# UDC-GAC/pRIblast

Measured on AMD Instinct MI355X. Metric: query RNAs/sec in `ris` step, higher is better.
Workload: dtype f64

## Files before the change

include/priblast_hip.h:

```cpp
#ifndef PRIBLAST_HIP_H
#define PRIBLAST_HIP_H

#include <stddef.h>
#include <stdint.h>

#ifdef __cplusplus
extern "C" {
#endif

#define PRB_OK 0
#define PRB_ERR_ARG (-1)
#define PRB_ERR_IO (-2)
#define PRB_ERR_HIP (-3)
#define PRB_ERR_NOMEM (-4)
#define PRB_ERR_STATE (-5)

typedef struct prb_ctx prb_ctx;
typedef struct prb_db prb_db;
typedef struct prb_qbatch prb_qbatch;
typedef struct prb_hitset prb_hitset;
typedef struct prb_pairmask prb_pairmask;

typedef struct prb_ris_opts {
  int32_t max_seed_length;
  double hybrid_threshold;
  double interaction_threshold;
  double final_threshold;
  int32_t drop_out_wo_gap;
  int32_t drop_out_w_gap;
  int32_t min_helix_length;
  int32_t output_style;
  int32_t distinct_sites;
  int32_t chain_sites;
  const prb_pairmask *allowed_pairs;
} prb_ris_opts;
#ifdef __cplusplus
static_assert(sizeof(prb_ris_opts) == 64, "prb_ris_opts: eleven fields, allowed_pairs the last one, no tail padding");
#endif


int prb_pairmask_create(prb_ctx *ctx, const prb_qbatch *qb, const prb_db *db, prb_pairmask **out);
int prb_pairmask_allow(prb_pairmask *pm, int64_t n, const int32_t *query, const int32_t *page, const int32_t *db_id);
int64_t prb_pairmask_count(const prb_pairmask *pm);
void prb_pairmask_free(prb_pairmask *pm);

typedef struct prb_hit {
  int32_t q_sp, db_sp;
  int32_t q_len, db_len;
  int32_t db_id, db_id_start;
  double e_acc, e_hyb, e_tot;
  int32_t query;
  int32_t bp_count;
  int64_t bp_offset;
} prb_hit;

const char *prb_last_error(void);
const char *prb_version(void);
int prb_cpu_budget(void);
int prb_host_threads_default(void);
void prb_ris_opts_default(prb_ris_opts *o);

int prb_ctx_create(int device, const char *param_file, prb_ctx **out);
void prb_ctx_destroy(prb_ctx *ctx);
int prb_ctx_synchronize(prb_ctx *ctx);
int prb_ctx_stage_ms(prb_ctx *ctx, const char *stage, double *ms, int64_t *launches);
void prb_ctx_reset_timers(prb_ctx *ctx);

int prb_accessibility(prb_ctx *ctx, int32_t nseq, const char *seqs, const int64_t *offsets,
                      int32_t maximal_span, int32_t min_accessible_length, float *acc, float *cond);

int prb_accessibility_tables(prb_ctx *ctx, const char *seq, int32_t len, int32_t maximal_span,
                             int32_t min_accessible_length, float *acc, float *cond,
                             double *alpha_outer, double *beta_outer, double *const tables[12]);

int prb_encode_query(const char *seq, int32_t len, int32_t repeat_flag, uint8_t *enc );
int prb_suffix_array(const uint8_t *text, int32_t n, int32_t *sa);
int prb_shuffle_sequence(const char *seq, int32_t len, uint64_t seed, int64_t file_pos, int32_t decoy, char *out);

int prb_db_open(prb_ctx *ctx, const char *prefix, prb_db **out);
int prb_db_open_streaming(prb_ctx *ctx, const char *prefix, int32_t max_resident_pages, prb_db **out);
int64_t prb_db_page_uploads(const prb_db *db);
void prb_db_close(prb_db *db);
int prb_db_info(const prb_db *db, int32_t *hash_size, int32_t *repeat_flag, int32_t *maximal_span,
                int32_t *min_accessible_length, int32_t *npages);
int prb_db_page_info(const prb_db *db, int32_t page, int32_t *nseq, int64_t *nchars);
const char *prb_db_seq_name(const prb_db *db, int32_t page, int32_t id);
int prb_db_seq_lengths(const prb_db *db, int32_t page, int32_t id, int32_t *length,
                       int32_t *length_unmasked, int32_t *start_pos);
int prb_db_build(prb_ctx *ctx, const char *prefix, int32_t nseq, const char *const *names,
                 const char *seqs, const int64_t *offsets, int32_t repeat_flag, int32_t hash_size,
                 int32_t maximal_span, int32_t min_accessible_length, int32_t page_size);

int prb_qbatch_create(prb_ctx *ctx, int32_t nq, const char *seqs, const int64_t *offsets,
                      int32_t repeat_flag, prb_qbatch **out);
void prb_qbatch_destroy(prb_qbatch *qb);
int prb_qbatch_accessibility(prb_ctx *ctx, prb_qbatch *qb, int32_t maximal_span,
                             int32_t min_accessible_length);
int prb_qbatch_get(prb_qbatch *qb, int32_t q, uint8_t *enc, int32_t *sa, float *acc, float *cond);
int32_t prb_qbatch_length_unmasked(const prb_qbatch *qb, int32_t q);
int prb_qbatch_seed_search_begin(prb_ctx *ctx, prb_qbatch *qb, const prb_db *db, int32_t page, const prb_ris_opts *opts);

int prb_search_page(prb_ctx *ctx, prb_qbatch *qb, prb_db *db, int32_t page, const prb_ris_opts *opts,
                    int32_t last_stage, prb_hitset **out);
int64_t prb_hitset_size(const prb_hitset *hs);
const prb_hit *prb_hitset_hits(const prb_hitset *hs);
const int32_t *prb_hitset_basepairs(const prb_hitset *hs, int64_t *count);
void prb_hitset_counts(const prb_hitset *hs, int64_t counts[3]);
void prb_hitset_free(prb_hitset *hs);

int prb_distinct_sites(prb_ctx *ctx, const prb_hit *hits, int64_t n, uint8_t *keep);
int prb_chain_sites(prb_ctx *ctx, const prb_hit *hits, int64_t n, uint8_t *keep);

enum {
  PRB_SORT_PACKED_TWO_LENGTHS = 0,
  PRB_SORT_PACKED_ONE_LENGTH = 1,
  PRB_SORT_GENERAL_WIDTH = 2,
  PRB_SORT_GENERAL_TIE_RUN = 3,
  PRB_SORT_GENERAL_FORCED = 4
};
int prb_sort_filter(prb_ctx *ctx, const prb_hit *hits, int64_t n, double threshold, prb_hit *sorted, uint8_t *keep,
                    int32_t *form);

typedef struct prb_pair_summary {
  int32_t query, db_id;
  int64_t hits;
  double e_min, e_sum, e_acc, e_hyb;
  int32_t bp_first[2], bp_last[2];
} prb_pair_summary;
typedef struct prb_pairset prb_pairset;
int prb_search_page_summary(prb_ctx *ctx, prb_qbatch *qb, prb_db *db, int32_t page, const prb_ris_opts *opts,
                            prb_pairset **out);
int64_t prb_pairset_size(const prb_pairset *ps);
const prb_pair_summary *prb_pairset_pairs(const prb_pairset *ps);
void prb_pairset_counts(const prb_pairset *ps, int64_t counts[3]);
void prb_pairset_free(prb_pairset *ps);

typedef struct prb_top_pair {
  prb_pair_summary s;
  int32_t page, rank;
} prb_top_pair;
typedef struct prb_topset prb_topset;
int prb_topset_create(prb_ctx *ctx, const prb_qbatch *qb, int32_t n, prb_topset **out);
int prb_search_page_top(prb_ctx *ctx, prb_qbatch *qb, prb_db *db, int32_t page, const prb_ris_opts *opts,
                        prb_topset *ts);
int prb_topset_merge(prb_ctx *ctx, prb_topset *dst, prb_topset *src);
int prb_topset_finish(prb_ctx *ctx, prb_topset *ts);
int64_t prb_topset_size(const prb_topset *ts);
const prb_top_pair *prb_topset_pairs(const prb_topset *ts);
void prb_topset_counts(const prb_topset *ts, int64_t counts[3]);
void prb_topset_free(prb_topset *ts);

typedef struct prb_top_hit {
  prb_hit h;
  int32_t page, rank;
} prb_top_hit;
typedef struct prb_tophits prb_tophits;
int prb_tophits_create(prb_ctx *ctx, const prb_qbatch *qb, int32_t n, prb_tophits **out);
int prb_search_page_tophits(prb_ctx *ctx, prb_qbatch *qb, prb_db *db, int32_t page, const prb_ris_opts *opts,
                            prb_tophits *th);
int prb_tophits_merge(prb_ctx *ctx, prb_tophits *dst, prb_tophits *src);
int prb_tophits_finish(prb_ctx *ctx, prb_tophits *th);
int64_t prb_tophits_size(const prb_tophits *th);
const prb_top_hit *prb_tophits_hits(const prb_tophits *th);
const int32_t *prb_tophits_basepairs(const prb_tophits *th, int64_t *npairs);
void prb_tophits_counts(const prb_tophits *th, int64_t counts[3]);
void prb_tophits_free(prb_tophits *th);

typedef struct prb_profile_pos {
  int32_t query, pos;
  int64_t hits;
  int32_t targets, page, db_id;
  int32_t reserved;
  double e_min;
  int32_t bp_first[2], bp_last[2];
} prb_profile_pos;
typedef struct prb_profset prb_profset;
int prb_profset_create(prb_ctx *ctx, const prb_qbatch *qb, prb_profset **out);
int prb_search_page_profile(prb_ctx *ctx, prb_qbatch *qb, prb_db *db, int32_t page, const prb_ris_opts *opts,
                            prb_profset *ps);
int prb_profset_merge(prb_ctx *ctx, prb_profset *dst, prb_profset *src);
int prb_profset_finish(prb_ctx *ctx, prb_profset *ps);
int64_t prb_profset_size(const prb_profset *ps);
const prb_profile_pos *prb_profset_rows(const prb_profset *ps);
void prb_profset_counts(const prb_profset *ps, int64_t counts[3]);
void prb_profset_free(prb_profset *ps);

typedef struct prb_target_pair {
  prb_pair_summary s;
  int32_t page, rank;
} prb_target_pair;
typedef struct prb_targetset prb_targetset;
int prb_targetset_create(prb_ctx *ctx, prb_db *db, int32_t n, prb_targetset **out);
int prb_search_page_targets(prb_ctx *ctx, prb_qbatch *qb, prb_db *db, int32_t page, const prb_ris_opts *opts,
                            const int32_t *query_ids, prb_targetset *ts);
int prb_targetset_merge(prb_ctx *ctx, prb_targetset *dst, prb_targetset *src);
int prb_targetset_finish(prb_ctx *ctx, prb_targetset *ts);
int64_t prb_targetset_size(const prb_targetset *ts);
const prb_target_pair *prb_targetset_pairs(const prb_targetset *ts);
void prb_targetset_counts(const prb_targetset *ts, int64_t counts[3]);
void prb_targetset_free(prb_targetset *ts);

typedef struct prb_target_region {
  int32_t page, db_id;
  int32_t start, end;
  int64_t hits, max_hits;
  int32_t max_queries, peak;
  double e_min;
  int32_t query, reserved;
  int32_t bp_first[2], bp_last[2];
} prb_target_region;
#ifdef __cplusplus
static_assert(sizeof(prb_target_region) == 72, "prb_target_region: no padding");
#endif
// ... 81 lines not shown
```

priblast_amd/capi.py:

```python
import ctypes
import os
import subprocess

import numpy as np

ROOT = os.path.dirname(os.path.abspath(__file__))
LIB_PATH = os.environ.get("PRB_LIB_PATH") or os.path.join(ROOT, "lib", "libpriblast_hip.so")
BIN_PATH = os.path.join(ROOT, "bin", "pRIblast-hip")
PARAMS = os.path.join(ROOT, "params", "rna_andronescu2007.par")

c_i32, c_i64, c_dbl = ctypes.c_int32, ctypes.c_int64, ctypes.c_double
P = ctypes.POINTER


class RisOpts(ctypes.Structure):
    _fields_ = [("max_seed_length", c_i32), ("hybrid_threshold", c_dbl), ("interaction_threshold", c_dbl),
                ("final_threshold", c_dbl), ("drop_out_wo_gap", c_i32), ("drop_out_w_gap", c_i32),
                ("min_helix_length", c_i32), ("output_style", c_i32), ("distinct_sites", c_i32), ("chain_sites", c_i32),
                ("allowed_pairs", ctypes.c_void_p)]


class Hit(ctypes.Structure):
    _fields_ = [("q_sp", c_i32), ("db_sp", c_i32), ("q_len", c_i32), ("db_len", c_i32), ("db_id", c_i32),
                ("db_id_start", c_i32), ("e_acc", c_dbl), ("e_hyb", c_dbl), ("e_tot", c_dbl), ("query", c_i32),
                ("bp_count", c_i32), ("bp_offset", c_i64)]


class PageHits(ctypes.Structure):
    _fields_ = [("hits", ctypes.c_void_p), ("nhits", c_i64), ("basepairs", ctypes.c_void_p), ("npairs", c_i64)]


HIT_DTYPE = np.dtype([("q_sp", "<i4"), ("db_sp", "<i4"), ("q_len", "<i4"), ("db_len", "<i4"), ("db_id", "<i4"),
                      ("db_id_start", "<i4"), ("e_acc", "<f8"), ("e_hyb", "<f8"), ("e_tot", "<f8"),
                      ("query", "<i4"), ("bp_count", "<i4"), ("bp_offset", "<i8")])
assert HIT_DTYPE.itemsize == ctypes.sizeof(Hit)

PAIR_DTYPE = np.dtype([("query", "<i4"), ("db_id", "<i4"), ("hits", "<i8"), ("e_min", "<f8"), ("e_sum", "<f8"),
                       ("e_acc", "<f8"), ("e_hyb", "<f8"), ("bp_first", "<i4", (2,)), ("bp_last", "<i4", (2,))])
assert PAIR_DTYPE.itemsize == 64

TOP_DTYPE = np.dtype(PAIR_DTYPE.descr + [("page", "<i4"), ("rank", "<i4")])
assert TOP_DTYPE.itemsize == 72

TOPHIT_DTYPE = np.dtype(HIT_DTYPE.descr + [("page", "<i4"), ("rank", "<i4")])
assert TOPHIT_DTYPE.itemsize == 72

TARGET_DTYPE = np.dtype(PAIR_DTYPE.descr + [("page", "<i4"), ("rank", "<i4")])
assert TARGET_DTYPE.itemsize == 72

PROFILE_DTYPE = np.dtype([("query", "<i4"), ("pos", "<i4"), ("hits", "<i8"), ("targets", "<i4"), ("page", "<i4"),
                          ("db_id", "<i4"), ("reserved", "<i4"), ("e_min", "<f8"), ("bp_first", "<i4", (2,)),
                          ("bp_last", "<i4", (2,))])
assert PROFILE_DTYPE.itemsize == 56

REGION_DTYPE = np.dtype([("page", "<i4"), ("db_id", "<i4"), ("start", "<i4"), ("end", "<i4"), ("hits", "<i8"),
                         ("max_hits", "<i8"), ("max_queries", "<i4"), ("peak", "<i4"), ("e_min", "<f8"), ("query", "<i4"),
                         ("reserved", "<i4"), ("bp_first", "<i4", (2,)), ("bp_last", "<i4", (2,))])
assert REGION_DTYPE.itemsize == 72

NULL_DTYPE = np.dtype(PAIR_DTYPE.descr + [("page", "<i4"), ("decoys", "<i4"), ("null_hits", "<i8"), ("null_le", "<i8"),
                                          ("null_min", "<f8")])
assert NULL_DTYPE.itemsize == 96


class PagePairs(ctypes.Structure):
    _fields_ = [("pairs", ctypes.c_void_p), ("npairs", c_i64)]

SYMBOLS = {
    "prb_last_error": (ctypes.c_char_p, []),
    "prb_version": (ctypes.c_char_p, []),
    "prb_cpu_budget": (ctypes.c_int, []),
    "prb_host_threads_default": (ctypes.c_int, []),
    "prb_ris_opts_default": (None, [P(RisOpts)]),
    "prb_ctx_create": (ctypes.c_int, [ctypes.c_int, ctypes.c_char_p, P(ctypes.c_void_p)]),
    "prb_ctx_destroy": (None, [ctypes.c_void_p]),
    "prb_ctx_synchronize": (ctypes.c_int, [ctypes.c_void_p]),
    "prb_ctx_stage_ms": (ctypes.c_int, [ctypes.c_void_p, ctypes.c_char_p, P(c_dbl), P(c_i64)]),
    "prb_ctx_reset_timers": (None, [ctypes.c_void_p]),
    "prb_accessibility": (ctypes.c_int, [ctypes.c_void_p, c_i32, ctypes.c_char_p, ctypes.c_void_p, c_i32, c_i32,
                                         ctypes.c_void_p, ctypes.c_void_p]),
    "prb_accessibility_tables": (ctypes.c_int, [ctypes.c_void_p, ctypes.c_char_p, c_i32, c_i32, c_i32,
                                                ctypes.c_void_p, ctypes.c_void_p, ctypes.c_void_p, ctypes.c_void_p,
                                                ctypes.c_void_p]),
    "prb_encode_query": (ctypes.c_int, [ctypes.c_char_p, c_i32, c_i32, ctypes.c_void_p]),
    "prb_suffix_array": (ctypes.c_int, [ctypes.c_void_p, c_i32, ctypes.c_void_p]),
    "prb_db_open": (ctypes.c_int, [ctypes.c_void_p, ctypes.c_char_p, P(ctypes.c_void_p)]),
    "prb_db_open_streaming": (ctypes.c_int, [ctypes.c_void_p, ctypes.c_char_p, c_i32, P(ctypes.c_void_p)]),
    "prb_db_page_uploads": (c_i64, [ctypes.c_void_p]),
    "prb_db_close": (None, [ctypes.c_void_p]),
    "prb_db_info": (ctypes.c_int, [ctypes.c_void_p, P(c_i32), P(c_i32), P(c_i32), P(c_i32), P(c_i32)]),
    "prb_db_page_info": (ctypes.c_int, [ctypes.c_void_p, c_i32, P(c_i32), P(c_i64)]),
    "prb_db_seq_name": (ctypes.c_char_p, [ctypes.c_void_p, c_i32, c_i32]),
    "prb_db_seq_lengths": (ctypes.c_int, [ctypes.c_void_p, c_i32, c_i32, P(c_i32), P(c_i32), P(c_i32)]),
    "prb_db_build": (ctypes.c_int, [ctypes.c_void_p, ctypes.c_char_p, c_i32, P(ctypes.c_char_p), ctypes.c_char_p,
                                    ctypes.c_void_p, c_i32, c_i32, c_i32, c_i32, c_i32]),
    "prb_qbatch_create": (ctypes.c_int, [ctypes.c_void_p, c_i32, ctypes.c_char_p, ctypes.c_void_p, c_i32,
                                         P(ctypes.c_void_p)]),
    "prb_qbatch_destroy": (None, [ctypes.c_void_p]),
    "prb_qbatch_accessibility": (ctypes.c_int, [ctypes.c_void_p, ctypes.c_void_p, c_i32, c_i32]),
    "prb_qbatch_get": (ctypes.c_int, [ctypes.c_void_p, c_i32, ctypes.c_void_p, ctypes.c_void_p, ctypes.c_void_p,
                                      ctypes.c_void_p]),
    "prb_qbatch_length_unmasked": (c_i32, [ctypes.c_void_p, c_i32]),
    "prb_qbatch_seed_search_begin": (ctypes.c_int, [ctypes.c_void_p, ctypes.c_void_p, ctypes.c_void_p, c_i32, P(RisOpts)]),
    "prb_search_page": (ctypes.c_int, [ctypes.c_void_p, ctypes.c_void_p, ctypes.c_void_p, c_i32, P(RisOpts), c_i32,
                                       P(ctypes.c_void_p)]),
    "prb_pairmask_create": (ctypes.c_int, [ctypes.c_void_p, ctypes.c_void_p, ctypes.c_void_p, P(ctypes.c_void_p)]),
    "prb_pairmask_allow": (ctypes.c_int, [ctypes.c_void_p, c_i64, ctypes.c_void_p, ctypes.c_void_p, ctypes.c_void_p]),
    "prb_pairmask_count": (c_i64, [ctypes.c_void_p]),
    "prb_pairmask_free": (None, [ctypes.c_void_p]),
    "prb_hitset_size": (c_i64, [ctypes.c_void_p]),
    "prb_hitset_hits": (ctypes.c_void_p, [ctypes.c_void_p]),
    "prb_hitset_basepairs": (ctypes.c_void_p, [ctypes.c_void_p, P(c_i64)]),
    "prb_hitset_counts": (None, [ctypes.c_void_p, P(c_i64)]),
    "prb_hitset_free": (None, [ctypes.c_void_p]),
    "prb_distinct_sites": (ctypes.c_int, [ctypes.c_void_p, ctypes.c_void_p, c_i64, ctypes.c_void_p]),
    "prb_chain_sites": (ctypes.c_int, [ctypes.c_void_p, ctypes.c_void_p, c_i64, ctypes.c_void_p]),
    "prb_sort_filter": (ctypes.c_int, [ctypes.c_void_p, ctypes.c_void_p, c_i64, c_dbl, ctypes.c_void_p, ctypes.c_void_p,
                                       ctypes.c_void_p]),
    "prb_search_page_summary": (ctypes.c_int, [ctypes.c_void_p, ctypes.c_void_p, ctypes.c_void_p, c_i32, P(RisOpts),
                                               P(ctypes.c_void_p)]),
    "prb_pairset_size": (c_i64, [ctypes.c_void_p]),
    "prb_pairset_pairs": (ctypes.c_void_p, [ctypes.c_void_p]),
    "prb_pairset_counts": (None, [ctypes.c_void_p, P(c_i64)]),
    "prb_pairset_free": (None, [ctypes.c_void_p]),
    "prb_topset_create": (ctypes.c_int, [ctypes.c_void_p, ctypes.c_void_p, c_i32, P(ctypes.c_void_p)]),
    "prb_search_page_top": (ctypes.c_int, [ctypes.c_void_p, ctypes.c_void_p, ctypes.c_void_p, c_i32, P(RisOpts), ctypes.c_void_p]),
    "prb_topset_merge": (ctypes.c_int, [ctypes.c_void_p, ctypes.c_void_p, ctypes.c_void_p]),
    "prb_topset_finish": (ctypes.c_int, [ctypes.c_void_p, ctypes.c_void_p]),
    "prb_topset_size": (c_i64, [ctypes.c_void_p]),
    "prb_topset_pairs": (ctypes.c_void_p, [ctypes.c_void_p]),
    "prb_topset_counts": (None, [ctypes.c_void_p, P(c_i64)]),
    "prb_topset_free": (None, [ctypes.c_void_p]),
    "prb_tophits_create": (ctypes.c_int, [ctypes.c_void_p, ctypes.c_void_p, c_i32, P(ctypes.c_void_p)]),
    "prb_search_page_tophits": (ctypes.c_int, [ctypes.c_void_p, ctypes.c_void_p, ctypes.c_void_p, c_i32, P(RisOpts), ctypes.c_void_p]),
    "prb_tophits_merge": (ctypes.c_int, [ctypes.c_void_p, ctypes.c_void_p, ctypes.c_void_p]),
    "prb_tophits_finish": (ctypes.c_int, [ctypes.c_void_p, ctypes.c_void_p]),
    "prb_tophits_size": (c_i64, [ctypes.c_void_p]),
    "prb_tophits_hits": (ctypes.c_void_p, [ctypes.c_void_p]),
    "prb_tophits_basepairs": (ctypes.c_void_p, [ctypes.c_void_p, P(c_i64)]),
    "prb_tophits_counts": (None, [ctypes.c_void_p, P(c_i64)]),
    "prb_tophits_free": (None, [ctypes.c_void_p]),
    "prb_profset_create": (ctypes.c_int, [ctypes.c_void_p, ctypes.c_void_p, P(ctypes.c_void_p)]),
    "prb_search_page_profile": (ctypes.c_int, [ctypes.c_void_p, ctypes.c_void_p, ctypes.c_void_p, c_i32, P(RisOpts), ctypes.c_void_p]),
    "prb_profset_merge": (ctypes.c_int, [ctypes.c_void_p, ctypes.c_void_p, ctypes.c_void_p]),
    "prb_profset_finish": (ctypes.c_int, [ctypes.c_void_p, ctypes.c_void_p]),
    "prb_profset_size": (c_i64, [ctypes.c_void_p]),
    "prb_profset_rows": (ctypes.c_void_p, [ctypes.c_void_p]),
    "prb_profset_counts": (None, [ctypes.c_void_p, P(c_i64)]),
    "prb_profset_free": (None, [ctypes.c_void_p]),
    "prb_targetset_create": (ctypes.c_int, [ctypes.c_void_p, ctypes.c_void_p, c_i32, P(ctypes.c_void_p)]),
    "prb_search_page_targets": (ctypes.c_int, [ctypes.c_void_p, ctypes.c_void_p, ctypes.c_void_p, c_i32, P(RisOpts), ctypes.c_void_p,
                                               ctypes.c_void_p]),
    "prb_targetset_merge": (ctypes.c_int, [ctypes.c_void_p, ctypes.c_void_p, ctypes.c_void_p]),
    "prb_targetset_finish": (ctypes.c_int, [ctypes.c_void_p, ctypes.c_void_p]),
    "prb_targetset_size": (c_i64, [ctypes.c_void_p]),
    "prb_targetset_pairs": (ctypes.c_void_p, [ctypes.c_void_p]),
    "prb_targetset_counts": (None, [ctypes.c_void_p, P(c_i64)]),
    "prb_targetset_free": (None, [ctypes.c_void_p]),
    "prb_covset_create": (ctypes.c_int, [ctypes.c_void_p, ctypes.c_void_p, P(ctypes.c_void_p)]),
    "prb_search_page_coverage": (ctypes.c_int, [ctypes.c_void_p, ctypes.c_void_p, ctypes.c_void_p, c_i32, P(RisOpts), ctypes.c_void_p,
                                                ctypes.c_void_p]),
    "prb_covset_add_hits": (ctypes.c_int, [ctypes.c_void_p, ctypes.c_void_p, c_i32, ctypes.c_void_p, c_i32, ctypes.c_void_p, c_i64,
                                           ctypes.c_void_p, c_i64]),
    "prb_covset_merge": (ctypes.c_int, [ctypes.c_void_p, ctypes.c_void_p, ctypes.c_void_p]),
    "prb_covset_finish": (ctypes.c_int, [ctypes.c_void_p, ctypes.c_void_p, c_i32]),
    "prb_covset_size": (c_i64, [ctypes.c_void_p]),
    "prb_covset_regions": (ctypes.c_void_p, [ctypes.c_void_p]),
    "prb_covset_counts": (None, [ctypes.c_void_p, P(c_i64)]),
    "prb_covset_free": (None, [ctypes.c_void_p]),
    "prb_nullset_create": (ctypes.c_int, [ctypes.c_void_p, ctypes.c_void_p, ctypes.c_void_p, c_i32, P(ctypes.c_void_p)]),
    "prb_search_page_observed": (ctypes.c_int, [ctypes.c_void_p, ctypes.c_void_p, ctypes.c_void_p, c_i32, P(RisOpts), ctypes.c_void_p]),
    "prb_search_page_decoys": (ctypes.c_int, [ctypes.c_void_p, ctypes.c_void_p, ctypes.c_void_p, c_i32, P(RisOpts), ctypes.c_void_p,
                                              ctypes.c_void_p, ctypes.c_void_p]),
    "prb_nullset_observe": (ctypes.c_int, [ctypes.c_void_p, ctypes.c_void_p, c_i32, ctypes.c_void_p, c_i64]),
    "prb_nullset_add_pairs": (ctypes.c_int, [ctypes.c_void_p, ctypes.c_void_p, c_i32, ctypes.c_void_p, ctypes.c_void_p, c_i32,
                                             ctypes.c_void_p, c_i64]),
    "prb_nullset_finish": (ctypes.c_int, [ctypes.c_void_p, ctypes.c_void_p]),
    "prb_nullset_size": (c_i64, [ctypes.c_void_p]),
    "prb_nullset_pairs": (ctypes.c_void_p, [ctypes.c_void_p]),
    "prb_nullset_counts": (None, [ctypes.c_void_p, P(c_i64)]),
    "prb_nullset_decoy_counts": (None, [ctypes.c_void_p, P(c_i64)]),
    "prb_nullset_free": (None, [ctypes.c_void_p]),
    "prb_write_null_lines": (ctypes.c_int, [ctypes.c_void_p, c_i32, P(ctypes.c_char_p), ctypes.c_void_p, ctypes.c_void_p, c_i64,
                                            c_i64, ctypes.c_int, P(c_i64), P(c_i64)]),
    "prb_comm_unique_id": (ctypes.c_int, [ctypes.c_char_p]),
    "prb_comm_create": (ctypes.c_int, [ctypes.c_void_p, c_i32, c_i32, ctypes.c_char_p, P(ctypes.c_void_p)]),
    "prb_comm_destroy": (None, [ctypes.c_void_p]),
    "prb_gather_hits": (ctypes.c_int, [ctypes.c_void_p, ctypes.c_void_p, c_i32, ctypes.c_void_p, c_i32, P(ctypes.c_void_p)]),
    "prb_hitset_gathered_queries": (ctypes.c_int, [ctypes.c_void_p, P(c_i32), P(P(c_i32)), P(P(c_i32))]),
    "prb_gather_plan": (ctypes.c_int, [c_i32, ctypes.c_void_p, ctypes.c_void_p]),
    "prb_ctx_keep_device_records": (None, [ctypes.c_void_p, c_i32]),
    "prb_write_lines": (ctypes.c_int, [ctypes.c_void_p, c_i32, P(ctypes.c_char_p), ctypes.c_void_p, ctypes.c_void_p, c_i32,
                                       c_i32, c_i64, ctypes.c_int, P(c_i64), P(c_i64)]),
    "prb_write_summary_lines": (ctypes.c_int, [ctypes.c_void_p, c_i32, P(ctypes.c_char_p), ctypes.c_void_p, ctypes.c_void_p,
                                               c_i32, c_i64, ctypes.c_int, P(c_i64), P(c_i64)]),
    "prb_write_top_lines": (ctypes.c_int, [ctypes.c_void_p, c_i32, P(ctypes.c_char_p), ctypes.c_void_p, ctypes.c_void_p, c_i64,
                                           c_i64, ctypes.c_int, P(c_i64), P(c_i64)]),
    "prb_shuffle_sequence": (ctypes.c_int, [ctypes.c_char_p, c_i32, ctypes.c_uint64, c_i64, c_i32, ctypes.c_char_p]),
    "prb_write_target_lines": (ctypes.c_int, [ctypes.c_void_p, c_i32, P(ctypes.c_char_p), ctypes.c_void_p, ctypes.c_void_p, c_i64,
                                              c_i64, ctypes.c_int, P(c_i64), P(c_i64)]),
    "prb_write_profile_lines": (ctypes.c_int, [ctypes.c_void_p, c_i32, P(ctypes.c_char_p), ctypes.c_void_p, ctypes.c_void_p, c_i64,
                                               c_i64, ctypes.c_int, P(c_i64), P(c_i64)]),
    "prb_write_region_lines": (ctypes.c_int, [ctypes.c_void_p, c_i32, P(ctypes.c_char_p), ctypes.c_void_p, ctypes.c_void_p, c_i64,
                                              c_i64, ctypes.c_int, P(c_i64), P(c_i64)]),
}

_lib = None


def build():
    subprocess.run(["make", "-s", "-j8", "-C", os.path.join(ROOT, "csrc")], check=True)


def lib():
    global _lib
    if _lib is None:
        if not os.path.exists(LIB_PATH):
            raise RuntimeError(f"{LIB_PATH} is missing: run `python -c 'import __graft_entry__ as g; g.build()'` "
                               "(there is no CPU fallback)")
        L = ctypes.CDLL(LIB_PATH)
        for name, (res, args) in SYMBOLS.items():
            if not hasattr(L, name):
                continue
            fn = getattr(L, name)
            fn.restype = res
            fn.argtypes = args
        _lib = L
    return _lib


class PrbError(RuntimeError):
    pass


def _check(rc):
    if rc != 0:
        raise PrbError(f"libpriblast_hip error {rc}: {lib().prb_last_error().decode()}")


def _concat(seqs):
    offs = np.zeros(len(seqs) + 1, np.int64)
    for i, s in enumerate(seqs):
        offs[i + 1] = offs[i] + len(s)
    return "".join(seqs).encode(), offs


def encode_query(seq, repeat_flag=0):
    enc = np.zeros(len(seq) + 1, np.uint8)
    _check(lib().prb_encode_query(seq.encode(), len(seq), repeat_flag, enc.ctypes.data))
    return enc


def suffix_array(text):
    text = np.ascontiguousarray(text, np.uint8)
    sa = np.zeros(len(text), np.int32)
    _check(lib().prb_suffix_array(text.ctypes.data, len(text), sa.ctypes.data))
    return sa


def shuffle_sequence(seq, seed=1, file_pos=0, decoy=0):
    raw = seq.encode("latin-1") if isinstance(seq, str) else bytes(seq)
    out = ctypes.create_string_buffer(max(len(raw), 1))
    _check(lib().prb_shuffle_sequence(raw, len(raw), seed, file_pos, decoy, out))
    res = out.raw[:len(raw)]
    return res.decode("latin-1") if isinstance(seq, str) else res


def default_opts(**kw):
    o = RisOpts()
    lib().prb_ris_opts_default(ctypes.byref(o))
    for k, v in kw.items():
        setattr(o, k, v)
    return o


class Context:
    def __init__(self, device=0, param_file=None):
        h = ctypes.c_void_p()
        _check(lib().prb_ctx_create(device, param_file.encode() if param_file else PARAMS.encode(), ctypes.byref(h)))
        self.h = h

    def close(self):
        if self.h:
            lib().prb_ctx_destroy(self.h)
            self.h = None

    def __enter__(self):
        return self

    def __exit__(self, *a):
        self.close()

    def accessibility(self, seqs, W=70, delta=5):
        buf, offs = _concat(seqs)
        total = int(offs[-1])
        acc = np.zeros(max(total, 1), np.float32)
        cond = np.zeros(max(total, 1), np.float32)
        _check(lib().prb_accessibility(self.h, len(seqs), buf, offs.ctypes.data, W, delta, acc.ctypes.data,
                                       cond.ctypes.data))
        return [(acc[offs[i]:offs[i + 1]], cond[offs[i]:offs[i + 1]]) for i in range(len(seqs))]

    def accessibility_tables(self, seq, W=70, delta=5):
        L = len(seq)
        acc = np.zeros(max(L, 1), np.float32)
        cond = np.zeros(max(L, 1), np.float32)
        out = {"alpha_outer": np.zeros(L + 1), "beta_outer": np.zeros(L + 1)}
        names = ["stem", "stemend", "multi", "multibif", "multi1", "multi2"]
        ptrs = (ctypes.c_void_p * 12)()
        k = 0
        for side in ("alpha", "beta"):
            for nm in names:
                t = np.zeros((L + 1, W + 2))
                out[f"{side}_{nm}"] = t
                ptrs[k] = t.ctypes.data
                k += 1
        _check(lib().prb_accessibility_tables(self.h, seq.encode(), L, W, delta, acc.ctypes.data, cond.ctypes.data,
                                              out["alpha_outer"].ctypes.data, out["beta_outer"].ctypes.data, ptrs))
        return acc[:L], cond[:L], out

    def stage_ms(self, stage):
        ms, n = c_dbl(), c_i64()
        _check(lib().prb_ctx_stage_ms(self.h, stage.encode(), ctypes.byref(ms), ctypes.byref(n)))
        return ms.value, n.value

    def reset_timers(self):
        lib().prb_ctx_reset_timers(self.h)

    def synchronize(self):
        _check(lib().prb_ctx_synchronize(self.h))


class Db:

    def __init__(self, ctx, prefix, max_resident_pages=None):
        h = ctypes.c_void_p()
        if max_resident_pages is None:
            _check(lib().prb_db_open(ctx.h, prefix.encode(), ctypes.byref(h)))
        else:
            _check(lib().prb_db_open_streaming(ctx.h, prefix.encode(), max_resident_pages, ctypes.byref(h)))
        self.h, self.ctx = h, ctx
        v = [c_i32() for _ in range(5)]
        _check(lib().prb_db_info(self.h, *[ctypes.byref(x) for x in v]))
        self.hash_size, self.repeat_flag, self.W, self.delta, self.npages = (x.value for x in v)

    def close(self):
        if self.h:
            lib().prb_db_close(self.h)
            self.h = None

    @property
    def page_uploads(self):
        return lib().prb_db_page_uploads(self.h)

    def page_info(self, page):
        n, c = c_i32(), c_i64()
        _check(lib().prb_db_page_info(self.h, page, ctypes.byref(n), ctypes.byref(c)))
        return n.value, c.value

    def seq_name(self, page, i):
        return lib().prb_db_seq_name(self.h, page, i).decode()

    def seq_lengths(self, page, i):
        a, b, c = c_i32(), c_i32(), c_i32()
        _check(lib().prb_db_seq_lengths(self.h, page, i, ctypes.byref(a), ctypes.byref(b), ctypes.byref(c)))
        return a.value, b.value, c.value


def db_build(ctx, prefix, names, seqs, repeat_flag=0, hash_size=8, W=70, delta=5, page_size=2 ** 31 - 1):
    buf, offs = _concat(seqs)
    arr = (ctypes.c_char_p * len(names))(*[n.encode() for n in names])
    _check(lib().prb_db_build(ctx.h, prefix.encode(), len(seqs), arr, buf, offs.ctypes.data, repeat_flag, hash_size, W,
                              delta, page_size))


class QBatch:

    def __init__(self, ctx, seqs, repeat_flag=0):
        buf, offs = _concat(seqs)
        h = ctypes.c_void_p()
        _check(lib().prb_qbatch_create(ctx.h, len(seqs), buf, offs.ctypes.data, repeat_flag, ctypes.byref(h)))
        self.h, self.ctx, self.lens = h, ctx, [len(s) for s in seqs]

    def close(self):
        if self.h:
            lib().prb_qbatch_destroy(self.h)
            self.h = None

    def accessibility(self, W, delta):
        _check(lib().prb_qbatch_accessibility(self.ctx.h, self.h, W, delta))

    def get(self, q):
        L = self.lens[q]
        enc = np.zeros(L + 1, np.uint8)
        sa = np.zeros(L + 1, np.int32)
        acc = np.zeros(max(L, 1), np.float32)
        cond = np.zeros(max(L, 1), np.float32)
        _check(lib().prb_qbatch_get(self.h, q, enc.ctypes.data, sa.ctypes.data, acc.ctypes.data, cond.ctypes.data))
        return enc, sa, acc[:L], cond[:L]

    def length_unmasked(self, q):
        return lib().prb_qbatch_length_unmasked(self.h, q)

    def seed_search_begin(self, db, page, opts=None):
        o = opts or default_opts()
        _check(lib().prb_qbatch_seed_search_begin(self.ctx.h, self.h, db.h, page, ctypes.byref(o)))


class PairMask:

    def __init__(self, ctx, qb, db):
        h = ctypes.c_void_p()
        _check(lib().prb_pairmask_create(ctx.h, qb.h, db.h, ctypes.byref(h)))
        self.h = h

    def allow(self, query, page, db_id):
        q, p, d = (np.ascontiguousarray(np.atleast_1d(x), np.int32) for x in (query, page, db_id))
        assert len(q) == len(p) == len(d)
        _check(lib().prb_pairmask_allow(self.h, len(q), q.ctypes.data, p.ctypes.data, d.ctypes.data))
        return self

# ... 455 lines not shown
```

priblast_amd/csrc/capi_search.hip:

```cpp
#include <omp.h>

#include <algorithm>
#include <cmath>
#include <cstdlib>
#include <cstring>

#include "search_stages.hpp"

using namespace prb;

namespace prb {

static bool env_off(const char *e) { return e && atoi(e) == 0; }
static SearchKnobs read_search_knobs() {
  SearchKnobs k;
  const char *e;
  e = getenv("PRB_SEARCH_PAIRS");
  k.budget = e ? atof(e) : 4.0e8;
  k.chunk_pairs = k.budget;
  if ((e = getenv("PRB_SEARCH_CHUNK_PAIRS"))) k.chunk_pairs = atof(e);
  e = getenv("PRB_SEED_ROW_SHIFT");
  k.row_shift = e ? std::min(atoi(e), 30) : 7;
  k.fused = !env_off(getenv("PRB_SEED_FUSED"));
  k.front_ahead = !getenv("PRB_NO_FRONT_AHEAD");
  k.sort_four_keys = getenv("PRB_SORT_FOUR_KEYS") != nullptr;
  k.sort_two_lengths = getenv("PRB_SORT_TWO_LENGTHS") != nullptr;
  e = getenv("PRB_BIG_LIST_BYTES");
  k.big_list_bytes = e ? (size_t)atof(e) : (size_t)20 << 30;
  e = getenv("PRB_GAPPED_CHUNK_HITS");
  k.gapped_chunk_hits = e ? std::max<int64_t>(1, (int64_t)atof(e)) : 120000000;
  e = getenv("PRB_GAPPED_FIRST_TIER");
  k.first_tier = e ? std::min(std::max(atoi(e), 0), kWaveTier) : 0;
  k.wave_hbm = getenv("PRB_GAPPED_WAVE_HBM") != nullptr;
  k.no_resume = getenv("PRB_GAPPED_NO_RESUME") != nullptr;
  e = getenv("PRB_GAPPED_RESUME_CAP");
  k.resume_cap = e ? std::max(1, atoi(e)) : 0;
  k.front_paired = getenv("PRB_GAPPED_FRONT_PAIRED") != nullptr;
  e = getenv("PRB_GAPPED_SKIP_TIERS");
  k.skip_tiers = e ? atoi(e) : 0;
  k.front = !env_off(getenv("PRB_GAPPED_FRONT"));
  k.handover = !env_off(getenv("PRB_GAPPED_HANDOVER"));
  k.tiers.pair = !env_off(getenv("PRB_GAPPED_PAIR"));
  k.tiers.pool = !env_off(getenv("PRB_GAPPED_POOL"));
  GapTierKnobs &t = k.tiers;
  if ((e = getenv("PRB_GAPPED_LDS_PAD"))) sscanf(e, "%d,%d,%d", &t.pad[1], &t.pad[2], &t.pad[3]);
  t.pad_set = e != nullptr;
  if ((e = getenv("PRB_GAPPED_PERIOD"))) sscanf(e, "%d,%d,%d,%d", &t.period[0], &t.period[1], &t.period[2], &t.period[3]);
  t.period_set = e != nullptr;
  if ((e = getenv("PRB_GAPPED_EARLY"))) sscanf(e, "%d,%d,%d,%d", &t.early[0], &t.early[1], &t.early[2], &t.early[3]);
  t.early_set = e != nullptr;
  k.filter_tiles = !env_off(getenv("PRB_FILTER_TILES"));
  k.trace_no_long = getenv("PRB_TRACE_NO_LONG") != nullptr;
  e = getenv("PRB_TRACE_LONG_CAP");
  k.trace_long_cap = e ? std::max(1, atoi(e)) : 1024;
  k.trace_no_slots = getenv("PRB_TRACE_NO_SLOTS") != nullptr;
  e = getenv("PRB_TRACE_SLOT_CAP");
  k.trace_slot_cap = e ? std::min(kTraceCap, atoi(e)) : kTraceCap;
  e = getenv("PRB_DISTINCT_LDS_HITS");
  k.distinct_lds_hits = e ? atoi(e) : kSiteLdsHits;
  e = getenv("PRB_CHAIN_LDS_HITS");
  k.chain_lds_hits = e ? atoi(e) : kChainLdsHits;
  k.debug_rows = getenv("PRB_DEBUG_ROWS") != nullptr;
  k.debug_mem = getenv("PRB_DEBUG_MEM") != nullptr;
  return k;
}

HitSoA carve_hits(uint8_t *p, int64_t n) {
  HitSoA h;
  const size_t n8 = ((size_t)n + 1) & ~(size_t)1;
  h.e_acc = reinterpret_cast<double *>(p);
  h.e_hyb = h.e_acc + n8;
  h.e_tot = h.e_hyb + n8;
  int32_t *ip = reinterpret_cast<int32_t *>(h.e_tot + n8);
  h.q_sp = ip;
  h.db_sp = ip + n8;
  h.q_len = ip + 2 * n8;
  h.db_len = ip + 3 * n8;
  h.db_id = ip + 4 * n8;
  h.db_id_start = ip + 5 * n8;
  h.query = ip + 6 * n8;
  return h;
}

int sort_target_keys(hipStream_t s, DevBuf &tmp, const uint32_t *kin, uint32_t *kout, const uint32_t *vin, uint32_t *vout, size_t n, unsigned bits) {
  return sort_pairs(s, tmp, kin, kout, vin, vout, n, bits);
}
hipError_t sort_span_keys(void *tmp, size_t &bytes, uint64_t *kin, uint64_t *kout, uint32_t *vin, uint32_t *vout, size_t n, int bits, hipStream_t s) {
  return rocprim::radix_sort_pairs(tmp, bytes, kin, kout, vin, vout, n, 0, bits, s);
}

static int sort_hits(prb_ctx *ctx, SearchWs &w, const SearchKnobs &k, const HitRec *recs, HitSoA out, int64_t n, const SortBounds &sb,
                     uint32_t **perm_out, int32_t *form = nullptr) {
  int rc;
  int32_t why = PRB_SORT_GENERAL_FORCED;
  const size_t N = (size_t)n;
  {
    PackedKeyInfo f;
    f.qmin = sb.qmin;
    f.one_len = sb.eq_len_max > 0;
    f.lmax = f.one_len ? sb.eq_len_max : std::max(sb.max_qlen, sb.max_dblen);
    f.bl = bits_for(f.lmax);
    f.bq = bits_for(sb.max_qlen);
    f.bd = bits_for(sb.nchars);
    const int total = (f.one_len ? 1 : 2) * f.bl + f.bq + f.bd + bits_for(sb.qspan - 1);
    if (!k.sort_four_keys) why = PRB_SORT_GENERAL_WIDTH;
    if (total <= 64 && f.lmax <= 65535 && !k.sort_four_keys) {
      if ((rc = w.kP.ensure(N * 8)) || (rc = w.kTmp2.ensure(N * 8)) || (rc = w.kE.ensure(N * 8)) || (rc = w.kTmp.ensure(N * 8)) ||
          (rc = w.idxA.ensure(N * 4)) || (rc = w.idxB.ensure(N * 4)) || (rc = w.pending.ensure(16)))
        return rc;
      PRB_HIP(launch_make_packed_keys_recs(recs, n, f, w.kP.as<uint64_t>(), w.kE.as<uint64_t>(), w.idxA.as<uint32_t>(), ctx->stream));
      if ((rc = sort_pairs(ctx->stream, w.sortTmp, w.kP.as<uint64_t>(), w.kTmp2.as<uint64_t>(), w.idxA.as<uint32_t>(),
                           w.idxB.as<uint32_t>(), N, (unsigned)total)))
        return rc;
      PRB_HIP(launch_gather_u64(w.kE.as<uint64_t>(), w.idxB.as<uint32_t>(), w.kTmp.as<uint64_t>(), n, ctx->stream));
      PRB_HIP(hipMemsetAsync(w.pending.p, 0, 4, ctx->stream));
      PRB_HIP(launch_fix_ties(w.kTmp2.as<uint64_t>(), w.kTmp.as<uint64_t>(), w.idxB.as<uint32_t>(), n, recs, w.idxA.as<uint32_t>(),
                              w.pending.as<int32_t>(), ctx->stream));
      int32_t too_long = 0;
      PRB_HIP(hipMemcpyAsync(&too_long, w.pending.p, 4, hipMemcpyDeviceToHost, ctx->stream));
      PRB_HIP(hipStreamSynchronize(ctx->stream));
      if (!too_long) {
        PRB_HIP(launch_gather_recs_to_hits(recs, w.idxA.as<uint32_t>(), out, n, ctx->stream));
        *perm_out = w.idxA.as<uint32_t>();
        if (form) *form = f.one_len ? PRB_SORT_PACKED_ONE_LENGTH : PRB_SORT_PACKED_TWO_LENGTHS;
        return PRB_OK;
      }
      why = PRB_SORT_GENERAL_TIE_RUN;
    }
  }
  if (form) *form = why;
  if (k.debug_mem) fprintf(stderr, "[mem] sort: the general form (%lld hits)\n", (long long)n);
  if ((rc = w.hitsTmp.ensure(hits_bytes(n)))) return rc;
  const HitSoA in = carve_hits(w.hitsTmp, n);
  PRB_HIP(launch_gather_recs_to_hits(recs, nullptr, in, n, ctx->stream));
  if ((rc = w.kE.ensure(N * 8)) || (rc = w.kL.ensure(N * 4)) || (rc = w.kQ.ensure(N * 4)) || (rc = w.kP.ensure(N * 8)) ||
      (rc = w.kTmp.ensure(N * 8)) || (rc = w.kTmp2.ensure(N * 8)) || (rc = w.idxA.ensure(N * 4)) ||
      (rc = w.idxB.ensure(N * 4)))
    return rc;
  PRB_HIP(launch_make_keys(in, n, w.kE.as<uint64_t>(), w.kL.as<uint32_t>(), w.kQ.as<uint32_t>(), w.kP.as<uint64_t>(),
                           w.idxA.as<uint32_t>(), ctx->stream));
  uint32_t *ia = w.idxA.as<uint32_t>(), *ib = w.idxB.as<uint32_t>();
  auto sort_step = [&](auto *keys, unsigned bits) -> int {
    using K = std::remove_pointer_t<decltype(keys)>;
    if (int r = sort_pairs(ctx->stream, w.sortTmp, keys, w.kTmp2.as<K>(), ia, ib, N, bits)) return r;
    std::swap(ia, ib);
    return PRB_OK;
  };
  PRB_HIP(launch_order_keys(in.e_acc, n, w.kTmp.as<uint64_t>(), ctx->stream));
  if ((rc = sort_step(w.kTmp.as<uint64_t>(), 64))) return rc;
  PRB_HIP(launch_order_keys(in.e_hyb, n, w.kTmp2.as<uint64_t>(), ctx->stream));
  PRB_HIP(launch_gather_u64(w.kTmp2.as<uint64_t>(), ia, w.kTmp.as<uint64_t>(), n, ctx->stream));
  if ((rc = sort_step(w.kTmp.as<uint64_t>(), 64))) return rc;
  PRB_HIP(launch_gather_u64(w.kE.as<uint64_t>(), ia, w.kTmp.as<uint64_t>(), n, ctx->stream));
  if ((rc = sort_step(w.kTmp.as<uint64_t>(), 64))) return rc;
  PRB_HIP(launch_gather_u32(w.kL.as<uint32_t>(), ia, w.kTmp.as<uint32_t>(), n, ctx->stream));
  if ((rc = sort_step(w.kTmp.as<uint32_t>(), 32))) return rc;
  PRB_HIP(launch_gather_u32(w.kQ.as<uint32_t>(), ia, w.kTmp.as<uint32_t>(), n, ctx->stream));
  if ((rc = sort_step(w.kTmp.as<uint32_t>(), 32))) return rc;
  PRB_HIP(launch_gather_u64(w.kP.as<uint64_t>(), ia, w.kTmp.as<uint64_t>(), n, ctx->stream));
  unsigned qbits = 1;
  while ((int64_t(1) << qbits) < (int64_t)sb.qmin + sb.qspan && qbits < 31) qbits++;
  if ((rc = sort_step(w.kTmp.as<uint64_t>(), 32 + qbits))) return rc;
  PRB_HIP(launch_gather_hits(in, ia, out, n, ctx->stream));
  *perm_out = ia;
  return PRB_OK;
}

struct MaxOp {
  __host__ __device__ int64_t operator()(const int64_t &a, const int64_t &b) const { return a > b ? a : b; }
};

static int filter_hits(prb_ctx *ctx, SearchWs &w, const HitSoA &h, int64_t n, double thr, bool tiles, int64_t *nsurv) {
  int rc;
  const size_t N = (size_t)n;
  *nsurv = 0;
  if (n == 0) return PRB_OK;
  if ((rc = w.endKey.ensure(N * 8)) || (rc = w.pmax.ensure(N * 8)) || (rc = w.state.ensure(N)) || (rc = w.keep.ensure(N)) ||
      (rc = w.pending.ensure(16)) || (rc = w.surv.ensure(N * 4)) || (rc = w.count.ensure(16)))
    return rc;
  PRB_HIP(launch_filter_init(h, n, thr, w.endKey.as<int64_t>(), w.state.as<uint8_t>(), ctx->stream));
  if ((rc = with_temp(w.scanTmp, "rocprim::inclusive_scan", [&](void *t, size_t &b) {
         return rocprim::inclusive_scan(t, b, w.endKey.as<int64_t>(), w.pmax.as<int64_t>(), N, MaxOp(), ctx->stream);
       })))
    return rc;
  for (int round = 0;; round++) {
    PRB_HIP(hipMemsetAsync(w.pending.p, 0, 4, ctx->stream));
    PRB_HIP(launch_filter_round(h, n, w.pmax.as<int64_t>(), w.state.as<uint8_t>(), w.pending.as<int32_t>(), tiles, ctx->stream));
    int32_t pend = 0;
    PRB_HIP(hipMemcpyAsync(&pend, w.pending.p, 4, hipMemcpyDeviceToHost, ctx->stream));
    PRB_HIP(hipStreamSynchronize(ctx->stream));
    if (!pend) break;
    if (round > 100000) {
      set_error("redundancy filter did not converge");
      return PRB_ERR_STATE;
    }
  }
  PRB_HIP(launch_filter_final(h, n, w.pmax.as<int64_t>(), w.state.as<uint8_t>(), w.keep.as<uint8_t>(), tiles, ctx->stream));
  return select_flagged(ctx, w, nullptr, w.keep.as<uint8_t>(), w.surv.as<uint32_t>(), N, nsurv);
}

static void mem_note(const char *where, const SearchWs &w) {
  static const bool on = getenv("PRB_DEBUG_MEM") != nullptr;
  if (!on) return;
  size_t free_b = 0, total_b = 0;
  (void)hipMemGetInfo(&free_b, &total_b);
  fprintf(stderr, "[mem] %-18s free %7zu MiB | hitsA %6zu hitsB %6zu hitsC %6zu hitsTmp %6zu MiB\n", where, free_b >> 20, w.hitsA.cap >> 20,
          w.hitsB.cap >> 20, w.hitsC.cap >> 20, w.hitsTmp.cap >> 20);
}

int grow_keep(prb_ctx *ctx, DevBuf &buf, size_t have, size_t need, size_t spare_limit) {
  int rc;
  if (have > 0 && need > buf.cap) {
    DevBuf bigger;
    if ((rc = need > spare_limit ? PRB_ERR_NOMEM : bigger.ensure(need + need / 2)) && (rc = bigger.ensure(need + need / 6)) &&
        (rc = bigger.ensure(need)))
      return rc;
    PRB_HIP(hipMemcpyAsync(bigger.p, buf.p, have, hipMemcpyDeviceToDevice, ctx->stream));
    PRB_HIP(hipStreamSynchronize(ctx->stream));
    buf.release();
    buf = bigger;
    return PRB_OK;
  }
  return buf.ensure(need);
}
static int reserve_recs(prb_ctx *ctx, DevBuf &recbuf, int64_t have, int64_t more) {
  return grow_keep(ctx, recbuf, (size_t)have * sizeof(HitRec), ((size_t)have + (size_t)more) * sizeof(HitRec), (size_t)16 << 30);
}

int compact_below(prb_ctx *ctx, SearchWs &w, const HitSoA &in, int64_t n, double thr, DevBuf &idxbuf, DevBuf &recbuf, int64_t *m,
                  int64_t have) {
  int rc;
  *m = 0;
  if (n == 0) return PRB_OK;
  const size_t N = (size_t)n;
  if ((rc = w.keep.ensure(N)) || (rc = idxbuf.ensure(N * 4)) || (rc = w.count.ensure(16))) return rc;
  PRB_HIP(launch_flag_not_above(in.e_tot, n, thr, w.keep.as<uint8_t>(), ctx->stream));
  if ((rc = select_flagged(ctx, w, nullptr, w.keep.as<uint8_t>(), idxbuf.as<uint32_t>(), N, m))) return rc;
  if ((rc = reserve_recs(ctx, recbuf, have, std::max<int64_t>(*m, 1)))) return rc;
  PRB_HIP(launch_gather_hits_to_recs(in, idxbuf.as<uint32_t>(), recbuf.as<HitRec>() + have, *m, ctx->stream));
  return PRB_OK;
}

static int download_hits(prb_ctx *ctx, SearchWs &w, const HitSoA &h, int64_t n, std::vector<prb_hit> &out) {
  HostTimer ht(ctx, "host_download");
  const size_t base = out.size();
  if (n == 0) return PRB_OK;
  int rc;
  const size_t bytes = (size_t)n * sizeof(prb_hit);
  if ((rc = w.packed.ensure(bytes)) || (rc = w.pinned.ensure(bytes))) return rc;
  PRB_HIP(launch_pack_hits(h, n, nullptr, nullptr, -1, w.packed.p, ctx->stream));
  PRB_HIP(hipMemcpyAsync(w.pinned.p, w.packed.p, bytes, hipMemcpyDeviceToHost, ctx->stream));
  if (out.capacity() < base + (size_t)n) out.reserve(std::max(2 * out.capacity(), base + (size_t)n));
  PRB_HIP(hipStreamSynchronize(ctx->stream));
  const prb_hit *src = static_cast<const prb_hit *>(w.pinned.p);
  out.insert(out.end(), src, src + n);
  return PRB_OK;
}

static int32_t chunk_end(const CandDev *cd, int32_t ncand, int32_t c0, double chunk_pairs, double *pairs_out) {
  int32_t c1 = c0;
  double acc = 0;
  while (c1 < ncand) {
    const double pairs = (double)(cd[c1].ep_q - cd[c1].sp_q + 1) * (double)(cd[c1].ep_db - cd[c1].sp_db + 1);
    if (c1 > c0 && (acc + pairs > chunk_pairs || c1 - c0 >= kMaxFusedCands)) break;
    acc += pairs;
    c1++;
  }
  *pairs_out = acc;
  return c1;
}

struct RowKeyBits {
  int dbits, kbits;
  bool wide() const { return kbits > 32; }
};
static RowKeyBits row_key_bits(const PageDev &pd, int row_shift, const CandDev *cd, int32_t nc) {
  const int dbits = bits_for(std::max<int64_t>(1, ((int64_t)pd.nchars - 1) >> row_shift));
  return RowKeyBits{dbits, dbits + bits_for(std::max<int64_t>(1, (int64_t)cd[nc - 1].query - cd[0].query))};
}
template <class V>
static int sort_by_row_key(hipStream_t s, DevBuf &tmp, const RowKeyBits &kb, DevBuf &kin, DevBuf &kout, const V *vin, V *vout, size_t n) {
  return kb.wide() ? sort_pairs(s, tmp, kin.as<uint64_t>(), kout.as<uint64_t>(), vin, vout, n, (unsigned)kb.kbits)
                   : sort_pairs(s, tmp, kin.as<uint32_t>(), kout.as<uint32_t>(), vin, vout, n, (unsigned)kb.kbits);
}

static int scan_row_counts(prb_ctx *ctx, SearchWs &w, int64_t n) {
  auto in = rocprim::make_transform_iterator(w.row_count.as<int32_t>(), ToI64());
  return with_temp(w.scanTmp, "rocprim::exclusive_scan", [&](void *t, size_t &b) {
    return rocprim::exclusive_scan(t, b, in, w.row_off.as<int64_t>(), (int64_t)0, (size_t)n + 1, rocprim::plus<int64_t>(), ctx->stream);
  });
}

static int issue_front(SearchWs &w, const prb_qbatch *qb, const PageDev &pd, int delta, int row_shift, const CandDev *cd, int32_t nc,
                       int64_t cents, hipStream_t s, int64_t *np_out, const AllowDev *allow, prb_ctx *timed) {
  SearchWs::FrontStage &F = w.front;
  int rc;
  *np_out = -1;
  if ((rc = F.pair0_pin.ensure(((size_t)nc + 1) * 8))) return rc;
  int64_t *pair0 = static_cast<int64_t *>(F.pair0_pin.p);
  int64_t np = 0;
  for (int32_t c = 0; c < nc; c++) {
    const int64_t qw = cd[c].ep_q - cd[c].sp_q + 1;
    if (qw > kMaxFusedEntries) return PRB_OK;
    pair0[c] = np;
    np += qw * (int64_t)(cd[c].ep_db - cd[c].sp_db + 1);
  }
  pair0[nc] = np;
  const size_t NP = (size_t)np;
  const RowKeyBits kb = row_key_bits(pd, row_shift, cd, nc);
  if ((rc = F.cands.ensure((size_t)nc * sizeof(CandDev))) || (rc = F.seed_qacc.ensure((size_t)std::max<int64_t>(cents, 1) * 8)) ||
      (rc = F.pair0.ensure(((size_t)nc + 1) * 8)) || (rc = F.keyA.ensure(NP * (kb.wide() ? 8 : 4))) ||
      (rc = F.keyB.ensure(NP * (kb.wide() ? 8 : 4))) || (rc = F.valA.ensure(NP * 8)) || (rc = F.valB.ensure(NP * 8)))
    return rc;
  PRB_HIP(hipMemcpyAsync(F.cands.p, cd, (size_t)nc * sizeof(CandDev), hipMemcpyHostToDevice, s));
  PRB_HIP(hipMemcpyAsync(F.pair0.p, pair0, ((size_t)nc + 1) * 8, hipMemcpyHostToDevice, s));
  PRB_HIP(launch_seed_qacc(F.cands.as<CandDev>(), nc, cents, qb->view, delta, F.seed_qacc.as<double>(), s));
  PRB_HIP(launch_pair_keys(F.cands.as<CandDev>(), F.pair0.as<int64_t>(), nc, np, pd, cd[0].query, row_shift, kb.dbits, kb.wide(), F.keyA.p,
                           F.valA.as<uint64_t>(), s));
  F.unsorted = false;
  F.np_all = np;
  F.vals = F.valB.as<uint64_t>();
  if (allow) {
    const int64_t nw = allow_words(np);
    if ((rc = F.ballot.ensure((size_t)nw * 8)) || (rc = F.wcount.ensure((size_t)(nw + 1) * 4)) || (rc = F.woff.ensure((size_t)(nw + 1) * 8)) ||
        (rc = F.kept_pin.ensure(8)))
      return rc;
    if (timed && ((rc = timed->time_end("seed", 1)) || (rc = timed->time_begin()))) return rc;
    PRB_HIP(hipMemsetAsync(F.wcount.as<int32_t>() + nw, 0, 4, s));
    PRB_HIP(launch_allow_test(F.cands.as<CandDev>(), F.pair0.as<int64_t>(), F.valA.as<uint64_t>(), np, pd, *allow, F.ballot.as<uint64_t>(),
                              F.wcount.as<int32_t>(), s));
    auto counts = rocprim::make_transform_iterator(F.wcount.as<int32_t>(), ToI64());
    if ((rc = with_temp(F.scanTmp, "rocprim::exclusive_scan", [&](void *t, size_t &b) {
           return rocprim::exclusive_scan(t, b, counts, F.woff.as<int64_t>(), (int64_t)0, (size_t)nw + 1, rocprim::plus<int64_t>(), s);
         })))
      return rc;
    PRB_HIP(launch_allow_scatter(F.keyA.p, F.valA.as<uint64_t>(), np, kb.wide(), F.ballot.as<uint64_t>(), F.woff.as<int64_t>(), F.keyB.p,
                                 F.valB.as<uint64_t>(), s));
    PRB_HIP(hipMemcpyAsync(F.kept_pin.p, F.woff.as<int64_t>() + nw, 8, hipMemcpyDeviceToHost, s));
    if (timed && ((rc = timed->time_end(timed->allow_timer, 3)) || (rc = timed->time_begin()))) return rc;
    F.unsorted = true;
    F.key_bits = kb.kbits;
    *np_out = np;
    return PRB_OK;
  }
  if ((rc = sort_by_row_key(s, F.sortTmp, kb, F.keyA, F.keyB, F.valA.as<uint64_t>(), F.valB.as<uint64_t>(), NP))) return rc;
  *np_out = np;
  return PRB_OK;
}

static int finish_front(prb_ctx *ctx, SearchWs &w, const SearchKnobs &k, int32_t nc, int64_t *np) {
  SearchWs::FrontStage &F = w.front;
  int rc;
  PRB_HIP(hipStreamSynchronize(ctx->stream));
  F.unsorted = false;
  const int64_t kept = *static_cast<const int64_t *>(F.kept_pin.p);
  if (kept < 0 || kept > F.np_all) {
    set_error("pair mask: " + std::to_string(kept) + " of " + std::to_string(F.np_all) + " pairs kept");
    return PRB_ERR_STATE;
  }
  if (k.debug_rows) fprintf(stderr, "[allow] cands %d pairs %lld allowed %lld\n", nc, (long long)F.np_all, (long long)kept);
  *np = kept;
  if (kept == 0) return PRB_OK;
  if ((rc = sort_by_row_key(ctx->stream, F.sortTmp, RowKeyBits{0, F.key_bits}, F.keyB, F.keyA, F.valB.as<uint64_t>(), F.valA.as<uint64_t>(),
                            (size_t)kept)))
    return rc;
  F.vals = F.valA.as<uint64_t>();
  return PRB_OK;
}

struct SeedChunk {
  int32_t c0, c1, nc;
  int64_t crows, cents;
  double pairs;
};

static int count_hits_under_f(SubSearch &s, int64_t more) {
  s.nf += more;
  if (s.nf > (int64_t)UINT32_MAX - 16) {
    set_error("more than 4e9 hits under the -f threshold in one sub-batch: build the database in smaller pages (db -c)");
    return PRB_ERR_NOMEM;
  }
  return PRB_OK;
}

static int seed_chunk_one_pass(SubSearch &s, const SeedChunk &c, int64_t np) {
  prb_ctx *ctx = s.ctx;
  SearchWs &w = s.w;
  SearchWs::FrontStage &F = w.front;
  int rc;
  if ((rc = w.count.ensure(16))) return rc;
  if ((rc = ctx->time_end("seed", s.allow ? 1 : 2))) return rc;
  if ((rc = ctx->time_begin())) return rc;
  const int64_t nsl = fused_slices(np);
  if ((rc = w.hitsA.ensure((size_t)nsl * kFusePairs * kSliceRecBytes)) || (rc = w.row_count.ensure((size_t)(nsl + 1) * 4)) ||
      (rc = w.row_off.ensure((size_t)(nsl + 1) * 8)))
    return rc;
  PRB_HIP(hipMemsetAsync(w.count.p, 0, 16, ctx->stream));
  PRB_HIP(hipMemsetAsync(w.row_count.as<int32_t>() + nsl, 0, 4, ctx->stream));
  PRB_HIP(launch_seed_extend(F.cands.as<CandDev>(), F.vals, np, s.qb->view, s.pd, s.sc, s.eo, F.seed_qacc.as<double>(),
                             s.opts.interaction_threshold, s.max_qlen, w.hitsA.p, w.row_count.as<int32_t>(), w.count.as<uint64_t>(),
                             ctx->stream));
  if ((rc = scan_row_counts(ctx, w, nsl))) return rc;
  uint64_t kept = 0, seeds_maxlen[2] = {0, 0};
  PRB_HIP(hipMemcpyAsync(seeds_maxlen, w.count.p, 16, hipMemcpyDeviceToHost, ctx->stream));
  PRB_HIP(hipMemcpyAsync(&kept, w.row_off.as<int64_t>() + nsl, 8, hipMemcpyDeviceToHost, ctx->stream));
  PRB_HIP(hipStreamSynchronize(ctx->stream));
  s.one_pass_maxlen = std::max<int64_t>(s.one_pass_maxlen, (int64_t)seeds_maxlen[1]);
  if (kept > 0) {
    if ((rc = reserve_recs(ctx, w.hitsB, s.nf, (int64_t)kept))) return rc;
    PRB_HIP(launch_collect_slices(w.hitsA.p, w.row_count.as<int32_t>(), w.row_off.as<int64_t>(), nsl, w.hitsB.as<HitRec>() + s.nf,
                                  ctx->stream));
  }
  if ((rc = ctx->time_end("ungapped", 1))) return rc;
  s.hs->counts[0] += (int64_t)seeds_maxlen[0];
  if (s.k.debug_rows)
    fprintf(stderr, "[pairs] cands %d pairs %lld seeds %lld kept %lld\n", c.nc, (long long)np, (long long)seeds_maxlen[0], (long long)kept);
  return count_hits_under_f(s, (int64_t)kept);
}

static int seed_chunk_lists(SubSearch &s, const SeedChunk &c) {
  prb_ctx *ctx = s.ctx;
  SearchWs &w = s.w;
  const CandDev *cd = s.b.cd + c.c0;
  const int32_t nc = c.nc;
  const int64_t crows = c.crows, cents = c.cents;
  const int delta = s.eo.delta;
  int rc;
  s.all_one_pass = false;
  if ((rc = w.cands.ensure((size_t)nc * sizeof(CandDev))) || (rc = w.row_count.ensure((size_t)(crows + 1) * 4)) ||
      (rc = w.row_off.ensure((size_t)(crows + 1) * 8)) || (rc = w.row_cand.ensure((size_t)(crows + 1) * 4)) ||
      (rc = w.seed_qacc.ensure((size_t)std::max<int64_t>(cents, 1) * 8)))
    return rc;
  PRB_HIP(hipMemcpyAsync(w.cands.p, cd, (size_t)nc * sizeof(CandDev), hipMemcpyHostToDevice, ctx->stream));
  if ((rc = ctx->time_begin())) return rc;
  PRB_HIP(hipMemsetAsync(w.row_count.as<int32_t>() + crows, 0, 4, ctx->stream));
  PRB_HIP(launch_seed_qacc(w.cands.as<CandDev>(), nc, cents, s.qb->view, delta, w.seed_qacc.as<double>(), ctx->stream));
  const uint32_t *row_perm = nullptr;
  if (s.last_stage != 1 && crows > 1 && crows < (int64_t)UINT32_MAX && s.k.row_shift >= 0) {
    const size_t NR = (size_t)crows;
    const RowKeyBits kb = row_key_bits(s.pd, s.k.row_shift, cd, nc);
    if ((rc = w.kP.ensure(NR * 8)) || (rc = w.kTmp2.ensure(NR * 8)) || (rc = w.idxA.ensure(NR * 4)) || (rc = w.idxB.ensure(NR * 4)))
      return rc;
    PRB_HIP(launch_row_keys(w.cands.as<CandDev>(), nc, crows, s.pd, cd[0].query, s.k.row_shift, kb.dbits, kb.wide(), w.row_cand.as<int32_t>(),
                            w.kP.p, w.idxA.as<uint32_t>(), ctx->stream));
    if ((rc = sort_by_row_key(ctx->stream, w.sortTmp, kb, w.kP, w.kTmp2, w.idxA.as<uint32_t>(), w.idxB.as<uint32_t>(), NR))) return rc;
    row_perm = w.idxB.as<uint32_t>();
  }
  if (s.allow)
    PRB_HIP(launch_seed_count_allowed(w.cands.as<CandDev>(), nc, crows, s.qb->view, s.pd, delta, w.seed_qacc.as<double>(),
                                      w.row_count.as<int32_t>(), w.row_cand.as<int32_t>(), row_perm, *s.allow, ctx->stream));
  else
    PRB_HIP(launch_seed_count(w.cands.as<CandDev>(), nc, crows, s.qb->view, s.pd, delta, w.seed_qacc.as<double>(),
                              w.row_count.as<int32_t>(), w.row_cand.as<int32_t>(), row_perm, ctx->stream));
  if ((rc = scan_row_counts(ctx, w, crows))) return rc;
  int64_t nseed = 0;
  PRB_HIP(hipMemcpyAsync(&nseed, w.row_off.as<int64_t>() + crows, 8, hipMemcpyDeviceToHost, ctx->stream));
  PRB_HIP(hipStreamSynchronize(ctx->stream));
  s.hs->counts[0] += nseed;
  if (s.k.debug_rows)
    fprintf(stderr, "[rows] cands %d rows %lld qents %lld pairs %.0f seeds %lld\n", nc, (long long)crows, (long long)cents, c.pairs, (long long)nseed);
  if (nseed == 0) return ctx->time_end("seed", 2);
  if (nseed > (int64_t)UINT32_MAX - 16) {
    set_error("too many seed hits in one chunk of candidates (a single candidate with more than 4e9 seed hits?): lower "
              "PRB_SEARCH_CHUNK_PAIRS");
    return PRB_ERR_NOMEM;
  }
  if ((rc = w.hitsA.ensure(hits_bytes(nseed)))) return rc;
  HitSoA A = carve_hits(w.hitsA, nseed);
  if (s.allow)
    PRB_HIP(launch_seed_emit_allowed(w.cands.as<CandDev>(), nc, crows, s.qb->view, s.pd, delta, w.seed_qacc.as<double>(),
                                     w.row_cand.as<int32_t>(), w.row_off.as<int64_t>(), A, row_perm, *s.allow, ctx->stream));
  else
    PRB_HIP(launch_seed_emit(w.cands.as<CandDev>(), nc, crows, s.qb->view, s.pd, delta, w.seed_qacc.as<double>(),
                             w.row_cand.as<int32_t>(), w.row_off.as<int64_t>(), A, row_perm, ctx->stream));
  if ((rc = ctx->time_end("seed", 2))) return rc;
  if (s.last_stage == 1) return download_hits(ctx, w, A, nseed, s.hs->hits);
  if ((rc = ctx->time_begin())) return rc;
  PRB_HIP(launch_ungapped(A, nseed, s.qb->view, s.pd, s.sc, s.eo, s.max_qlen, ctx->stream));
  if ((rc = ctx->time_end("ungapped", 1))) return rc;
  int64_t mc = 0;
  if ((rc = ctx->time_begin())) return rc;
  if ((rc = compact_below(ctx, w, A, nseed, s.opts.interaction_threshold, w.cidx, w.hitsB, &mc, s.nf))) return rc;
  if ((rc = ctx->time_end("filter", 2))) return rc;
  return count_hits_under_f(s, mc);
}

static int seeds_to_hits(SubSearch &s) {
  SearchWs &w = s.w;
  CandDev *cd = s.b.cd;
  int rc;
  if ((rc = w.front.init())) return rc;
  for (int32_t c0 = 0; c0 < s.ncand;) {
    SeedChunk c;
    c.c0 = c0;
    c.c1 = chunk_end(cd, s.ncand, c0, s.k.chunk_pairs, &c.pairs);
    c.nc = c.c1 - c0;
    const int64_t row_base = cd[c0].row0, ent_base = cd[c0].qoff;
    c.crows = (c.c1 < s.ncand ? cd[c.c1].row0 : s.b.nrows) - row_base;
    c.cents = (c.c1 < s.ncand ? cd[c.c1].qoff : s.b.nqent) - ent_base;
    for (int32_t i = c0; i < c.c1; i++) {
      cd[i].row0 -= row_base;
      cd[i].qoff -= ent_base;
    }
    int64_t np = -1;
    if (s.k.fused && s.last_stage != 1 && s.k.row_shift >= 0 && c.pairs < 4.0e9) {
      if ((rc = s.ctx->time_begin())) return rc;
      SearchWs::FrontStage &F = w.front;
      if (c0 == 0 && F.ahead && F.cd == cd && F.nc == c.nc) {
        np = F.np;
        PRB_HIP(hipStreamWaitEvent(s.ctx->stream, F.done, 0));
      } else {
        if (F.ahead) PRB_HIP(hipStreamSynchronize(F.stream));
        if ((rc = issue_front(w, s.qb, s.pd, s.eo.delta, s.k.row_shift, cd + c0, c.nc, c.cents, s.ctx->stream, &np, s.allow, s.ctx))) return rc;
      }
      F.ahead = false;
      if (np >= 0 && F.unsorted) {
        if ((rc = finish_front(s.ctx, w, s.k, c.nc, &np))) return rc;
        if (np == 0) {
          if ((rc = s.ctx->time_end("seed", 0))) return rc;
          c0 = c.c1;
          continue;
        }
      }
    }
    if ((rc = np >= 0 ? seed_chunk_one_pass(s, c, np) : seed_chunk_lists(s, c))) return rc;
    c0 = c.c1;
  }
  return PRB_OK;
}

static int sort_filter_ungapped(SubSearch &s) {
  prb_ctx *ctx = s.ctx;
  SearchWs &w = s.w;
  int rc;
  const bool big_list = hits_bytes(s.nf) > s.k.big_list_bytes;
  mem_note("seed chunks done", w);
  if (big_list) {
    w.trim_next = true;
    PRB_HIP(hipStreamSynchronize(ctx->stream));
    w.front.release();
    for (DevBuf *b : {&w.hitsA, &w.hitsTmp, &w.row_count, &w.row_off, &w.row_cand, &w.seed_qacc, &w.cands, &w.trace, &w.keptU, &w.keptTrace})
      b->release();
    for (DevBuf &b : w.resumePool) b.release();
    for (DevBuf *b : {&ctx->ra_band, &ctx->ra_vec, &ctx->ra_codes, &ctx->ra_desc}) b->release();
    if ((rc = w.front.init())) return rc;
  }
  mem_note("before the sort", w);
  if ((rc = w.hitsC.ensure(hits_bytes(s.nf)))) return rc;
  HitSoA B = carve_hits(w.hitsC, s.nf);
  uint32_t *perm = nullptr;
  if ((rc = ctx->time_begin())) return rc;
  SortBounds sb1 = s.sb;
  if (s.all_one_pass && s.one_pass_maxlen > 0 && !s.k.sort_two_lengths) sb1.eq_len_max = (int32_t)s.one_pass_maxlen;
  if ((rc = sort_hits(ctx, w, s.k, w.hitsB.as<HitRec>(), B, s.nf, sb1, &perm))) return rc;
  if ((rc = ctx->time_end("sort", 9))) return rc;
  if (big_list)
    for (DevBuf *b : {&w.hitsB, &w.kE, &w.kL, &w.kQ, &w.kP, &w.kTmp, &w.kTmp2, &w.idxA, &w.idxB, &w.sortTmp}) b->release();
  mem_note("sorted", w);
  if ((rc = ctx->time_begin())) return rc;
  if ((rc = filter_hits(ctx, w, B, s.nf, s.opts.interaction_threshold, s.k.filter_tiles, &s.nung))) return rc;
  if ((rc = ctx->time_end("filter", 3))) return rc;
  s.hs->counts[1] += s.nung;
  if (s.nung == 0) return PRB_OK;
  if ((rc = w.hitsA.ensure(hits_bytes(s.nung)))) return rc;
  s.U = carve_hits(w.hitsA, s.nung);
  PRB_HIP(launch_gather_hits(B, w.surv.as<uint32_t>(), s.U, s.nung, ctx->stream));
  if ((rc = w.first.ensure((size_t)s.nung))) return rc;
  PRB_HIP(launch_mark_first(s.U.query, s.nung, w.first.as<uint8_t>(), ctx->stream));
  s.first = w.first.as<uint8_t>();
  return PRB_OK;
}

static int emit_ungapped(SubSearch &s) {
  prb_hitset *hs = s.hs;
  const size_t base = hs->hits.size();
  if (int rc = download_hits(s.ctx, s.w, s.U, s.nung, hs->hits)) return rc;
  auto code_base = [](unsigned c) { return c <= 5 ? (int)c - 1 : (int)c - 5; };
  for (size_t i = base; i < hs->hits.size(); i++) {
    prb_hit &h = hs->hits[i];
    const uint8_t *qs = s.qb->enc.data() + s.qb->off[h.query];
    h.bp_offset = (int64_t)hs->bp.size() / 2;
    const int len = (int)(uint16_t)h.q_len;
    for (int j = 0; j < len; j++)
      if (s.ctx->params.bp_pair[code_base(qs[h.q_sp + j])][code_base(s.pg.seqs[h.db_sp + j])] != 0) {
        hs->bp.push_back(h.q_sp + j);
        hs->bp.push_back(h.db_sp + j);
        h.bp_count++;
      }
  }
  return PRB_OK;
}

static int final_sort_filter(SubSearch &s) {
  prb_ctx *ctx = s.ctx;
  SearchWs &w = s.w;
  int rc;
  if (!s.chunked) {
    if ((rc = ctx->time_begin())) return rc;
    if ((rc = compact_below(ctx, w, s.G, s.nung, s.opts.final_threshold, w.cidx, w.hitsB, &s.ngap))) return rc;
    if ((rc = ctx->time_end("filter", 2))) return rc;
  }
  if (s.ngap == 0) return PRB_OK;
  if ((rc = w.hitsC.ensure(hits_bytes(s.ngap)))) return rc;
  HitSoA S = carve_hits(w.hitsC, s.ngap);
  uint32_t *perm = nullptr;
  if ((rc = ctx->time_begin())) return rc;
  if ((rc = sort_hits(ctx, w, s.k, w.hitsB.as<HitRec>(), S, s.ngap, s.sb, &perm))) return rc;
  if ((rc = ctx->time_end("sort", 9))) return rc;
  if ((rc = ctx->time_begin())) return rc;
  if ((rc = filter_hits(ctx, w, S, s.ngap, s.opts.final_threshold, s.k.filter_tiles, &s.nfin))) return rc;
  if ((rc = ctx->time_end("filter", 3))) return rc;
  s.hs->counts[2] += s.nfin;
  if (s.nfin == 0) return PRB_OK;
  if ((rc = w.hitsB.ensure(hits_bytes(s.nfin)))) return rc;
  s.F = carve_hits(w.hitsB, s.nfin);
  PRB_HIP(launch_gather_hits(S, w.surv.as<uint32_t>(), s.F, s.nfin, ctx->stream));
  if ((rc = w.subset2.ensure((size_t)s.nfin * 4)) || (rc = w.subset.ensure((size_t)s.nfin * 4))) return rc;
  PRB_HIP(launch_gather_u32(perm, w.surv.as<uint32_t>(), w.subset2.as<uint32_t>(), s.nfin, ctx->stream));
  PRB_HIP(launch_gather_u32(w.cidx.as<uint32_t>(), w.subset2.as<uint32_t>(), w.subset.as<uint32_t>(), s.nfin, ctx->stream));
  return PRB_OK;
}

enum class SiteRule { kDistinct, kChain };
static const char *rule_name(SiteRule rule) { return rule == SiteRule::kChain ? "chain sites" : "distinct sites"; }
static StageTimer &rule_timer(prb_ctx *ctx, SiteRule rule) { return rule == SiteRule::kChain ? ctx->chain_timer : ctx->distinct_timer; }

static int select_sites(prb_ctx *ctx, SearchWs &w, const HitSoA &h, int64_t n, SiteRule rule, const SearchKnobs &k) {
  const size_t N = (size_t)n;
  const bool chain = rule == SiteRule::kChain;
  int rc;
  if (n > INT32_MAX) {
    set_error(std::string(rule_name(rule)) + ": more than 2^31 - 1 final hits in one list");
    return PRB_ERR_ARG;
  }
  if ((rc = w.pairHead.ensure(N)) || (rc = w.keep.ensure(N)) || (rc = w.state.ensure(N)) || (rc = w.endKey.ensure(N * (chain ? 8 : 4))) ||
      (rc = w.pmax.ensure(N * 4)) || (rc = w.listA.ensure((size_t)site_long_runs_max(n) * 4)) || (rc = w.pending.ensure(16)))
    return rc;
  PRB_HIP(launch_pair_heads(h.query, h.db_id, n, w.pairHead.as<uint8_t>(), ctx->stream));
  if (chain) {
    const ChainScratch scratch{w.listA.as<uint32_t>(), w.pending.as<uint32_t>(), w.endKey.as<double>(), w.pmax.as<int32_t>()};
    PRB_HIP(launch_chain_select(h, n, w.pairHead.as<uint8_t>(), k.chain_lds_hits, scratch, w.keep.as<uint8_t>(), ctx->stream));
  } else {
    const SiteScratch scratch{w.listA.as<uint32_t>(), w.pending.as<uint32_t>(), w.endKey.as<int32_t>(), w.pmax.as<int32_t>(), w.state.as<uint8_t>()};
    PRB_HIP(launch_site_select(h, n, w.pairHead.as<uint8_t>(), k.distinct_lds_hits, scratch, w.keep.as<uint8_t>(), ctx->stream));
  }
  return PRB_OK;
}

static int thin_sites(SubSearch &s, SiteRule rule) {
  prb_ctx *ctx = s.ctx;
  SearchWs &w = s.w;
  StageTimer &timer = rule_timer(ctx, rule);
  int rc;
  if ((rc = ctx->time_begin())) return rc;
  if ((rc = select_sites(ctx, w, s.F, s.nfin, rule, s.k))) return rc;
  int64_t nkeep = 0;
  if ((rc = w.surv.ensure((size_t)s.nfin * 4)) || (rc = w.count.ensure(16))) return rc;
  if ((rc = select_flagged(ctx, w, nullptr, w.keep.as<uint8_t>(), w.surv.as<uint32_t>(), (size_t)s.nfin, &nkeep))) return rc;
  if (nkeep <= 0 || nkeep > s.nfin) {
    set_error(std::string(rule_name(rule)) + ": " + std::to_string(nkeep) + " of " + std::to_string(s.nfin) + " final hits kept");
    return PRB_ERR_STATE;
  }
  if (nkeep == s.nfin) return ctx->time_end(timer, 4);
  if ((rc = w.hitsTmp.ensure(hits_bytes(nkeep))) || (rc = w.subset2.ensure((size_t)nkeep * 4))) return rc;
  const HitSoA kept = carve_hits(w.hitsTmp, nkeep);
  PRB_HIP(launch_gather_hits(s.F, w.surv.as<uint32_t>(), kept, nkeep, ctx->stream));
// ... 345 lines not shown
  }
  if (opts->chain_sites && opts->distinct_sites) {
    set_error(std::string(fn) + ": chain_sites and distinct_sites can't both be 1 (each of them selects among every final hit of a pair)");
    return PRB_ERR_ARG;
  }
  return PRB_OK;
}

static int convert_cands(prb_ctx *ctx, SeedPlan &plan, int32_t a, int32_t b, PinnedBuf &pin, CandBatch &out) {
  const int32_t nb = b - a;
  std::vector<int64_t> cbase((size_t)nb + 1, 0), rbase((size_t)nb + 1, 0), ebase((size_t)nb + 1, 0);
  for (int32_t k = 0; k < nb; k++) {
    cbase[k + 1] = cbase[k] + (int64_t)plan.per_q[a + k].size();
    rbase[k + 1] = rbase[k] + plan.qrows[a + k];
    ebase[k + 1] = ebase[k] + plan.qents[a + k];
  }
  out.q0 = a;
  out.q1 = b;
  out.ncand = cbase[nb];
  out.nrows = rbase[nb];
  out.nqent = ebase[nb];
  if (int r = pin.ensure((size_t)std::max<int64_t>(out.ncand, 1) * sizeof(CandDev))) return r;
  CandDev *cd = static_cast<CandDev *>(pin.p);
  out.cd = cd;
  HostTimer ht(ctx, "host_cands");
#pragma omp parallel for schedule(dynamic, 1) num_threads(std::min(8, host_threads(nb)))
  for (int32_t k = 0; k < nb; k++) {
    std::vector<SeedCandidate> &v = plan.per_q[a + k];
    CandDev *o = cd + cbase[k];
    int64_t row = rbase[k], ent = ebase[k];
    for (size_t i = 0; i < v.size(); i++) {
      const SeedCandidate &c = v[i];
      o[i] = CandDev{c.sp_q, c.ep_q, c.sp_db, c.ep_db, c.length, c.query, c.score, row, ent};
      row += (int64_t)c.ep_db - c.sp_db + 1;
      ent += (int64_t)c.ep_q - c.sp_q + 1;
    }
    std::vector<SeedCandidate>().swap(v);
  }
  return PRB_OK;
}

static bool take_queries(SeedPlan &plan, int32_t q0, double budget, bool wait, int32_t *q1_out) {
  int32_t q1 = q0;
  double acc = 0;
  for (; q1 < plan.nq; q1++) {
    if (wait) plan.wait_for(q1);
    else if (!plan.done[q1].load(std::memory_order_acquire)) return false;
    if (q1 > q0 && acc + plan.qpairs[q1] > budget) break;
    acc += plan.qpairs[q1];
  }
  *q1_out = q1;
  return true;
}

int search_page(prb_ctx *ctx, prb_qbatch *qb, prb_db *db, int32_t page, const prb_ris_opts *opts, int32_t last_stage,
                SearchMode mode, prb_hitset **out, TableState *table) {
  const bool summary = reduces_to_pairs(mode);
  const char *fn = summary ? "prb_search_page_summary" : "prb_search_page";
  if (!out) {
    set_error(std::string(fn) + ": bad argument");
    return PRB_ERR_ARG;
  }
  if (int rc = check_search_args(fn, ctx, qb, db, page, opts, last_stage)) return rc;
  *out = nullptr;
  PRB_HIP(hipSetDevice(ctx->device));
  AllowDev allow{};
  if (opts->allowed_pairs)
    if (int rc = use_pairmask(fn, ctx, qb, db, page, opts->allowed_pairs, &allow)) return rc;
  {
    int slot = -1, rcp;
    if ((rcp = page_slot(ctx, db, page, -1, ctx->stream, &slot))) return rcp;
    PRB_HIP(hipStreamWaitEvent(ctx->stream, db->slot_ready[(size_t)slot], 0));
    const int next = page + 1 < (int32_t)db->pages.size() ? page + 1 : 0;
    if (db->copy_stream && db->mem.size() >= 2 && next != page && db->slot_of_page[(size_t)next] < 0) {
      int ns = -1;
      if ((rcp = page_slot(ctx, db, next, page, db->copy_stream, &ns))) return rcp;
      db->slot_used[(size_t)slot] = ++db->clock;
    }
  }
  const int32_t nq = qb->nq;
  std::unique_ptr<SeedPlan> plan_owner;
  if (qb->plan && qb->plan->db == db && qb->plan->page == page && qb->plan->max_seed_length == opts->max_seed_length &&
      qb->plan->hybrid_threshold == opts->hybrid_threshold) {
    plan_owner = std::move(qb->plan);
  } else {
    plan_owner = start_seed_plan(ctx, qb, db, page, opts->max_seed_length, opts->hybrid_threshold);
  }
  SeedPlan &plan = *plan_owner;
  auto *hs = new prb_hitset();
  hs->device = ctx->device;
  hs->on_device = ctx->keep_device_records && last_stage == 3 && !summary;
  hs->d_hits.hint = ctx->keep_hint_hits;
  hs->d_bp.hint = ctx->keep_hint_bp;
  SearchWs &wsp = ws_of(ctx);
  Drainer drain(&hs->hits, &hs->bp, wsp.pin_hits, wsp.pin_bp);
  if (summary) drain.pairs = &hs->pairs;
  hs->drain = &drain;
  if (last_stage == 3 && !summary) {
    drain.hint_hits = ctx->host_hint_hits + ctx->host_hint_hits / 20;
    drain.hint_bp = ctx->host_hint_bp + ctx->host_hint_bp / 20;
  }
  int rc = drain.start();
  double wait_ms = 0;
  const SearchKnobs knobs = read_search_knobs();
  const int delta = db->hdr.min_accessible_length;
  PageSearch ps{ctx,
                wsp,
                qb,
                db->pages[(size_t)page],
                db->mem[(size_t)db->slot_of_page[(size_t)page]].view,
                static_cast<SearchConstMem *>(ctx->search_const)->view,
                ExtOpts{delta, opts->drop_out_wo_gap, opts->drop_out_w_gap, opts->min_helix_length},
                *opts,
                knobs,
                page,
                last_stage,
                mode,
                table,
                hs,
                0,
                0};
  if (opts->allowed_pairs) ps.allow = &allow;
  for (int32_t q = 0; q < nq; q++) ps.max_qlen = std::max(ps.max_qlen, qb->len[q]);
  for (int32_t L : ps.pg.seq_length) ps.max_dblen = std::max(ps.max_dblen, L);
  CandBatch next;
  int parity = 0;
  for (int32_t q0 = 0; q0 < nq && rc == PRB_OK;) {
    CandBatch cur;
    if (next.q1 > next.q0 && next.q0 == q0) {
      cur = next;
    } else {
      const auto tw0 = std::chrono::steady_clock::now();
      int32_t q1 = q0;
      take_queries(plan, q0, knobs.budget, true, &q1);
      wait_ms += std::chrono::duration<double, std::milli>(std::chrono::steady_clock::now() - tw0).count();
      if ((rc = convert_cands(ctx, plan, q0, q1, wsp.cand_pinned[parity], cur))) break;
    }
    next = CandBatch{};
    const int32_t q1 = cur.q1;
    std::function<void()> front_free = [&]() {
      if (!knobs.front_ahead || q1 >= nq || last_stage == 1 || !knobs.fused || knobs.row_shift < 0) return;
      int32_t q2 = q1;
      if (!take_queries(plan, q1, knobs.budget, false, &q2)) return;
      CandBatch nb;
      if (convert_cands(ctx, plan, q1, q2, wsp.cand_pinned[parity ^ 1], nb) != PRB_OK) return;
      next = nb;
      if (nb.ncand == 0 || nb.ncand > INT32_MAX) return;
      double pairs = 0;
      const int32_t c1 = chunk_end(nb.cd, (int32_t)nb.ncand, 0, knobs.chunk_pairs, &pairs);
      if (pairs >= 4.0e9) return;
      const int64_t cents = (c1 < nb.ncand ? nb.cd[c1].qoff : nb.nqent) - nb.cd[0].qoff;
      SearchWs::FrontStage &F = wsp.front;
      int64_t np = -1;
      if (issue_front(wsp, qb, ps.pd, delta, knobs.row_shift, nb.cd, c1, cents, F.stream, &np, ps.allow, nullptr) != PRB_OK || np < 0 ||
          hipEventRecord(F.done, F.stream) != hipSuccess) {
        (void)hipStreamSynchronize(F.stream);
        return;
      }
      F.ahead = true;
      F.cd = nb.cd;
      F.nc = c1;
      F.np = np;
    };
    {
      HostTimer ht(ctx, "host_search_range");
      rc = search_range(ps, cur, front_free);
      if (rc == PRB_ERR_NOMEM)
        set_error(std::string(prb_last_error()) + " - the hits of queries " + std::to_string(q0) + ".." + std::to_string(q1 - 1) +
                  " that pass -f against this page do not fit the device (lower PRB_GAPPED_CHUNK_HITS / PRB_SEARCH_CHUNK_PAIRS if it is "
                  "their working state; else build the database in smaller pages, db -c, which bounds the list per page)");
    }
    if (rc == PRB_OK && hipStreamSynchronize(ctx->stream) != hipSuccess) rc = PRB_ERR_HIP;
    q0 = q1;
    parity ^= 1;
    if (q0 < nq) {
      const double scale = 1.1 * (double)nq / (double)q0;
      drain.hint_hits = std::max(drain.hint_hits.load(), (size_t)((double)hs->counts[2] * scale));
      drain.hint_bp = std::max(drain.hint_bp.load(), (size_t)((double)hs->bp_ints_total * scale));
    }
  }
  if (wsp.front.stream && wsp.front.ahead) {
    (void)hipStreamSynchronize(wsp.front.stream);
    wsp.front.ahead = false;
  }
  plan.producer.join();
  {
    HostTimer ht(ctx, "host_drain_tail");
    const int drc = drain.finish();
    if (rc == PRB_OK) rc = drc;
    hs->drain = nullptr;
  }
  ctx->timers["host_dfs"].ms += plan.dfs_ms;
  ctx->timers["host_dfs"].launches++;
  ctx->timers["host_dfs_wait"].ms += wait_ms;
  ctx->timers["host_dfs_wait"].launches++;
  if (rc != PRB_OK) {
    delete hs;
    return rc;
  }
  if (hs->on_device) {
    ctx->keep_hint_hits = hs->d_hits.used;
    ctx->keep_hint_bp = hs->d_bp.used;
  }
  if (last_stage == 3 && !summary) {
    ctx->host_hint_hits = hs->hits.size();
    ctx->host_hint_bp = hs->bp.size();
  }
  *out = hs;
  return PRB_OK;
}

}

extern "C" {

int prb_search_page(prb_ctx *ctx, prb_qbatch *qb, prb_db *db, int32_t page, const prb_ris_opts *opts, int32_t last_stage,
                    prb_hitset **out) {
  return search_page(ctx, qb, db, page, opts, last_stage, SearchMode::kRecords, out);
}

static int select_callers_sites(const char *fn_name, prb_ctx *ctx, const prb_hit *hits, int64_t n, uint8_t *keep, prb::SiteRule rule) {
  const std::string fn = fn_name;
  if (!ctx || n < 0 || (n > 0 && (!hits || !keep))) {
    set_error(fn + ": bad argument");
    return PRB_ERR_ARG;
  }
  if (n == 0) return PRB_OK;
  if (n > INT32_MAX) {
    set_error(fn + ": more than 2^31 - 1 hits");
    return PRB_ERR_ARG;
  }
  if (rule == prb::SiteRule::kChain)
    for (int64_t i = 1; i < n; i++)
      if (hits[i].query == hits[i - 1].query && hits[i].db_id == hits[i - 1].db_id && hits[i].db_sp < hits[i - 1].db_sp) {
        set_error(fn + ": hit " + std::to_string(i) + " has a lower db_sp than the hit before it in its run of equal (query, db_id)");
        return PRB_ERR_ARG;
      }
  PRB_HIP(hipSetDevice(ctx->device));
  SearchWs &w = ws_of(ctx);
  const SearchKnobs knobs = read_search_knobs();
  int rc;
  if ((rc = w.hitsTmp.ensure(hits_bytes(n)))) return rc;
  try {
    std::vector<uint8_t> host(hits_bytes(n), 0);
    const HitSoA hh = carve_hits(host.data(), n);
    for (int64_t i = 0; i < n; i++) {
      hh.q_sp[i] = hits[i].q_sp;
      hh.db_sp[i] = hits[i].db_sp;
      hh.q_len[i] = hits[i].q_len;
      hh.db_len[i] = hits[i].db_len;
      hh.db_id[i] = hits[i].db_id;
      hh.query[i] = hits[i].query;
      hh.e_tot[i] = hits[i].e_tot;
    }
    PRB_HIP(hipMemcpyAsync(w.hitsTmp.p, host.data(), host.size(), hipMemcpyHostToDevice, ctx->stream));
    PRB_HIP(hipStreamSynchronize(ctx->stream));
  } catch (const std::exception &e) {
    set_error(fn + ": " + e.what());
    return PRB_ERR_NOMEM;
  }
  if ((rc = ctx->time_begin())) return rc;
  if ((rc = select_sites(ctx, w, carve_hits(w.hitsTmp, n), n, rule, knobs))) return rc;
  if ((rc = ctx->time_end(rule_timer(ctx, rule), 3))) return rc;
  PRB_HIP(hipMemcpyAsync(keep, w.keep.p, (size_t)n, hipMemcpyDeviceToHost, ctx->stream));
  PRB_HIP(hipStreamSynchronize(ctx->stream));
  return PRB_OK;
}
int prb_distinct_sites(prb_ctx *ctx, const prb_hit *hits, int64_t n, uint8_t *keep) {
  return select_callers_sites("prb_distinct_sites", ctx, hits, n, keep, prb::SiteRule::kDistinct);
}
int prb_chain_sites(prb_ctx *ctx, const prb_hit *hits, int64_t n, uint8_t *keep) {
  return select_callers_sites("prb_chain_sites", ctx, hits, n, keep, prb::SiteRule::kChain);
}

int prb_sort_filter(prb_ctx *ctx, const prb_hit *hits, int64_t n, double threshold, prb_hit *sorted, uint8_t *keep, int32_t *form) {
  if (!ctx || n < 0 || (n > 0 && (!hits || !sorted || !keep || !form))) {
    set_error("prb_sort_filter: bad argument");
    return PRB_ERR_ARG;
  }
  if (n == 0) return PRB_OK;
  if (n > INT32_MAX) {
    set_error("prb_sort_filter: more than 2^31 - 1 hits");
    return PRB_ERR_ARG;
  }
  const SearchKnobs knobs = read_search_knobs();
  SortBounds sb;
  int32_t qlo = INT32_MAX, qhi = 0, eq_len = 0;
  bool one_len = !knobs.sort_two_lengths;
  auto len16 = [](int32_t v) { return (int32_t)(uint16_t)v; };
  for (int64_t i = 0; i < n; i++) {
    const prb_hit &h = hits[i];
    const int64_t qend = (int64_t)h.q_sp + len16(h.q_len), dend = (int64_t)h.db_sp + len16(h.db_len);
    if (h.query < 0 || h.q_sp < 0 || h.db_sp < 0 || qend > INT32_MAX || dend > INT32_MAX) {
      set_error("prb_sort_filter: hit " + std::to_string(i) + " has a negative query or a coordinate outside 0 .. 2^31 - 1");
      return PRB_ERR_ARG;
    }
    qlo = std::min(qlo, h.query);
    qhi = std::max(qhi, h.query);
    sb.max_qlen = std::max(sb.max_qlen, (int32_t)qend);
    sb.max_dblen = std::max(sb.max_dblen, len16(h.db_len));
    sb.nchars = std::max(sb.nchars, (int32_t)dend);
    one_len = one_len && len16(h.q_len) == len16(h.db_len);
    eq_len = std::max(eq_len, len16(h.db_len));
  }
  sb.qmin = qlo;
  sb.qspan = qhi - qlo + 1;
  sb.eq_len_max = one_len ? eq_len : 0;
  PRB_HIP(hipSetDevice(ctx->device));
  SearchWs &w = ws_of(ctx);
  int rc;
  const size_t N = (size_t)n;
  if ((rc = w.hitsB.ensure(N * sizeof(HitRec))) || (rc = w.hitsC.ensure(hits_bytes(n))) || (rc = w.packed.ensure(N * sizeof(prb_hit))))
    return rc;
  try {
    std::vector<HitRec> host(N);
    for (int64_t i = 0; i < n; i++) {
      const prb_hit &h = hits[i];
      host[(size_t)i] = HitRec{h.q_sp, h.db_sp, h.q_len, h.db_len, h.db_id, h.db_id_start, h.query, 0, h.e_acc, h.e_hyb, h.e_tot, 0};
    }
    PRB_HIP(hipMemcpyAsync(w.hitsB.p, host.data(), N * sizeof(HitRec), hipMemcpyHostToDevice, ctx->stream));
    PRB_HIP(hipStreamSynchronize(ctx->stream));
  } catch (const std::exception &e) {
    set_error(std::string("prb_sort_filter: ") + e.what());
    return PRB_ERR_NOMEM;
  }
  const HitSoA S = carve_hits(w.hitsC, n);
  uint32_t *perm = nullptr;
  int64_t nsurv = 0;
  if ((rc = sort_hits(ctx, w, knobs, w.hitsB.as<HitRec>(), S, n, sb, &perm, form))) return rc;
  if ((rc = filter_hits(ctx, w, S, n, threshold, knobs.filter_tiles, &nsurv))) return rc;
  PRB_HIP(launch_pack_hits(S, n, nullptr, nullptr, -1, w.packed.p, ctx->stream));
  PRB_HIP(hipMemcpyAsync(sorted, w.packed.p, N * sizeof(prb_hit), hipMemcpyDeviceToHost, ctx->stream));
  PRB_HIP(hipMemcpyAsync(keep, w.keep.p, N, hipMemcpyDeviceToHost, ctx->stream));
  PRB_HIP(hipStreamSynchronize(ctx->stream));
  return PRB_OK;
}

int prb_search_page_summary(prb_ctx *ctx, prb_qbatch *qb, prb_db *db, int32_t page, const prb_ris_opts *opts, prb_pairset **out) {
  if (!out) {
    set_error("prb_search_page_summary: bad argument");
    return PRB_ERR_ARG;
  }
  *out = nullptr;
  prb_hitset *hs = nullptr;
  const int rc = search_page(ctx, qb, db, page, opts, 3, SearchMode::kSummary, &hs);
  if (rc != PRB_OK) return rc;
  auto *ps = new (std::nothrow) prb_pairset();
  if (!ps) {
    delete hs;
    set_error("prb_search_page_summary: out of host memory");
    return PRB_ERR_NOMEM;
  }
  ps->pairs.swap(hs->pairs);
  for (int i = 0; i < 3; i++) ps->counts[i] = hs->counts[i];
  delete hs;
  *out = ps;
  return PRB_OK;
}

int64_t prb_pairset_size(const prb_pairset *ps) { return ps ? (int64_t)ps->pairs.size() : -1; }
const prb_pair_summary *prb_pairset_pairs(const prb_pairset *ps) { return ps ? ps->pairs.data() : nullptr; }
void prb_pairset_counts(const prb_pairset *ps, int64_t counts[3]) {
  for (int i = 0; i < 3; i++) counts[i] = ps ? ps->counts[i] : 0;
}
void prb_pairset_free(prb_pairset *ps) { delete ps; }

int64_t prb_hitset_size(const prb_hitset *hs) { return !hs ? -1 : hs->ext_hits ? hs->ext_nhits : (int64_t)hs->hits.size(); }
const prb_hit *prb_hitset_hits(const prb_hitset *hs) { return !hs ? nullptr : hs->ext_hits ? hs->ext_hits : hs->hits.data(); }
const int32_t *prb_hitset_basepairs(const prb_hitset *hs, int64_t *count) {
  if (!hs) return nullptr;
  if (count) *count = (hs->ext_hits ? hs->ext_bp_ints : (int64_t)hs->bp.size()) / 2;
  return hs->ext_hits ? hs->ext_bp : hs->bp.data();
}
// ... 7 lines not shown
```

priblast_amd/csrc/search_host.hpp:

```cpp
#pragma once
#include <atomic>
#include <chrono>
#include <condition_variable>
#include <cstring>
#include <deque>
#include <memory>
#include <mutex>
#include <thread>

#include <rocprim/rocprim.hpp>

#include "../../include/priblast_hip.h"
#include "context.hpp"
#include "db_format.hpp"
#include "hitset.hpp"
#include "output.hpp"
#include "search_kernels.hpp"
#include "seed_dfs.hpp"

namespace prb {

struct SearchConstMem {
  DevBuf ints, bulge;
  SearchConst view{};
};

struct PageMem {
  DevBuf seqs, sa, sa_seq, blk_seq, start_pos, seq_length, acc, cond;
  PageDev view{};
};

#define PRB_SEARCH_BUFFERS(X)                                                                                                   \
  X(cands, 1) X(row_count, 1) X(row_off, 1) X(row_cand, 1) X(seed_qacc, 1)                                           \
  X(hitsA, 1) X(hitsB, 1) X(hitsC, 1) X(hitsTmp, 1)                                                              \
  X(kE, 1) X(kL, 1) X(kQ, 1) X(kP, 1) X(kTmp, 1) X(kTmp2, 1) X(idxA, 1) X(idxB, 1) X(sortTmp, 1)                      \
  X(endKey, 1) X(pmax, 1) X(state, 1) X(keep, 1) X(pending, 0) X(surv, 1) X(count, 0) X(scanTmp, 1)         \
  X(first, 1) X(cidx, 1)                                                                                                        \
  X(gapScratch, 1) X(overflow, 1) X(tierOf, 1) X(listA, 1) X(listB, 1) X(listC, 1) X(ntrace, 1) X(trace, 1)         \
  X(frontScratch, 1) X(accScratch, 0)                                                                                           \
  X(resumeSlot, 0) X(resumeCount, 0)                                                                                            \
  X(slowList, 1) X(slowSlot, 1) X(slowCnt, 1) X(slowTrace, 1)                                                                   \
  X(keptU, 1) X(keptFirst, 1) X(keptTier, 1) X(keptNtrace, 1) X(keptTrace, 1)                               \
  X(subset, 1) X(subset2, 1) X(tierFin, 1) X(ntraceFin, 1)                                                       \
  X(bpCount, 1) X(bpOff, 1) X(bpOff2, 1) X(bpOut, 1) X(bpEnds, 1)                                                               \
  X(packed, 0) X(pairHead, 1) X(pairStart, 1)

struct SearchWs {
#define X(name, trimmable) DevBuf name;
  PRB_SEARCH_BUFFERS(X)
#undef X
  DevBuf resumePool[kLdsTiers - 1];
  struct FrontStage {
    DevBuf cands, seed_qacc, pair0, keyA, keyB, valA, valB, sortTmp;
    PinnedBuf pair0_pin;
    hipStream_t stream = nullptr;
    hipEvent_t done = nullptr;
    bool ahead = false;
    const CandDev *cd = nullptr;
    int32_t nc = 0;
    int64_t np = 0;
    const uint64_t *vals = nullptr;
    DevBuf ballot, wcount, woff, scanTmp;
    PinnedBuf kept_pin;
    bool unsorted = false;
    int key_bits = 0;
    int64_t np_all = 0;
    int init() {
      if (stream) return PRB_OK;
      int lo = 0, hi = 0;
      (void)hipDeviceGetStreamPriorityRange(&lo, &hi);
      if (hipStreamCreateWithPriority(&stream, hipStreamNonBlocking, lo) != hipSuccess ||
          hipEventCreateWithFlags(&done, hipEventDisableTiming) != hipSuccess) {
        set_error("hipStreamCreateWithPriority / hipEventCreate failed (seed front stage)");
        return PRB_ERR_HIP;
      }
      return PRB_OK;
    }
    void release() {
      if (stream) {
        (void)hipStreamSynchronize(stream);
        (void)hipStreamDestroy(stream);
        (void)hipEventDestroy(done);
        stream = nullptr;
      }
      for (DevBuf *b : {&cands, &seed_qacc, &pair0, &keyA, &keyB, &valA, &valB, &sortTmp, &ballot, &wcount, &woff, &scanTmp}) b->release();
      pair0_pin.release();
      kept_pin.release();
      ahead = false;
    }
  } front;
  hipStream_t copy_stream = nullptr;
  hipEvent_t packed_ready = nullptr, copy_done = nullptr;
  bool copy_pending = false;
  int copy_init() {
    if (copy_stream) return PRB_OK;
    if (hipStreamCreateWithFlags(&copy_stream, hipStreamNonBlocking) != hipSuccess ||
        hipEventCreateWithFlags(&packed_ready, hipEventDisableTiming) != hipSuccess ||
        hipEventCreateWithFlags(&copy_done, hipEventDisableTiming) != hipSuccess) {
      set_error("hipStreamCreate / hipEventCreate failed (result copies)");
      return PRB_ERR_HIP;
    }
    return PRB_OK;
  }
  PinnedBuf pinned, cand_pinned[2], tb_pinned, pin_hits[2], pin_bp[2];
  bool trim_next = false;
  void trim() {
#define X(name, trimmable) \
  if (trimmable && name.cap > ((size_t)256 << 20)) name.release();
    PRB_SEARCH_BUFFERS(X)
#undef X
    for (DevBuf &b : resumePool)
      if (b.cap > ((size_t)256 << 20)) b.release();
    trim_next = false;
  }
  void release() {
#define X(name, trimmable) name.release();
    PRB_SEARCH_BUFFERS(X)
#undef X
    for (DevBuf &b : resumePool) b.release();
    front.release();
    if (copy_stream) {
      (void)hipStreamSynchronize(copy_stream);
      (void)hipStreamDestroy(copy_stream);
      (void)hipEventDestroy(packed_ready);
      (void)hipEventDestroy(copy_done);
      copy_stream = nullptr;
    }
    for (PinnedBuf *b : {&pinned, &cand_pinned[0], &cand_pinned[1], &tb_pinned, &pin_hits[0], &pin_hits[1], &pin_bp[0], &pin_bp[1]})
      b->release();
  }
};

inline SearchWs &ws_of(prb_ctx *ctx) {
  if (!ctx->search_ws) ctx->search_ws = new SearchWs();
  return *static_cast<SearchWs *>(ctx->search_ws);
}

struct Drainer {
  struct Job {
    int slot;
    int64_t nhits, nbp_ints;
  };
  std::vector<prb_hit> *hits;
  std::vector<int32_t> *bp;
  std::vector<prb_pair_summary> *pairs = nullptr;
  PinnedBuf *pin_hits, *pin_bp;
  hipEvent_t ev[2] = {nullptr, nullptr};
  std::thread th;
  std::mutex m;
  std::condition_variable cv;
  std::deque<Job> jobs;
  bool busy[2] = {false, false}, stop = false, failed = false;
  std::atomic<size_t> hint_hits{0}, hint_bp{0};

  Drainer(std::vector<prb_hit> *h, std::vector<int32_t> *b, PinnedBuf *ph, PinnedBuf *pb)
      : hits(h), bp(b), pin_hits(ph), pin_bp(pb) {}
  int start() {
    for (int i = 0; i < 2; i++)
      if (hipEventCreateWithFlags(&ev[i], hipEventDisableTiming) != hipSuccess) return PRB_ERR_HIP;
    th = std::thread([this] { run(); });
    return PRB_OK;
  }
  void run() {
    for (;;) {
      Job j;
      {
        std::unique_lock<std::mutex> lk(m);
        cv.wait(lk, [this] { return stop || !jobs.empty(); });
        if (jobs.empty()) return;
        j = jobs.front();
        jobs.pop_front();
      }
      if (hipEventSynchronize(ev[j.slot]) != hipSuccess) failed = true;
      if (pairs) {
        const prb_pair_summary *ps = static_cast<const prb_pair_summary *>(pin_hits[j.slot].p);
        pairs->insert(pairs->end(), ps, ps + j.nhits);
      } else {
        const prb_hit *src = static_cast<const prb_hit *>(pin_hits[j.slot].p);
        if (hits->capacity() < hits->size() + (size_t)j.nhits)
          hits->reserve(std::max({2 * hits->capacity(), hits->size() + (size_t)j.nhits, hint_hits.load()}));
        hits->insert(hits->end(), src, src + j.nhits);
        const int32_t *bsrc = static_cast<const int32_t *>(pin_bp[j.slot].p);
        if (bp->capacity() < bp->size() + (size_t)j.nbp_ints)
          bp->reserve(std::max({2 * bp->capacity(), bp->size() + (size_t)j.nbp_ints, hint_bp.load()}));
        bp->insert(bp->end(), bsrc, bsrc + j.nbp_ints);
      }
      {
        std::lock_guard<std::mutex> lk(m);
        busy[j.slot] = false;
      }
      cv.notify_all();
    }
  }
  void acquire(int slot) {
    std::unique_lock<std::mutex> lk(m);
    cv.wait(lk, [&] { return !busy[slot]; });
    busy[slot] = true;
  }
  void submit(const Job &j) {
    {
      std::lock_guard<std::mutex> lk(m);
      jobs.push_back(j);
    }
    cv.notify_all();
  }
  int finish() {
    {
      std::lock_guard<std::mutex> lk(m);
      stop = true;
    }
    cv.notify_all();
    if (th.joinable()) th.join();
    for (int i = 0; i < 2; i++)
      if (ev[i]) (void)hipEventDestroy(ev[i]);
    return failed ? PRB_ERR_HIP : PRB_OK;
  }
};

struct HostTimer {
  prb_ctx *ctx;
  const char *name;
  std::chrono::steady_clock::time_point t0 = std::chrono::steady_clock::now();
  HostTimer(prb_ctx *c, const char *n) : ctx(c), name(n) {}
  ~HostTimer() {
    auto &t = ctx->timers[name];
    t.ms += std::chrono::duration<double, std::milli>(std::chrono::steady_clock::now() - t0).count();
    t.launches++;
  }
};

struct ToI64 {
  __host__ __device__ int64_t operator()(const int32_t &v) const { return (int64_t)v; }
};
inline int bits_for(int64_t max_value) {
  int b = 1;
  while (b < 40 && (int64_t(1) << b) <= max_value) b++;
  return b;
}

template <class Call> int with_temp(DevBuf &tmp, const char *what, Call &&call) {
  size_t bytes = 0;
  if (hipError_t e = call(nullptr, bytes); e != hipSuccess) return hip_fail(e, what);
  if (int rc = tmp.ensure(bytes)) return rc;
  if (hipError_t e = call(tmp.p, bytes); e != hipSuccess) return hip_fail(e, what);
  return PRB_OK;
}

template <class K, class V>
int sort_pairs(hipStream_t s, DevBuf &tmp, const K *kin, K *kout, const V *vin, V *vout, size_t n, unsigned bits) {
  return with_temp(tmp, "rocprim::radix_sort_pairs",
                   [&](void *t, size_t &b) { return rocprim::radix_sort_pairs(t, b, kin, kout, vin, vout, n, 0, bits, s); });
}

inline int select_flagged(prb_ctx *ctx, SearchWs &w, const uint32_t *in, const uint8_t *flags, uint32_t *out, size_t n, int64_t *nsel) {
  int rc;
  if (in)
    rc = with_temp(w.scanTmp, "rocprim::select",
                   [&](void *t, size_t &b) { return rocprim::select(t, b, in, flags, out, w.count.as<size_t>(), n, ctx->stream); });
  else
    rc = with_temp(w.scanTmp, "rocprim::select", [&](void *t, size_t &b) {
      return rocprim::select(t, b, rocprim::counting_iterator<uint32_t>(0), flags, out, w.count.as<size_t>(), n, ctx->stream);
    });
  if (rc) return rc;
  size_t cnt = 0;
  PRB_HIP(hipMemcpyAsync(&cnt, w.count.p, sizeof(size_t), hipMemcpyDeviceToHost, ctx->stream));
  PRB_HIP(hipStreamSynchronize(ctx->stream));
  *nsel = (int64_t)cnt;
  return PRB_OK;
}

}

struct prb_db {
  prb_ctx *ctx = nullptr;
  prb::DbHeader hdr;
  std::vector<prb::DbPage> pages;
  std::vector<prb::PageMem> mem;
  std::vector<int> slot_of_page, page_in_slot;
  std::vector<uint64_t> slot_used;
  std::vector<hipEvent_t> slot_ready;
  uint64_t clock = 0;
  hipStream_t copy_stream = nullptr;
  bool pinned = false;
  int64_t uploads = 0;
  std::vector<prb::SeqTable> tabs;
};

namespace prb {
struct SeedPlan {
  const prb_db *db = nullptr;
  int32_t page = 0, nq = 0, max_seed_length = 0;
  double hybrid_threshold = 0;
  std::vector<std::vector<SeedCandidate>> per_q;
  std::vector<double> qpairs;
  std::vector<int64_t> qrows, qents;
  std::unique_ptr<std::atomic<int>[]> done;
  std::atomic<int32_t> next_query{0};
  std::thread producer;
  double dfs_ms = 0;
  ~SeedPlan() {
    if (producer.joinable()) producer.join();
  }
  void wait_for(int32_t q) const {
    while (!done[q].load(std::memory_order_acquire)) std::this_thread::sleep_for(std::chrono::microseconds(50));
  }
};
}

struct prb_qbatch {
  prb_ctx *ctx = nullptr;
  int32_t nq = 0, repeat_flag = 0;
  std::vector<int64_t> off;
  std::vector<int32_t> len, len_unmasked;
  std::vector<char> seqs;
  std::vector<uint8_t> enc;
  std::vector<int32_t> sa;
  prb::DevBuf d_enc, d_sa, d_acc, d_cond, d_off, d_len;
  bool have_acc = false;
  int32_t W = 0, delta = 0;
  prb::QBatchDev view{};
  std::unique_ptr<prb::SeedPlan> plan;
};

struct prb_pairmask {
  prb_ctx *ctx = nullptr;
  const prb_qbatch *qb = nullptr;
  const prb_db *db = nullptr;
  int32_t nq = 0;
  std::vector<int64_t> tbase;
  int64_t row_words = 0;
  std::vector<uint32_t> bits;
  int64_t count = 0;
  bool used = false;
  std::mutex first_use;
  prb::DevBuf dev;
  ~prb_pairmask() {
    if (dev.p) (void)hipSetDevice(ctx->device);
    dev.release();
  }
};

namespace prb {
int use_pairmask(const char *fn, prb_ctx *ctx, const prb_qbatch *qb, const prb_db *db, int32_t page, const prb_pairmask *pm, AllowDev *view);

struct TableState {
  prb_ctx *ctx = nullptr;
  const prb_db *db = nullptr;
  bool broken = false;
  bool finished = false;
  int32_t distinct = -1;
  int32_t chain = -1;
  int64_t counts[3] = {0, 0, 0};
  DevBuf table;
};

struct MergeTable : TableState {
  const prb_qbatch *qb = nullptr;
  int32_t nq = 0;
  std::vector<int32_t> qlen;
  std::vector<uint8_t> merged;
};

struct RunTable : TableState {
  std::vector<int64_t> tbase;
  std::vector<std::vector<uint64_t>> merged;
  DevBuf ids;
  int64_t targets() const { return tbase.empty() ? 0 : tbase.back(); }
  bool has(size_t page, int32_t id) const {
    const std::vector<uint64_t> &m = merged[page];
    return ((size_t)id >> 6) < m.size() && (m[(size_t)id >> 6] >> (id & 63) & 1);
  }
  void set(size_t page, int32_t id) {
    std::vector<uint64_t> &m = merged[page];
    if (((size_t)id >> 6) >= m.size()) m.resize(((size_t)id >> 6) + 1, 0);
    m[(size_t)id >> 6] |= 1ull << (id & 63);
  }
};

struct SpanBufs {
  DevBuf keyA, keyB, valA, valB, span, scan, sortTmp;
  void release() {
    for (DevBuf *b : {&keyA, &keyB, &valA, &valB, &span, &scan, &sortTmp}) b->release();
  }
};

template <class Slot> struct TopTable : MergeTable {
  int32_t n = 0;
  size_t slots_bytes() const { return (size_t)nq * (size_t)n * sizeof(Slot); }
  size_t bytes() const { return slots_bytes() + (size_t)nq * sizeof(int32_t); }
  int32_t *fill() const { return reinterpret_cast<int32_t *>(table.template as<char>() + slots_bytes()); }
};
}

struct prb_topset : prb::TopTable<prb_top_pair> {
  std::vector<prb_top_pair> pairs;
  ~prb_topset() {
    if (table.p) (void)hipSetDevice(ctx->device);
    table.release();
  }
};

struct prb_tophits : prb::TopTable<prb_top_hit> {
  int32_t style = -1;
  prb::DevBuf pool, pool2;
// ... 175 lines not shown
```

priblast_amd/csrc/search_kernels.hpp:

```cpp
#pragma once
#include <hip/hip_runtime.h>

#include <cstdint>

namespace prb {

struct SearchTab {
  static constexpr int kStack = 0;
  static constexpr int kInternal = kStack + 49;
  static constexpr int kMismatchI = kInternal + 31;
  static constexpr int kInt11 = kMismatchI + 175;
  static constexpr int kInt21 = kInt11 + 1600;
  static constexpr int kInt22 = kInt21 + 8000;
  static constexpr int kDangle5 = kInt22 + 40000;
  static constexpr int kDangle3 = kDangle5 + 40;
  static constexpr int kBulge = kDangle3 + 40;
  static constexpr int kTau = kBulge + 31;
  static constexpr int kZero = kTau + 8;
  static constexpr int kCount = kZero + 1;
};

struct SearchConst {
  const int32_t *tab;
  const int32_t *stack37;
  const int32_t *internal37;
  const int32_t *mismatchI37;
  const int32_t *int11;
  const int32_t *int21;
  const int32_t *int22;
  const int32_t *dangle5;
  const int32_t *dangle3;
  const double *bulge;
  int32_t terminal_au;
  uint64_t bp_rows;
  uint32_t pair_mask, wobble_mask;
  unsigned char bp_pair[25];
};

struct PageDev {
  const uint8_t *seqs;
  const int32_t *sa;
  const int32_t *sa_seq;
  const int32_t *blk_seq;
  const int32_t *start_pos;
  const int32_t *seq_length;
  const float *acc;
  const float *cond;
  int32_t nchars, nseq;
};

struct QBatchDev {
  const uint8_t *enc;
  const int32_t *sa;
  const float *acc;
  const float *cond;
  const int64_t *off;
  const int32_t *len;
  int32_t nq;
};

struct CandDev {
  int32_t sp_q, ep_q, sp_db, ep_db, length, query;
  double score;
  int64_t row0;
  int64_t qoff;
};

struct AllowDev {
  const uint32_t *bits;
  int64_t row_words, tbase;
};
__host__ __device__ inline bool pair_allowed(const AllowDev &a, int query, int db_id) {
  const int64_t t = a.tbase + db_id;
  return (a.bits[(int64_t)query * a.row_words + (t >> 5)] >> (t & 31)) & 1u;
}

struct HitSoA {
  int32_t *q_sp, *db_sp, *q_len, *db_len, *db_id, *db_id_start, *query;
  double *e_acc, *e_hyb, *e_tot;
};
constexpr int kHitInts = 7, kHitDoubles = 3;
constexpr size_t kHitBytes = kHitInts * 4 + kHitDoubles * 8;

struct ExtOpts {
  int32_t delta;
  int32_t drop_wo_gap;
  int32_t drop_w_gap;
  int32_t min_helix;
};

struct alignas(16) HitRec {
  int32_t q_sp, db_sp, q_len, db_len, db_id, db_id_start, query, pad0;
  double e_acc, e_hyb, e_tot;
  int64_t pad1;
};
static_assert(sizeof(HitRec) == 64, "one cache line half, two per 128-byte line");

hipError_t launch_sa_seq(const PageDev &pg, int32_t *sa_seq, hipStream_t s);
hipError_t launch_seed_qacc(const CandDev *cands, int32_t ncand, int64_t nq_entries, const QBatchDev &qb, int delta, double *qacc,
                            hipStream_t s);
hipError_t launch_row_keys(const CandDev *cands, int32_t ncand, int64_t nrows, const PageDev &pg, int qmin, int shift, int dbits,
                           bool wide, int32_t *row_cand, void *key, uint32_t *val, hipStream_t s);
hipError_t launch_seed_count(const CandDev *cands, int32_t ncand, int64_t nrows, const QBatchDev &qb, const PageDev &pg,
                             int delta, const double *qacc, int32_t *row_count, int32_t *row_cand, const uint32_t *row_perm,
                             hipStream_t s);
hipError_t launch_seed_emit(const CandDev *cands, int32_t ncand, int64_t nrows, const QBatchDev &qb, const PageDev &pg,
                            int delta, const double *qacc, const int32_t *row_cand, const int64_t *row_off, HitSoA hits,
                            const uint32_t *row_perm, hipStream_t s);
hipError_t launch_seed_count_allowed(const CandDev *cands, int32_t ncand, int64_t nrows, const QBatchDev &qb, const PageDev &pg,
                                     int delta, const double *qacc, int32_t *row_count, int32_t *row_cand, const uint32_t *row_perm,
                                     const AllowDev &allow, hipStream_t s);
hipError_t launch_seed_emit_allowed(const CandDev *cands, int32_t ncand, int64_t nrows, const QBatchDev &qb, const PageDev &pg,
                                    int delta, const double *qacc, const int32_t *row_cand, const int64_t *row_off, HitSoA hits,
                                    const uint32_t *row_perm, const AllowDev &allow, hipStream_t s);

hipError_t launch_ungapped(HitSoA hits, int64_t n, const QBatchDev &qb, const PageDev &pg, const SearchConst &sc,
                           ExtOpts o, int max_query_len, hipStream_t s);
inline int64_t blk_seq_entries(int64_t nchars) { return (nchars >> 5) + 1; }
hipError_t launch_blk_seq(const PageDev &pg, int32_t *blk_seq, hipStream_t s);
constexpr int64_t kMaxFusedCands = 1 << 20, kMaxFusedEntries = 1 << 12;
hipError_t launch_pair_keys(const CandDev *cands, const int64_t *pair0, int32_t ncand, int64_t npairs, const PageDev &pg, int qmin,
                            int shift, int dbits, bool wide, void *key, uint64_t *val, hipStream_t s);
inline int64_t allow_words(int64_t npairs) { return (npairs + 63) / 64; }
hipError_t launch_allow_test(const CandDev *cands, const int64_t *pair0, const uint64_t *val, int64_t npairs, const PageDev &pg,
                             const AllowDev &allow, uint64_t *ballot, int32_t *count, hipStream_t s);
hipError_t launch_allow_scatter(const void *key_in, const uint64_t *val_in, int64_t npairs, bool wide, const uint64_t *ballot,
                                const int64_t *off, void *key_out, uint64_t *val_out, hipStream_t s);
constexpr int kFusePairs = 2048, kSliceRecBytes = 48;
inline int64_t fused_slices(int64_t npairs) { return (npairs + kFusePairs - 1) / kFusePairs; }
hipError_t launch_seed_extend(const CandDev *cands, const uint64_t *vals, int64_t npairs, const QBatchDev &qb, const PageDev &pg,
                              const SearchConst &sc, ExtOpts o, const double *qacc, double thr, int max_query_len, void *slices,
                              int32_t *slice_count, uint64_t *nseed, hipStream_t s);
hipError_t launch_collect_slices(const void *slices, const int32_t *slice_count, const int64_t *slice_off, int64_t nslices, HitRec *out,
                                 hipStream_t s);

struct PackedKeyInfo {
  int32_t qmin, lmax;
  int32_t bl, bq, bd;
  int32_t one_len = 0;
};
hipError_t launch_make_packed_keys(const HitSoA &hits, int64_t n, const PackedKeyInfo &f, uint64_t *key, uint64_t *k_energy,
                                   uint32_t *idx, hipStream_t s);
hipError_t launch_make_packed_keys_recs(const HitRec *hits, int64_t n, const PackedKeyInfo &f, uint64_t *key, uint64_t *k_energy,
                                        uint32_t *idx, hipStream_t s);
hipError_t launch_fix_ties(const uint64_t *key_sorted, const uint64_t *e_sorted, const uint32_t *perm, int64_t n, const HitRec *recs,
                           uint32_t *perm_out, int32_t *too_long, hipStream_t s);
hipError_t launch_make_keys(const HitSoA &hits, int64_t n, uint64_t *k_energy, uint32_t *k_len, uint32_t *k_qsp,
                            uint64_t *k_pos, uint32_t *idx, hipStream_t s);
hipError_t launch_order_keys(const double *v, int64_t n, uint64_t *key, hipStream_t s);
hipError_t launch_gather_u64(const uint64_t *src, const uint32_t *idx, uint64_t *dst, int64_t n, hipStream_t s);
hipError_t launch_gather_u32(const uint32_t *src, const uint32_t *idx, uint32_t *dst, int64_t n, hipStream_t s);
hipError_t launch_gather_u8(const uint8_t *src, const uint32_t *idx, uint8_t *dst, int64_t n, hipStream_t s);
hipError_t launch_iota_u32(uint32_t *dst, int64_t n, hipStream_t s);
hipError_t launch_gather_rows(const void *src, const uint32_t *idx, void *dst, int64_t n, int row_bytes, hipStream_t s);
hipError_t launch_gather_hits(const HitSoA &src, const uint32_t *idx, HitSoA dst, int64_t n, hipStream_t s);
hipError_t launch_gather_hits_to_recs(const HitSoA &src, const uint32_t *idx, HitRec *dst, int64_t n, hipStream_t s);
hipError_t launch_gather_recs_to_hits(const HitRec *src, const uint32_t *idx, HitSoA dst, int64_t n, hipStream_t s);
hipError_t launch_flag_marked(const uint8_t *marks, const uint32_t *list, int64_t n, uint8_t mask, uint8_t *flags, hipStream_t s);
hipError_t launch_flag_not_above(const double *e_tot, int64_t n, double thr, uint8_t *keep, hipStream_t s);
hipError_t launch_mark_first(const int32_t *query, int64_t n, uint8_t *first, hipStream_t s);
hipError_t launch_pack_hits(const HitSoA &src, int64_t n, const int32_t *bp_count, const int64_t *bp_off, int64_t bp_base,
                            void *out, hipStream_t s);

hipError_t launch_filter_init(const HitSoA &h, int64_t n, double thr, int64_t *db_end_key, uint8_t *state, hipStream_t s);
hipError_t launch_filter_round(const HitSoA &h, int64_t n, const int64_t *pmax, uint8_t *state, int32_t *pending, bool tiles,
                               hipStream_t s);
hipError_t launch_filter_final(const HitSoA &h, int64_t n, const int64_t *pmax, const uint8_t *state, uint8_t *keep, bool tiles,
                               hipStream_t s);

constexpr size_t kGapWaveLdsBytes = 64 * 1024;
struct GapScratch {
  uint8_t *base;
  size_t bytes_per_wave;
  int32_t cap_rec, cap_diag;
  int32_t nwaves;
};
size_t gapped_wave_scratch_bytes(int cap_diag, int cap_rec);
struct GapResume {
  int32_t *slot = nullptr;
  uint8_t *pool = nullptr;
  uint32_t *count = nullptr;
  int32_t cap = 0;
};
size_t gapped_resume_bytes(int tier);
constexpr int kLdsTiers = 4, kWaveTier = 4;
struct GapTierKnobs {
  bool pair = true;
  bool pool = true;
  bool pad_set = false, period_set = false, early_set = false;
  int pad[kLdsTiers] = {};
  int period[kLdsTiers] = {};
  int early[kLdsTiers] = {};
};
constexpr int kTraceCap = 32;
constexpr int kLongTraceTier = 5;
struct LongTrace {
  uint32_t *trace = nullptr;
  int32_t *count = nullptr;
  const int32_t *slot = nullptr;
  int32_t cap = 0;
};
constexpr uint8_t kResumeMark = 0x40, kHandoverMark = 0x80, kMarkTier = 0x07;
__host__ __device__ inline bool is_resumed(uint8_t t) { return (t & (kResumeMark | kHandoverMark)) != 0; }
struct GapArgs {
  HitSoA in{}, out{};
  int64_t n = 0;
  const uint32_t *subset = nullptr;
  QBatchDev qb{};
  PageDev pg{};
  SearchConst sc{};
  ExtOpts o{};
  uint8_t *overflow = nullptr;
  uint8_t *tier_out = nullptr;
  int tier_id = 0;
  const uint8_t *first_flag = nullptr;
  int32_t *bp_count = nullptr;
  uint16_t *trace = nullptr;
  const int64_t *bp_off = nullptr;
  int32_t *bp_out = nullptr;
  unsigned long long *next_work = nullptr;
  GapResume rin{}, rout{};
  LongTrace lt{};
  double *acc_scratch = nullptr;
  int period = 0;
  int early = 0;
  int pool = 1;
  int handover = 0;
};
hipError_t launch_gapped_lds(const GapArgs &a, int mode, int tier, const GapTierKnobs &knobs, hipStream_t s);
size_t gapped_acc_scratch_bytes();
hipError_t launch_gapped_wave(const GapArgs &a, GapScratch scratch, int mode, hipStream_t s);

constexpr int kFrontMaxDrop = 16;
bool gapped_front_supported(const SearchConst &sc, const ExtOpts &o);
size_t gapped_front_scratch_bytes();
hipError_t launch_gapped_front(const GapArgs &a, void *scratch, bool second_only, hipStream_t s);

hipError_t launch_assign_slots(const uint32_t *list, int64_t n, int32_t base, int32_t *slot, hipStream_t s);
hipError_t launch_bp_count(const HitSoA &in, int64_t n, const uint32_t *subset, const QBatchDev &qb, const PageDev &pg,
                           const SearchConst &sc, const int32_t *ntrace, int32_t *bp_count, hipStream_t s);
hipError_t launch_bp_expand(const HitSoA &in, int64_t n, const uint32_t *subset, const QBatchDev &qb, const PageDev &pg,
                            const SearchConst &sc, const uint8_t *first_flag, const int32_t *ntrace, const uint8_t *tier_of,
                            const uint16_t *trace, const LongTrace &lt, const int64_t *bp_off, int32_t *bp_out, hipStream_t s);
hipError_t launch_bp_ends(const int64_t *bp_off, int64_t n, const int32_t *bp, int32_t *ends, hipStream_t s);

hipError_t launch_pair_heads(const int32_t *query, const int32_t *db_id, int64_t n, uint8_t *head, hipStream_t s);
hipError_t launch_pair_fold(const HitSoA &h, int64_t n, const uint32_t *start, int64_t npairs, const int32_t *ends, void *out,
                            hipStream_t s);
constexpr int kSiteLdsHits = 2048;
constexpr int kSiteLongGrid = 1024;
inline int64_t site_long_runs_max(int64_t n) { return n / 2 + 1; }
struct SiteScratch {
  uint32_t *long_list;
  uint32_t *nlong;
  int32_t *lo, *hi;
  uint8_t *state;
};
hipError_t launch_site_select(const HitSoA &h, int64_t n, const uint8_t *head, int lds_hits, const SiteScratch &w, uint8_t *keep,
                              hipStream_t s);
constexpr int kChainLdsHits = 1536;
struct ChainScratch {
  uint32_t *long_list;
  uint32_t *nlong;
  double *score;
  int32_t *prev;
};
hipError_t launch_chain_select(const HitSoA &h, int64_t n, const uint8_t *head, int lds_hits, const ChainScratch &w, uint8_t *keep,
                               hipStream_t s);

constexpr int kTopMaxN = 1024;
hipError_t launch_top_merge(const void *rec, int64_t nrec, int32_t q0, int32_t q1, int32_t page, int32_t n, void *tab, int32_t *fill,
                            hipStream_t s);
hipError_t launch_tophits_merge(const void *rec, int64_t nrec, int32_t q0, int32_t q1, int32_t page, int32_t n, void *tab, int32_t *fill,
                                hipStream_t s);
hipError_t launch_tophits_counts(const void *tab, const int32_t *fill, int32_t n, int64_t nslots, int32_t *cnt, hipStream_t s);
hipError_t launch_tophits_gather(void *tab, const int32_t *fill, int32_t n, int64_t nslots, const int64_t *off, int64_t split,
                                 const int32_t *old_pool, const int32_t *fresh, int32_t *pool, hipStream_t s);
hipError_t launch_top_join(void *tab, int32_t *fill, const void *src, const int32_t *src_fill, int32_t nq, int32_t n, hipStream_t s);
hipError_t launch_tophits_join(void *tab, int32_t *fill, const void *src, const int32_t *src_fill, int32_t nq, int32_t n, int64_t shift,
                               hipStream_t s);

struct alignas(16) TargetKey {
  uint64_t e;
  uint32_t id, at;
};
// ... 93 lines not shown
```

priblast_amd/csrc/search_stages.hpp:

```cpp
#pragma once
#include <functional>

#include "search_host.hpp"

namespace prb {

struct SearchKnobs {
  double budget;
  double chunk_pairs;
  int row_shift;
  bool fused;
  bool front_ahead;
  bool sort_four_keys, sort_two_lengths;
  size_t big_list_bytes;
  int64_t gapped_chunk_hits;
  int first_tier;
  bool wave_hbm, no_resume, front_paired, front, handover;
  GapTierKnobs tiers;
  bool filter_tiles;
  int resume_cap;
  int skip_tiers;
  bool trace_no_long, trace_no_slots;
  int trace_long_cap, trace_slot_cap;
  int distinct_lds_hits;
  int chain_lds_hits;
  bool debug_rows, debug_mem;
};

struct SortBounds {
  int32_t qmin = 0, qspan = 1, max_qlen = 0, max_dblen = 0, nchars = 0;
  int32_t eq_len_max = 0;
};

struct PageSearch {
  prb_ctx *ctx;
  SearchWs &w;
  const prb_qbatch *qb;
  const DbPage &pg;
  const PageDev &pd;
  const SearchConst &sc;
  const ExtOpts eo;
  const prb_ris_opts &opts;
  const SearchKnobs &k;
  const int page, last_stage;
  const SearchMode mode;
  TableState *table;
  prb_hitset *hs;
  int max_qlen;
  int32_t max_dblen;
  const AllowDev *allow = nullptr;
};

struct CandBatch {
  int32_t q0 = 0, q1 = 0;
  CandDev *cd = nullptr;
  int64_t ncand = 0, nrows = 0, nqent = 0;
};

struct SubSearch : PageSearch {
  const CandBatch &b;
  const std::function<void()> &front_free;
  bool front_called = false;
  int32_t ncand = 0;
  SortBounds sb;
  int64_t nf = 0, one_pass_maxlen = 0;
  bool all_one_pass = true;
  int64_t nung = 0;
  HitSoA U, G;
  const uint8_t *first = nullptr;
  int64_t nch = 0;
  bool chunked = false;
  int64_t nmax = 0;
  int64_t ngap = 0;
  LongTrace lt{};
  int32_t lt_used = 0;
  const uint8_t *tier_all = nullptr;
  const int32_t *ntrace_all = nullptr;
  const uint16_t *trace_all = nullptr;
  HitSoA F;
  int64_t nfin = 0;
  int64_t bp_total = 0;
};

inline void call_front_free(SubSearch &s) {
  if (s.front_free && !s.front_called) {
    s.front_free();
    s.front_called = true;
  }
}

HitSoA carve_hits(uint8_t *p, int64_t n);
inline HitSoA carve_hits(DevBuf &b, int64_t n) { return carve_hits(b.as<uint8_t>(), n); }
inline size_t hits_bytes(int64_t n) { return (((size_t)n + 1) & ~(size_t)1) * kHitBytes + 64; }
inline HitSoA offset_hits(const HitSoA &h, int64_t first) {
  return HitSoA{h.q_sp + first, h.db_sp + first, h.q_len + first, h.db_len + first, h.db_id + first, h.db_id_start + first,
                h.query + first, h.e_acc + first, h.e_hyb + first, h.e_tot + first};
}
int grow_keep(prb_ctx *ctx, DevBuf &buf, size_t have, size_t need, size_t spare_limit = SIZE_MAX);
int compact_below(prb_ctx *ctx, SearchWs &w, const HitSoA &in, int64_t n, double thr, DevBuf &idxbuf, DevBuf &recbuf, int64_t *m,
                  int64_t have = 0);

int gapped_stage(SubSearch &s);
int retrace_tier(SubSearch &s, int tier, const uint32_t *subset2, const int64_t *bpOff2, int64_t m);

}
```

priblast_amd/csrc/ungapped_kernels.hip:

```cpp
#include <algorithm>

#include "launch.hpp"
#include "search_device.hpp"
#include "search_kernels.hpp"

namespace prb {

namespace {

struct UngappedTabs {
  const int32_t *stack37, *internal37, *mismatchI37, *int11;
  const int32_t *int22;
};
constexpr int kUtStack = 0, kUtInternal = 49, kUtMismatch = 49 + 31, kUtInt11 = 49 + 31 + 175, kUtTotal = 49 + 31 + 175 + 1600;

__device__ __forceinline__ double loop_energy_ungapped_abcd(const SearchConst &sc, const UngappedTabs &t, int type, int type2,
                                                           int u, int a, int b, int c, int d) {
  int z;
  if (u == 0) z = t.stack37[type * 7 + type2];
  else if (u == 1) z = t.int11[((type * 8 + type2) * 5 + a) * 5 + b];
  else if (u == 2) z = t.int22[((((type * 8 + type2) * 5 + a) * 5 + c) * 5 + d) * 5 + b];
  else z = t.internal37[2 * u] + t.mismatchI37[(type * 5 + a) * 5 + b] + t.mismatchI37[(type2 * 5 + d) * 5 + c];
  return div100(sc, z);
}
// ... 81 lines not shown
            min_e = e;
            min_a = a;
            min_h = hy;
            min_p = i;
            min_q = j;
          }
          p = i;
          tp = rtype_of(type);
        }
        bq = nq;
        bd = nd;
        if (min_p - i >= drop) done = true;
      }
    }
  }
  e = min_e;
  a = min_a;
  hy = min_h;
  int k = q_sp0 + len0 - 1, r = k, l = db_sp0 + len0 - 1, min_r = r;
  {
    int bq = base_of(qv.enc(k)), bd = base_of(ds[l]);
    int tr = bp_type(sc, bq, bd);
    int cq = 0, cd = 0;
    float acc_prev = pg.acc[base + id_start];
    bool done = false;
    while (!done) {
      unsigned dcs[kUngappedAhead];
      float dan[kUngappedAhead], dcn[kUngappedAhead];
#pragma unroll
      for (int s = 0; s < kUngappedAhead; s++) {
        const int ll = l + 1 + s;
        dcs[s] = ll < pg.nchars ? ds[ll] : 0u;
        int64_t ai = base + id_start - 1 - s;
        ai = ai > 0 ? ai : 0;
        int64_t ci = ai + delta;
        ci = ci < nacc ? ci : nacc - 1;
        dan[s] = pg.acc[ai];
        dcn[s] = pg.cond[ci];
      }
#pragma unroll
      for (int s = 0; s < kUngappedAhead; s++) {
        if (done) continue;
        k++;
        l++;
        id_start--;
        const unsigned qc = qv.enc(k), dc = dcs[s];
        if (qc < 2 || dc < 2) {
          done = true;
          continue;
        }
        const float acc_i = dan[s];
        const double ta = qv.cond(k) + acc_i - acc_prev + dcn[s];
        acc_prev = acc_i;
        e += ta;
        a += ta;
        const int nq = base_of(qc), nd = base_of(dc);
        if (k == r + 1) {
          cq = nq;
          cd = nd;
        }
        const int type2 = rtype_of(bp_type(sc, nq, nd));
        if (type2 != 0) {
          const double le = loop_energy_ungapped_abcd(sc, tabs, tr, type2, k - r - 1, cq, cd, bq, bd);
          e += le;
          hy += le;
          if (e < min_e) {
            min_e = e;
            min_a = a;
            min_h = hy;
            min_r = k;
            min_id_start = id_start;
          }
          r = k;
          tr = rtype_of(type2);
        }
        bq = nq;
        bd = nd;
        if (k - min_r >= drop) done = true;
      }
    }
  }
  w.id_start = min_id_start;
  w.q_sp = min_p;
  w.db_sp = min_q;
  w.len = min_r - min_p + 1;
  w.e_tot = min_e;
  w.e_acc = min_a;
  w.e_hyb = min_h;
}
template <class Q>
__device__ __forceinline__ void ungapped_walk(const Q &qv, const UngappedTabs &tabs, HitSoA &h, int64_t x, const PageDev &pg,
                                              const SearchConst &sc, const ExtOpts &o) {
  WalkHit w{h.q_sp[x], h.db_sp[x], h.q_len[x], h.db_id[x], h.db_id_start[x], h.e_acc[x], h.e_hyb[x], h.e_tot[x]};
  ungapped_walk_reg<8>(qv, tabs, w, pg, sc, o);
  h.db_id_start[x] = w.id_start;
  h.q_sp[x] = w.q_sp;
  h.db_sp[x] = w.db_sp;
  h.q_len[x] = w.len;
  h.db_len[x] = w.len;
  h.e_tot[x] = w.e_tot;
  h.e_acc[x] = w.e_acc;
  h.e_hyb[x] = w.e_hyb;
}

constexpr int kUngappedPer = 8;
__global__ __launch_bounds__(kBlock) void k_ungapped(HitSoA h, int64_t n, QBatchDev qb, PageDev pg, SearchConst sc, ExtOpts o,
                                                     int qcap) {
  extern __shared__ __align__(16) uint8_t ungapped_smem[];
  __shared__ int32_t s_tab[kUtTotal];
  const int64_t b0 = (int64_t)blockIdx.x * (kBlock * kUngappedPer);
  if (b0 >= n) return;
  const int64_t b1 = (b0 + kBlock * kUngappedPer < n ? b0 + kBlock * kUngappedPer : n) - 1;
  for (int t = threadIdx.x; t < kUtTotal; t += kBlock)
    s_tab[t] = t < kUtInternal   ? sc.stack37[t]
               : t < kUtMismatch ? sc.internal37[t - kUtInternal]
               : t < kUtInt11    ? sc.mismatchI37[t - kUtMismatch]
                                 : sc.int11[t - kUtInt11];
  const UngappedTabs tabs{s_tab + kUtStack, s_tab + kUtInternal, s_tab + kUtMismatch, s_tab + kUtInt11, sc.int22};
  const int q0 = h.query[b0];
  const int nslots = qb.len[q0] + 1;
  const bool staged = q0 == h.query[b1] && nslots <= qcap;
  if (staged) {
    float *s_acc = reinterpret_cast<float *>(ungapped_smem), *s_cond = s_acc + qcap;
    uint8_t *s_enc = reinterpret_cast<uint8_t *>(s_cond + qcap);
    const int64_t qo = qb.off[q0];
    for (int t = threadIdx.x; t < nslots; t += kBlock) {
      s_acc[t] = qb.acc[qo + t];
      s_cond[t] = qb.cond[qo + t];
      s_enc[t] = qb.enc[qo + t];
    }
    __syncthreads();
    const QueryLds qv{s_enc, s_acc, s_cond};
    for (int64_t x = b0 + threadIdx.x; x <= b1; x += kBlock) ungapped_walk(qv, tabs, h, x, pg, sc, o);
  } else {
    __syncthreads();
    for (int64_t x = b0 + threadIdx.x; x <= b1; x += kBlock) {
      const int64_t qo = qb.off[h.query[x]];
      const QueryGlobal qv{qb.enc + qo, qb.acc + qo, qb.cond + qo};
      ungapped_walk(qv, tabs, h, x, pg, sc, o);
    }
  }
}

constexpr int kPairCandBits = 20, kPairEntBits = 12;
static_assert(kMaxFusedCands == (1 << kPairCandBits) && kMaxFusedEntries == (1 << kPairEntBits) && kPairCandBits + kPairEntBits == 32,
              "the value of a pair");
constexpr int kSeqBlkShift = 5;

__global__ __launch_bounds__(kBlock) void k_blk_seq(PageDev pg, int32_t *blk_seq, int64_t nblk) {
  const int64_t b = (int64_t)blockIdx.x * kBlock + threadIdx.x;
  if (b < nblk) blk_seq[b] = seq_of(pg, (int)(b << kSeqBlkShift));
}

template <class Key>
__global__ __launch_bounds__(kBlock) void k_pair_key(const CandDev *__restrict__ cands, const int64_t *__restrict__ pair0, int ncand,
                                                     int64_t npairs, PageDev pg, int qmin, int shift, int dbits,
                                                     Key *__restrict__ key, uint64_t *__restrict__ val) {
  __shared__ int64_t s_p0[kBlock + 1];
  __shared__ int s_c0;
  const int64_t p = (int64_t)blockIdx.x * kBlock + threadIdx.x;
  if (threadIdx.x == 0) {
    const int64_t first = (int64_t)blockIdx.x * kBlock;
    int lo = 0, hi = ncand - 1;
    while (lo < hi) {
      const int m = (lo + hi + 1) >> 1;
      if (pair0[m] <= first) lo = m;
      else hi = m - 1;
    }
    s_c0 = lo;
  }
  __syncthreads();
  const int c0 = s_c0;
  for (int t = threadIdx.x; t <= kBlock; t += kBlock) s_p0[t] = c0 + t < ncand ? pair0[c0 + t] : INT64_MAX;
  __syncthreads();
  if (p >= npairs) return;
  int lo = 0, hi = kBlock;
  while (lo < hi) {
    const int m = (lo + hi + 1) >> 1;
    if (s_p0[m] <= p) lo = m;
    else hi = m - 1;
  }
  const int ci = c0 + lo;
  const CandDev c = cands[ci];
  const uint32_t pl = (uint32_t)(p - s_p0[lo]), qw = (uint32_t)(c.ep_q - c.sp_q + 1);
  const uint32_t rowl = pl / qw, jrel = pl - rowl * qw;
  const uint32_t db_sp = (uint32_t)pg.sa[c.sp_db + (int)rowl];
  key[p] = ((Key)(uint32_t)(c.query - qmin) << dbits) | (Key)(db_sp >> shift);
  val[p] = (uint64_t)db_sp | ((uint64_t)(uint32_t)ci << 32) | ((uint64_t)jrel << (32 + kPairCandBits));
}

__device__ __forceinline__ int pair_cand(uint64_t v) { return (int)((v >> 32) & ((1u << kPairCandBits) - 1)); }

__global__ __launch_bounds__(kBlock) void k_allow_test(const CandDev *__restrict__ cands, const int64_t *__restrict__ pair0,
                                                       const uint64_t *__restrict__ val, int64_t npairs, PageDev pg, AllowDev allow,
                                                       uint64_t *__restrict__ ballot, int32_t *__restrict__ count) {
  const int64_t p = (int64_t)blockIdx.x * kBlock + threadIdx.x;
  bool ok = false;
  if (p < npairs) {
    const int ci = pair_cand(val[p]);
    const CandDev c = cands[ci];
    const uint32_t pl = (uint32_t)(p - pair0[ci]), qw = (uint32_t)(c.ep_q - c.sp_q + 1);
    ok = pair_allowed(allow, c.query, pg.sa_seq[c.sp_db + (int)(pl / qw)]);
  }
  const unsigned long long m = __ballot(ok);
  if ((threadIdx.x & 63) == 0 && p < npairs) {
    ballot[p >> 6] = m;
    count[p >> 6] = __popcll(m);
  }
}
template <class Key>
__global__ __launch_bounds__(kBlock) void k_allow_scatter(const Key *__restrict__ key_in, const uint64_t *__restrict__ val_in, int64_t npairs,
                                                          const uint64_t *__restrict__ ballot, const int64_t *__restrict__ off,
                                                          Key *__restrict__ key_out, uint64_t *__restrict__ val_out) {
  const int64_t p = (int64_t)blockIdx.x * kBlock + threadIdx.x;
  if (p >= npairs) return;
  const uint64_t m = ballot[p >> 6];
  const int lane = (int)(p & 63);
  if (!(m >> lane & 1)) return;
  const int64_t at = off[p >> 6] + __popcll(m & ((1ull << lane) - 1));
  key_out[at] = key_in[p];
  val_out[at] = val_in[p];
}

struct alignas(16) SliceRec {
  int32_t q_sp, db_sp, len, db_id, db_id_start, query;
  double e_acc, e_hyb, e_tot;
};
static_assert(sizeof(SliceRec) == kSliceRecBytes, "three 16-byte stores");

struct FuseArgs {
  const CandDev *cands;
  const uint64_t *vals;
  int64_t npairs;
  const double *qacc;
  double thr;
  SliceRec *slices;
  int32_t *slice_count;
  unsigned long long *nseed;
  int qcap;
};

constexpr int kFusePer = kFusePairs / kBlock;
static_assert(kFusePer * kBlock == kFusePairs, "pairs per workgroup");
template <int kAhead>
__global__ __launch_bounds__(kBlock) void k_seed_extend(FuseArgs f, QBatchDev qb, PageDev pg, SearchConst sc, ExtOpts o) {
  extern __shared__ __align__(16) uint8_t ungapped_smem[];
  __shared__ int32_t s_tab[kUtTotal];
  __shared__ unsigned s_kept, s_seeds, s_maxlen;
  const int64_t b0 = (int64_t)blockIdx.x * kFusePairs;
  if (b0 >= f.npairs) return;
  const int64_t b1 = (b0 + kFusePairs < f.npairs ? b0 + kFusePairs : f.npairs) - 1;
  if (threadIdx.x == 0) {
    s_kept = 0;
    s_seeds = 0;
    s_maxlen = 0;
  }
  for (int t = threadIdx.x; t < kUtTotal; t += kBlock)
    s_tab[t] = t < kUtInternal   ? sc.stack37[t]
               : t < kUtMismatch ? sc.internal37[t - kUtInternal]
               : t < kUtInt11    ? sc.mismatchI37[t - kUtMismatch]
                                 : sc.int11[t - kUtInt11];
  const UngappedTabs tabs{s_tab + kUtStack, s_tab + kUtInternal, s_tab + kUtMismatch, s_tab + kUtInt11, sc.int22};
  const int q0 = f.cands[pair_cand(f.vals[b0])].query;
  const int nslots = qb.len[q0] + 1;
  const bool staged = q0 == f.cands[pair_cand(f.vals[b1])].query && nslots <= f.qcap;
  float *s_acc = reinterpret_cast<float *>(ungapped_smem), *s_cond = s_acc + f.qcap;
  uint8_t *s_enc = reinterpret_cast<uint8_t *>(s_cond + f.qcap);
  if (staged) {
    const int64_t qo = qb.off[q0];
    for (int t = threadIdx.x; t < nslots; t += kBlock) {
      s_acc[t] = qb.acc[qo + t];
      s_cond[t] = qb.cond[qo + t];
      s_enc[t] = qb.enc[qo + t];
    }
  }
  __syncthreads();
  const int lane = threadIdx.x & 63;
  SliceRec *slice = f.slices + b0;
  unsigned nseed = 0, maxlen = 0;
  for (int it = 0; it < kFusePer; it++) {
    const int64_t x = b0 + (int64_t)it * kBlock + threadIdx.x;
    bool keep = false;
    WalkHit w{};
    int query = 0;
    if (x <= b1) {
      const uint64_t v = f.vals[x];
      const int db_sp = (int)(uint32_t)v, jrel = (int)(v >> (32 + kPairCandBits));
      const CandDev c = f.cands[pair_cand(v)];
      int id = pg.blk_seq[db_sp >> kSeqBlkShift];
      while (id + 1 < pg.nseq && pg.start_pos[id + 1] <= db_sp) id++;
      const int sp0 = pg.start_pos[id];
      const int st = pg.seq_length[id] - (db_sp - sp0) - c.length;
      const int64_t base = (int64_t)sp0 - id;
      const double dba = window_acc(pg.acc + base, pg.cond + base, st, c.length, o.delta);
      const double qa = f.qacc[c.qoff + jrel];
      const double ie = qa + dba + c.score;
      if (ie < 0) {
        nseed++;
        const int64_t qo = qb.off[c.query];
        const double ea = qa + dba;
        w = WalkHit{qb.sa[qo + c.sp_q + jrel], db_sp, c.length, id, st, ea, c.score, ea + c.score};
        query = c.query;
        if (staged) {
          const QueryLds qv{s_enc, s_acc, s_cond};
          ungapped_walk_reg<kAhead>(qv, tabs, w, pg, sc, o);
        } else {
          const QueryGlobal qv{qb.enc + qo, qb.acc + qo, qb.cond + qo};
          ungapped_walk_reg<kAhead>(qv, tabs, w, pg, sc, o);
        }
        keep = !(w.e_tot > f.thr);
      }
    }
    const unsigned long long mask = __ballot(keep);
    if (mask) {
      const int leader = __ffsll((long long)mask) - 1;
      unsigned basepos = 0;
      if (lane == leader) basepos = atomicAdd(&s_kept, (unsigned)__popcll(mask));
      basepos = (unsigned)__shfl((int)basepos, leader);
      if (keep) {
        SliceRec r;
        r.q_sp = w.q_sp;
        r.db_sp = w.db_sp;
        r.len = w.len;
        r.db_id = w.id;
        r.db_id_start = w.id_start;
        r.query = query;
        r.e_acc = w.e_acc;
        r.e_hyb = w.e_hyb;
        r.e_tot = w.e_tot;
        slice[basepos + (unsigned)__popcll(mask & ((1ull << lane) - 1))] = r;
        maxlen = (unsigned)w.len > maxlen ? (unsigned)w.len : maxlen;
      }
    }
  }
  for (int d = 32; d > 0; d >>= 1) {
    nseed += (unsigned)__shfl_down((int)nseed, d);
    const unsigned o = (unsigned)__shfl_down((int)maxlen, d);
    maxlen = o > maxlen ? o : maxlen;
  }
  if (lane == 0 && nseed) atomicAdd(&s_seeds, nseed);
  if (lane == 0 && maxlen) atomicMax(&s_maxlen, maxlen);
  __syncthreads();
  if (threadIdx.x == 0) {
    f.slice_count[blockIdx.x] = (int32_t)s_kept;
    if (s_seeds) atomicAdd(f.nseed, (unsigned long long)s_seeds);
    if (s_maxlen) atomicMax(f.nseed + 1, (unsigned long long)s_maxlen);
  }
}

__global__ __launch_bounds__(kBlock) void k_collect_slices(const SliceRec *__restrict__ slices, const int32_t *__restrict__ count,
                                                           const int64_t *__restrict__ off, HitRec *__restrict__ out) {
  const int n = count[blockIdx.x];
  const SliceRec *src = slices + (int64_t)blockIdx.x * kFusePairs;
  HitRec *dst = out + off[blockIdx.x];
  for (int t = threadIdx.x; t < n; t += kBlock) {
    const SliceRec a = src[t];
    HitRec r;
    r.q_sp = a.q_sp;
    r.db_sp = a.db_sp;
    r.q_len = a.len;
    r.db_len = a.len;
    r.db_id = a.db_id;
    r.db_id_start = a.db_id_start;
    r.query = a.query;
    r.pad0 = 0;
    r.e_acc = a.e_acc;
    r.e_hyb = a.e_hyb;
    r.e_tot = a.e_tot;
    r.pad1 = 0;
    dst[t] = r;
  }
}

inline int query_lds_slots(int max_query_len) { return std::min((max_query_len + 1 + 3) & ~3, 7168); }

}

hipError_t launch_ungapped(HitSoA hits, int64_t n, const QBatchDev &qb, const PageDev &pg, const SearchConst &sc, ExtOpts o,
                           int max_query_len, hipStream_t s) {
  if (n <= 0) return hipSuccess;
  const int qcap = query_lds_slots(max_query_len);
  const int64_t per_block = (int64_t)kBlock * kUngappedPer;
  hipLaunchKernelGGL(k_ungapped, dim3((unsigned)((n + per_block - 1) / per_block)), dim3(kBlock), (size_t)qcap * 9, s, hits, n,
                     qb, pg, sc, o, qcap);
  return hipGetLastError();
}
hipError_t launch_blk_seq(const PageDev &pg, int32_t *blk_seq, hipStream_t s) {
  const int64_t nblk = blk_seq_entries(pg.nchars);
  hipLaunchKernelGGL(k_blk_seq, dim3((unsigned)((nblk + kBlock - 1) / kBlock)), dim3(kBlock), 0, s, pg, blk_seq, nblk);
  return hipGetLastError();
}
hipError_t launch_pair_keys(const CandDev *cands, const int64_t *pair0, int32_t ncand, int64_t npairs, const PageDev &pg, int qmin,
                            int shift, int dbits, bool wide, void *key, uint64_t *val, hipStream_t s) {
  if (wide)
    return launch_1d(k_pair_key<uint64_t>, npairs, kBlock, 0, s, cands, pair0, ncand, npairs, pg, qmin, shift, dbits, (uint64_t *)key, val);
  return launch_1d(k_pair_key<uint32_t>, npairs, kBlock, 0, s, cands, pair0, ncand, npairs, pg, qmin, shift, dbits, (uint32_t *)key, val);
}
hipError_t launch_allow_test(const CandDev *cands, const int64_t *pair0, const uint64_t *val, int64_t npairs, const PageDev &pg,
                             const AllowDev &allow, uint64_t *ballot, int32_t *count, hipStream_t s) {
  return launch_1d(k_allow_test, npairs, kBlock, 0, s, cands, pair0, val, npairs, pg, allow, ballot, count);
}
hipError_t launch_allow_scatter(const void *key_in, const uint64_t *val_in, int64_t npairs, bool wide, const uint64_t *ballot,
                                const int64_t *off, void *key_out, uint64_t *val_out, hipStream_t s) {
  if (wide)
    return launch_1d(k_allow_scatter<uint64_t>, npairs, kBlock, 0, s, (const uint64_t *)key_in, val_in, npairs, ballot, off, (uint64_t *)key_out,
                     val_out);
  return launch_1d(k_allow_scatter<uint32_t>, npairs, kBlock, 0, s, (const uint32_t *)key_in, val_in, npairs, ballot, off, (uint32_t *)key_out,
                   val_out);
}
hipError_t launch_seed_extend(const CandDev *cands, const uint64_t *vals, int64_t npairs, const QBatchDev &qb, const PageDev &pg,
                              const SearchConst &sc, ExtOpts o, const double *qacc, double thr, int max_query_len, void *slices,
                              int32_t *slice_count, uint64_t *nseed, hipStream_t s) {
  if (npairs <= 0) return hipSuccess;
  const int qcap = query_lds_slots(max_query_len);
  FuseArgs f{cands, vals, npairs, qacc, thr, static_cast<SliceRec *>(slices), slice_count, reinterpret_cast<unsigned long long *>(nseed),
             qcap};
  hipLaunchKernelGGL(k_seed_extend<8>, dim3((unsigned)fused_slices(npairs)), dim3(kBlock), (size_t)qcap * 9, s, f, qb, pg, sc, o);
  return hipGetLastError();
}
hipError_t launch_collect_slices(const void *slices, const int32_t *slice_count, const int64_t *slice_off, int64_t nslices, HitRec *out,
                                 hipStream_t s) {
  if (nslices <= 0) return hipSuccess;
  hipLaunchKernelGGL(k_collect_slices, dim3((unsigned)nslices), dim3(kBlock), 0, s, static_cast<const SliceRec *>(slices), slice_count,
                     slice_off, out);
  return hipGetLastError();
}

}
```

Before: 7.681.

## Pack seed pairs into narrow 32-bit keys with partial radix sort and in-tile reordering

```diff
diff --git a/include/priblast_hip.h b/include/priblast_hip.h
--- a/include/priblast_hip.h
+++ b/include/priblast_hip.h
@@ -59,6 +59,8 @@
 int prb_cpu_budget(void);
 int prb_host_threads_default(void);
 void prb_ris_opts_default(prb_ris_opts *o);
+int prb_seed_pair_layout(int64_t nchars, int64_t query_span, int32_t row_shift, int32_t sort_bits, int32_t local_order,
+                         int32_t pair_wide, int32_t out[6]);
 
 int prb_ctx_create(int device, const char *param_file, prb_ctx **out);
 void prb_ctx_destroy(prb_ctx *ctx);
diff --git a/priblast_amd/capi.py b/priblast_amd/capi.py
--- a/priblast_amd/capi.py
+++ b/priblast_amd/capi.py
@@ -71,6 +71,7 @@
     "prb_version": (ctypes.c_char_p, []),
     "prb_cpu_budget": (ctypes.c_int, []),
     "prb_host_threads_default": (ctypes.c_int, []),
+    "prb_seed_pair_layout": (ctypes.c_int, [c_i64, c_i64, c_i32, c_i32, c_i32, c_i32, P(c_i32)]),
     "prb_ris_opts_default": (None, [P(RisOpts)]),
     "prb_ctx_create": (ctypes.c_int, [ctypes.c_int, ctypes.c_char_p, P(ctypes.c_void_p)]),
     "prb_ctx_destroy": (None, [ctypes.c_void_p]),
@@ -266,6 +267,12 @@
     return res.decode("latin-1") if isinstance(seq, str) else res
 
 
+def seed_pair_layout(nchars, query_span, row_shift=7, sort_bits=16, local_order=True, pair_wide=False):
+    out = (c_i32 * 6)()
+    _check(lib().prb_seed_pair_layout(nchars, query_span, row_shift, sort_bits, int(local_order), int(pair_wide), out))
+    return dict(narrow=bool(out[0]), pbits=out[1], kbits=out[2], begin=out[3], local_bits=out[4], wide_key=bool(out[5]))
+
+
 def default_opts(**kw):
     o = RisOpts()
     lib().prb_ris_opts_default(ctypes.byref(o))
diff --git a/priblast_amd/csrc/capi_search.hip b/priblast_amd/csrc/capi_search.hip
--- a/priblast_amd/csrc/capi_search.hip
+++ b/priblast_amd/csrc/capi_search.hip
@@ -21,6 +21,11 @@
   if ((e = getenv("PRB_SEARCH_CHUNK_PAIRS"))) k.chunk_pairs = atof(e);
   e = getenv("PRB_SEED_ROW_SHIFT");
   k.row_shift = e ? std::min(atoi(e), 30) : 7;
+  e = getenv("PRB_SEED_SORT_BITS");
+  k.sort_bits = e ? std::max(atoi(e), 1) : 16;
+  k.local_order = !env_off(getenv("PRB_SEED_LOCAL_ORDER"));
+  e = getenv("PRB_SEED_PAIR_WIDE");
+  k.pair_wide = e && atoi(e) != 0;
   k.fused = !env_off(getenv("PRB_SEED_FUSED"));
   k.front_ahead = !getenv("PRB_NO_FRONT_AHEAD");
   k.sort_four_keys = getenv("PRB_SORT_FOUR_KEYS") != nullptr;
@@ -272,6 +277,7 @@
 
 struct RowKeyBits {
   int dbits, kbits;
+  int begin = 0;
   bool wide() const { return kbits > 32; }
 };
 static RowKeyBits row_key_bits(const PageDev &pd, int row_shift, const CandDev *cd, int32_t nc) {
@@ -280,8 +286,13 @@
 }
 template <class V>
 static int sort_by_row_key(hipStream_t s, DevBuf &tmp, const RowKeyBits &kb, DevBuf &kin, DevBuf &kout, const V *vin, V *vout, size_t n) {
-  return kb.wide() ? sort_pairs(s, tmp, kin.as<uint64_t>(), kout.as<uint64_t>(), vin, vout, n, (unsigned)kb.kbits)
-                   : sort_pairs(s, tmp, kin.as<uint32_t>(), kout.as<uint32_t>(), vin, vout, n, (unsigned)kb.kbits);
+  return kb.wide() ? sort_pairs(s, tmp, kin.as<uint64_t>(), kout.as<uint64_t>(), vin, vout, n, (unsigned)kb.begin, (unsigned)kb.kbits)
+                   : sort_pairs(s, tmp, kin.as<uint32_t>(), kout.as<uint32_t>(), vin, vout, n, (unsigned)kb.begin, (unsigned)kb.kbits);
+}
+static int sort_chunk_pairs(hipStream_t s, DevBuf &tmp, const PairLayout &lay, DevBuf &kin, DevBuf &kout, DevBuf &vin, DevBuf &vout, size_t n) {
+  const RowKeyBits kb{lay.pbits, lay.kbits, lay.begin};
+  return lay.narrow ? sort_by_row_key(s, tmp, kb, kin, kout, vin.as<uint32_t>(), vout.as<uint32_t>(), n)
+                    : sort_by_row_key(s, tmp, kb, kin, kout, vin.as<uint64_t>(), vout.as<uint64_t>(), n);
 }
 
 static int scan_row_counts(prb_ctx *ctx, SearchWs &w, int64_t n) {
@@ -291,7 +302,7 @@
   });
 }
 
-static int issue_front(SearchWs &w, const prb_qbatch *qb, const PageDev &pd, int delta, int row_shift, const CandDev *cd, int32_t nc,
+static int issue_front(SearchWs &w, const prb_qbatch *qb, const PageDev &pd, int delta, const SearchKnobs &k, const CandDev *cd, int32_t nc,
                        int64_t cents, hipStream_t s, int64_t *np_out, const AllowDev *allow, prb_ctx *timed) {
   SearchWs::FrontStage &F = w.front;
   int rc;
@@ -307,19 +318,20 @@
   }
   pair0[nc] = np;
   const size_t NP = (size_t)np;
-  const RowKeyBits kb = row_key_bits(pd, row_shift, cd, nc);
+  const PairLayout lay = pair_layout(pd.nchars, (int64_t)cd[nc - 1].query - cd[0].query, k.row_shift, k.sort_bits, k.local_order, k.pair_wide);
   if ((rc = F.cands.ensure((size_t)nc * sizeof(CandDev))) || (rc = F.seed_qacc.ensure((size_t)std::max<int64_t>(cents, 1) * 8)) ||
-      (rc = F.pair0.ensure(((size_t)nc + 1) * 8)) || (rc = F.keyA.ensure(NP * (kb.wide() ? 8 : 4))) ||
-      (rc = F.keyB.ensure(NP * (kb.wide() ? 8 : 4))) || (rc = F.valA.ensure(NP * 8)) || (rc = F.valB.ensure(NP * 8)))
+      (rc = F.pair0.ensure(((size_t)nc + 1) * 8)) || (rc = F.keyA.ensure(NP * lay.key_bytes())) || (rc = F.keyB.ensure(NP * lay.key_bytes())) ||
+      (rc = F.valA.ensure(NP * lay.val_bytes())) || (rc = F.valB.ensure(NP * lay.val_bytes())))
     return rc;
   PRB_HIP(hipMemcpyAsync(F.cands.p, cd, (size_t)nc * sizeof(CandDev), hipMemcpyHostToDevice, s));
   PRB_HIP(hipMemcpyAsync(F.pair0.p, pair0, ((size_t)nc + 1) * 8, hipMemcpyHostToDevice, s));
   PRB_HIP(launch_seed_qacc(F.cands.as<CandDev>(), nc, cents, qb->view, delta, F.seed_qacc.as<double>(), s));
-  PRB_HIP(launch_pair_keys(F.cands.as<CandDev>(), F.pair0.as<int64_t>(), nc, np, pd, cd[0].query, row_shift, kb.dbits, kb.wide(), F.keyA.p,
-                           F.valA.as<uint64_t>(), s));
+  PRB_HIP(launch_pair_keys(F.cands.as<CandDev>(), F.pair0.as<int64_t>(), nc, np, pd, cd[0].query, lay, F.keyA.p, F.valA.p, s));
   F.unsorted = false;
   F.np_all = np;
-  F.vals = F.valB.as<uint64_t>();
+  F.lay = lay;
+  F.keys = F.keyB.p;
+  F.vals = F.valB.p;
   if (allow) {
     const int64_t nw = allow_words(np);
     if ((rc = F.ballot.ensure((size_t)nw * 8)) || (rc = F.wcount.ensure((size_t)(nw + 1) * 4)) || (rc = F.woff.ensure((size_t)(nw + 1) * 8)) ||
@@ -327,23 +339,21 @@
       return rc;
     if (timed && ((rc = timed->time_end("seed", 1)) || (rc = timed->time_begin()))) return rc;
     PRB_HIP(hipMemsetAsync(F.wcount.as<int32_t>() + nw, 0, 4, s));
-    PRB_HIP(launch_allow_test(F.cands.as<CandDev>(), F.pair0.as<int64_t>(), F.valA.as<uint64_t>(), np, pd, *allow, F.ballot.as<uint64_t>(),
+    PRB_HIP(launch_allow_test(F.cands.as<CandDev>(), F.pair0.as<int64_t>(), F.valA.p, lay, np, pd, *allow, F.ballot.as<uint64_t>(),
                               F.wcount.as<int32_t>(), s));
     auto counts = rocprim::make_transform_iterator(F.wcount.as<int32_t>(), ToI64());
     if ((rc = with_temp(F.scanTmp, "rocprim::exclusive_scan", [&](void *t, size_t &b) {
            return rocprim::exclusive_scan(t, b, counts, F.woff.as<int64_t>(), (int64_t)0, (size_t)nw + 1, rocprim::plus<int64_t>(), s);
          })))
       return rc;
-    PRB_HIP(launch_allow_scatter(F.keyA.p, F.valA.as<uint64_t>(), np, kb.wide(), F.ballot.as<uint64_t>(), F.woff.as<int64_t>(), F.keyB.p,
-                                 F.valB.as<uint64_t>(), s));
+    PRB_HIP(launch_allow_scatter(F.keyA.p, F.valA.p, np, lay, F.ballot.as<uint64_t>(), F.woff.as<int64_t>(), F.keyB.p, F.valB.p, s));
     PRB_HIP(hipMemcpyAsync(F.kept_pin.p, F.woff.as<int64_t>() + nw, 8, hipMemcpyDeviceToHost, s));
     if (timed && ((rc = timed->time_end(timed->allow_timer, 3)) || (rc = timed->time_begin()))) return rc;
     F.unsorted = true;
-    F.key_bits = kb.kbits;
     *np_out = np;
     return PRB_OK;
   }
-  if ((rc = sort_by_row_key(s, F.sortTmp, kb, F.keyA, F.keyB, F.valA.as<uint64_t>(), F.valB.as<uint64_t>(), NP))) return rc;
+  if ((rc = sort_chunk_pairs(s, F.sortTmp, lay, F.keyA, F.keyB, F.valA, F.valB, NP))) return rc;
   *np_out = np;
   return PRB_OK;
 }
@@ -361,10 +371,9 @@
   if (k.debug_rows) fprintf(stderr, "[allow] cands %d pairs %lld allowed %lld\n", nc, (long long)F.np_all, (long long)kept);
   *np = kept;
   if (kept == 0) return PRB_OK;
-  if ((rc = sort_by_row_key(ctx->stream, F.sortTmp, RowKeyBits{0, F.key_bits}, F.keyB, F.keyA, F.valB.as<uint64_t>(), F.valA.as<uint64_t>(),
-                            (size_t)kept)))
-    return rc;
-  F.vals = F.valA.as<uint64_t>();
+  if ((rc = sort_chunk_pairs(ctx->stream, F.sortTmp, F.lay, F.keyB, F.keyA, F.valB, F.valA, (size_t)kept))) return rc;
+  F.keys = F.keyA.p;
+  F.vals = F.valA.p;
   return PRB_OK;
 }
 
@@ -397,7 +406,7 @@
     return rc;
   PRB_HIP(hipMemsetAsync(w.count.p, 0, 16, ctx->stream));
   PRB_HIP(hipMemsetAsync(w.row_count.as<int32_t>() + nsl, 0, 4, ctx->stream));
-  PRB_HIP(launch_seed_extend(F.cands.as<CandDev>(), F.vals, np, s.qb->view, s.pd, s.sc, s.eo, F.seed_qacc.as<double>(),
+  PRB_HIP(launch_seed_extend(F.cands.as<CandDev>(), F.keys, F.vals, F.lay, np, s.qb->view, s.pd, s.sc, s.eo, F.seed_qacc.as<double>(),
                              s.opts.interaction_threshold, s.max_qlen, w.hitsA.p, w.row_count.as<int32_t>(), w.count.as<uint64_t>(),
                              ctx->stream));
   if ((rc = scan_row_counts(ctx, w, nsl))) return rc;
@@ -511,7 +520,7 @@
         PRB_HIP(hipStreamWaitEvent(s.ctx->stream, F.done, 0));
       } else {
         if (F.ahead) PRB_HIP(hipStreamSynchronize(F.stream));
-        if ((rc = issue_front(w, s.qb, s.pd, s.eo.delta, s.k.row_shift, cd + c0, c.nc, c.cents, s.ctx->stream, &np, s.allow, s.ctx))) return rc;
+        if ((rc = issue_front(w, s.qb, s.pd, s.eo.delta, s.k, cd + c0, c.nc, c.cents, s.ctx->stream, &np, s.allow, s.ctx))) return rc;
       }
       F.ahead = false;
       if (np >= 0 && F.unsorted) {
@@ -1163,7 +1172,7 @@
       const int64_t cents = (c1 < nb.ncand ? nb.cd[c1].qoff : nb.nqent) - nb.cd[0].qoff;
       SearchWs::FrontStage &F = wsp.front;
       int64_t np = -1;
-      if (issue_front(wsp, qb, ps.pd, delta, knobs.row_shift, nb.cd, c1, cents, F.stream, &np, ps.allow, nullptr) != PRB_OK || np < 0 ||
+      if (issue_front(wsp, qb, ps.pd, delta, knobs, nb.cd, c1, cents, F.stream, &np, ps.allow, nullptr) != PRB_OK || np < 0 ||
           hipEventRecord(F.done, F.stream) != hipSuccess) {
         (void)hipStreamSynchronize(F.stream);
         return;
@@ -1230,6 +1239,18 @@
   return search_page(ctx, qb, db, page, opts, last_stage, SearchMode::kRecords, out);
 }
 
+int prb_seed_pair_layout(int64_t nchars, int64_t query_span, int32_t row_shift, int32_t sort_bits, int32_t local_order, int32_t pair_wide,
+                         int32_t out[6]) {
+  if (!out || nchars < 1 || query_span < 0) {
+    set_error("prb_seed_pair_layout: bad argument");
+    return PRB_ERR_ARG;
+  }
+  const PairLayout L = pair_layout(nchars, query_span, std::min(row_shift, 30), std::max(sort_bits, 1), local_order != 0, pair_wide != 0);
+  const int32_t v[6] = {L.narrow, L.pbits, L.kbits, L.begin, L.local_bits, L.wide_key()};
+  std::copy(v, v + 6, out);
+  return PRB_OK;
+}
+
 static int select_callers_sites(const char *fn_name, prb_ctx *ctx, const prb_hit *hits, int64_t n, uint8_t *keep, prb::SiteRule rule) {
   const std::string fn = fn_name;
   if (!ctx || n < 0 || (n > 0 && (!hits || !keep))) {
diff --git a/priblast_amd/csrc/search_host.hpp b/priblast_amd/csrc/search_host.hpp
--- a/priblast_amd/csrc/search_host.hpp
+++ b/priblast_amd/csrc/search_host.hpp
@@ -59,11 +59,11 @@
     const CandDev *cd = nullptr;
     int32_t nc = 0;
     int64_t np = 0;
-    const uint64_t *vals = nullptr;
+    PairLayout lay;
+    const void *keys = nullptr, *vals = nullptr;
     DevBuf ballot, wcount, woff, scanTmp;
     PinnedBuf kept_pin;
     bool unsorted = false;
-    int key_bits = 0;
     int64_t np_all = 0;
     int init() {
       if (stream) return PRB_OK;
@@ -247,9 +247,33 @@
 }
 
 template <class K, class V>
+int sort_pairs(hipStream_t s, DevBuf &tmp, const K *kin, K *kout, const V *vin, V *vout, size_t n, unsigned begin, unsigned end) {
+  return with_temp(tmp, "rocprim::radix_sort_pairs",
+                   [&](void *t, size_t &b) { return rocprim::radix_sort_pairs(t, b, kin, kout, vin, vout, n, begin, end, s); });
+}
+template <class K, class V>
 int sort_pairs(hipStream_t s, DevBuf &tmp, const K *kin, K *kout, const V *vin, V *vout, size_t n, unsigned bits) {
-  return with_temp(tmp, "rocprim::radix_sort_pairs",
-                   [&](void *t, size_t &b) { return rocprim::radix_sort_pairs(t, b, kin, kout, vin, vout, n, 0, bits, s); });
+  return sort_pairs(s, tmp, kin, kout, vin, vout, n, 0u, bits);
+}
+
+inline PairLayout pair_layout(int64_t nchars, int64_t qspan, int row_shift, int sort_bits, bool local_order, bool force_wide) {
+  PairLayout L;
+  if (row_shift < 0) return L;
+  const int qbits = bits_for(std::max<int64_t>(1, qspan)), pbits = bits_for(std::max<int64_t>(1, nchars - 1));
+  if (!force_wide && pbits + qbits <= 32) {
+    L.narrow = true;
+    L.pbits = pbits;
+    L.kbits = pbits + qbits;
+    const int shift = std::min(row_shift, pbits);
+    L.begin = shift;
+    if (local_order) L.begin = std::min(std::max(shift, L.kbits - std::max(sort_bits, 1)), shift + kPairLocalBits);
+    L.local_bits = L.begin - shift;
+    return L;
+  }
+  L.shift = row_shift;
+  L.pbits = bits_for(std::max<int64_t>(1, (nchars - 1) >> row_shift));
+  L.kbits = L.pbits + qbits;
+  return L;
 }
 
 inline int select_flagged(prb_ctx *ctx, SearchWs &w, const uint32_t *in, const uint8_t *flags, uint32_t *out, size_t n, int64_t *nsel) {
diff --git a/priblast_amd/csrc/search_kernels.hpp b/priblast_amd/csrc/search_kernels.hpp
--- a/priblast_amd/csrc/search_kernels.hpp
+++ b/priblast_amd/csrc/search_kernels.hpp
@@ -119,18 +119,30 @@
 inline int64_t blk_seq_entries(int64_t nchars) { return (nchars >> 5) + 1; }
 hipError_t launch_blk_seq(const PageDev &pg, int32_t *blk_seq, hipStream_t s);
 constexpr int64_t kMaxFusedCands = 1 << 20, kMaxFusedEntries = 1 << 12;
+struct PairLayout {
+  bool narrow = false;
+  int shift = 0;
+  int pbits = 0;
+  int kbits = 0;
+  int begin = 0;
+  int local_bits = 0;
+  bool wide_key() const { return !narrow && kbits > 32; }
+  size_t key_bytes() const { return wide_key() ? 8 : 4; }
+  size_t val_bytes() const { return narrow ? 4 : 8; }
+};
+constexpr int kPairLocalBits = 5;
 hipError_t launch_pair_keys(const CandDev *cands, const int64_t *pair0, int32_t ncand, int64_t npairs, const PageDev &pg, int qmin,
-                            int shift, int dbits, bool wide, void *key, uint64_t *val, hipStream_t s);
+                            const PairLayout &lay, void *key, void *val, hipStream_t s);
 inline int64_t allow_words(int64_t npairs) { return (npairs + 63) / 64; }
-hipError_t launch_allow_test(const CandDev *cands, const int64_t *pair0, const uint64_t *val, int64_t npairs, const PageDev &pg,
-                             const AllowDev &allow, uint64_t *ballot, int32_t *count, hipStream_t s);
-hipError_t launch_allow_scatter(const void *key_in, const uint64_t *val_in, int64_t npairs, bool wide, const uint64_t *ballot,
-                                const int64_t *off, void *key_out, uint64_t *val_out, hipStream_t s);
+hipError_t launch_allow_test(const CandDev *cands, const int64_t *pair0, const void *val, const PairLayout &lay, int64_t npairs,
+                             const PageDev &pg, const AllowDev &allow, uint64_t *ballot, int32_t *count, hipStream_t s);
+hipError_t launch_allow_scatter(const void *key_in, const void *val_in, int64_t npairs, const PairLayout &lay, const uint64_t *ballot,
+                                const int64_t *off, void *key_out, void *val_out, hipStream_t s);
 constexpr int kFusePairs = 2048, kSliceRecBytes = 48;
 inline int64_t fused_slices(int64_t npairs) { return (npairs + kFusePairs - 1) / kFusePairs; }
-hipError_t launch_seed_extend(const CandDev *cands, const uint64_t *vals, int64_t npairs, const QBatchDev &qb, const PageDev &pg,
-                              const SearchConst &sc, ExtOpts o, const double *qacc, double thr, int max_query_len, void *slices,
-                              int32_t *slice_count, uint64_t *nseed, hipStream_t s);
+hipError_t launch_seed_extend(const CandDev *cands, const void *keys, const void *vals, const PairLayout &lay, int64_t npairs,
+                              const QBatchDev &qb, const PageDev &pg, const SearchConst &sc, ExtOpts o, const double *qacc, double thr,
+                              int max_query_len, void *slices, int32_t *slice_count, uint64_t *nseed, hipStream_t s);
 hipError_t launch_collect_slices(const void *slices, const int32_t *slice_count, const int64_t *slice_off, int64_t nslices, HitRec *out,
                                  hipStream_t s);
 
diff --git a/priblast_amd/csrc/search_stages.hpp b/priblast_amd/csrc/search_stages.hpp
--- a/priblast_amd/csrc/search_stages.hpp
+++ b/priblast_amd/csrc/search_stages.hpp
@@ -9,6 +9,9 @@
   double budget;
   double chunk_pairs;
   int row_shift;
+  int sort_bits;
+  bool local_order;
+  bool pair_wide;
   bool fused;
   bool front_ahead;
   bool sort_four_keys, sort_two_lengths;
diff --git a/priblast_amd/csrc/ungapped_kernels.hip b/priblast_amd/csrc/ungapped_kernels.hip
--- a/priblast_amd/csrc/ungapped_kernels.hip
+++ b/priblast_amd/csrc/ungapped_kernels.hip
@@ -257,10 +257,10 @@
   if (b < nblk) blk_seq[b] = seq_of(pg, (int)(b << kSeqBlkShift));
 }
 
-template <class Key>
+template <class Key, class Val>
 __global__ __launch_bounds__(kBlock) void k_pair_key(const CandDev *__restrict__ cands, const int64_t *__restrict__ pair0, int ncand,
                                                      int64_t npairs, PageDev pg, int qmin, int shift, int dbits,
-                                                     Key *__restrict__ key, uint64_t *__restrict__ val) {
+                                                     Key *__restrict__ key, Val *__restrict__ val) {
   __shared__ int64_t s_p0[kBlock + 1];
   __shared__ int s_c0;
   const int64_t p = (int64_t)blockIdx.x * kBlock + threadIdx.x;
@@ -291,13 +291,16 @@
   const uint32_t rowl = pl / qw, jrel = pl - rowl * qw;
   const uint32_t db_sp = (uint32_t)pg.sa[c.sp_db + (int)rowl];
   key[p] = ((Key)(uint32_t)(c.query - qmin) << dbits) | (Key)(db_sp >> shift);
-  val[p] = (uint64_t)db_sp | ((uint64_t)(uint32_t)ci << 32) | ((uint64_t)jrel << (32 + kPairCandBits));
+  if constexpr (sizeof(Val) == 4) val[p] = (uint32_t)ci | (jrel << kPairCandBits);
+  else val[p] = (uint64_t)db_sp | ((uint64_t)(uint32_t)ci << 32) | ((uint64_t)jrel << (32 + kPairCandBits));
 }
 
 __device__ __forceinline__ int pair_cand(uint64_t v) { return (int)((v >> 32) & ((1u << kPairCandBits) - 1)); }
-
+__device__ __forceinline__ int pair_cand(uint32_t v) { return (int)(v & ((1u << kPairCandBits) - 1)); }
+
+template <class Val>
 __global__ __launch_bounds__(kBlock) void k_allow_test(const CandDev *__restrict__ cands, const int64_t *__restrict__ pair0,
-                                                       const uint64_t *__restrict__ val, int64_t npairs, PageDev pg, AllowDev allow,
+                                                       const Val *__restrict__ val, int64_t npairs, PageDev pg, AllowDev allow,
                                                        uint64_t *__restrict__ ballot, int32_t *__restrict__ count) {
   const int64_t p = (int64_t)blockIdx.x * kBlock + threadIdx.x;
   bool ok = false;
@@ -313,10 +316,10 @@
     count[p >> 6] = __popcll(m);
   }
 }
-template <class Key>
-__global__ __launch_bounds__(kBlock) void k_allow_scatter(const Key *__restrict__ key_in, const uint64_t *__restrict__ val_in, int64_t npairs,
+template <class Key, class Val>
+__global__ __launch_bounds__(kBlock) void k_allow_scatter(const Key *__restrict__ key_in, const Val *__restrict__ val_in, int64_t npairs,
                                                           const uint64_t *__restrict__ ballot, const int64_t *__restrict__ off,
-                                                          Key *__restrict__ key_out, uint64_t *__restrict__ val_out) {
+                                                          Key *__restrict__ key_out, Val *__restrict__ val_out) {
   const int64_t p = (int64_t)blockIdx.x * kBlock + threadIdx.x;
   if (p >= npairs) return;
   const uint64_t m = ballot[p >> 6];
@@ -335,7 +338,10 @@
 
 struct FuseArgs {
   const CandDev *cands;
-  const uint64_t *vals;
+  const uint32_t *keys;
+  const void *vals;
+  int pbits;
+  int lshift, lbits;
   int64_t npairs;
   const double *qacc;
   double thr;
@@ -347,11 +353,18 @@
 
 constexpr int kFusePer = kFusePairs / kBlock;
 static_assert(kFusePer * kBlock == kFusePairs, "pairs per workgroup");
-template <int kAhead>
+static_assert(kFusePairs <= 65536 && kPairLocalBits <= 5, "a tile's order: 16-bit places, the buckets scanned by half a wavefront");
+template <bool kNarrow> __device__ __forceinline__ int sorted_pair_cand(const FuseArgs &f, int64_t x) {
+  if constexpr (kNarrow) return pair_cand(static_cast<const uint32_t *>(f.vals)[x]);
+  else return pair_cand(static_cast<const uint64_t *>(f.vals)[x]);
+}
+template <int kAhead, bool kNarrow>
 __global__ __launch_bounds__(kBlock) void k_seed_extend(FuseArgs f, QBatchDev qb, PageDev pg, SearchConst sc, ExtOpts o) {
   extern __shared__ __align__(16) uint8_t ungapped_smem[];
   __shared__ int32_t s_tab[kUtTotal];
   __shared__ unsigned s_kept, s_seeds, s_maxlen;
+  __shared__ uint16_t s_place[kNarrow ? kFusePairs : 1];
+  __shared__ unsigned s_bucket[kNarrow ? 1 << kPairLocalBits : 1];
   const int64_t b0 = (int64_t)blockIdx.x * kFusePairs;
   if (b0 >= f.npairs) return;
   const int64_t b1 = (b0 + kFusePairs < f.npairs ? b0 + kFusePairs : f.npairs) - 1;
@@ -360,15 +373,17 @@
     s_seeds = 0;
     s_maxlen = 0;
   }
+  if constexpr (kNarrow)
+    if (f.lbits > 0 && threadIdx.x < (1 << kPairLocalBits)) s_bucket[threadIdx.x] = 0;
   for (int t = threadIdx.x; t < kUtTotal; t += kBlock)
     s_tab[t] = t < kUtInternal   ? sc.stack37[t]
                : t < kUtMismatch ? sc.internal37[t - kUtInternal]
                : t < kUtInt11    ? sc.mismatchI37[t - kUtMismatch]
                                  : sc.int11[t - kUtInt11];
   const UngappedTabs tabs{s_tab + kUtStack, s_tab + kUtInternal, s_tab + kUtMismatch, s_tab + kUtInt11, sc.int22};
-  const int q0 = f.cands[pair_cand(f.vals[b0])].query;
+  const int q0 = f.cands[sorted_pair_cand<kNarrow>(f, b0)].query;
   const int nslots = qb.len[q0] + 1;
-  const bool staged = q0 == f.cands[pair_cand(f.vals[b1])].query && nslots <= f.qcap;
+  const bool staged = q0 == f.cands[sorted_pair_cand<kNarrow>(f, b1)].query && nslots <= f.qcap;
   float *s_acc = reinterpret_cast<float *>(ungapped_smem), *s_cond = s_acc + f.qcap;
   uint8_t *s_enc = reinterpret_cast<uint8_t *>(s_cond + f.qcap);
   if (staged) {
@@ -381,17 +396,64 @@
   }
   __syncthreads();
   const int lane = threadIdx.x & 63;
+  const int ntile = (int)(b1 - b0) + 1;
+  bool placed = false;
+  if constexpr (kNarrow) {
+    placed = f.lbits > 0;
+    if (placed) {
+      const unsigned bmask = (1u << f.lbits) - 1;
+      unsigned bucket[kFusePer];
+#pragma unroll
+      for (int it = 0; it < kFusePer; it++) {
+        const int i = it * kBlock + threadIdx.x;
+        bucket[it] = 0;
+        if (i < ntile) {
+          bucket[it] = (f.keys[b0 + i] >> f.lshift) & bmask;
+          atomicAdd(&s_bucket[bucket[it]], 1u);
+        }
+      }
+      __syncthreads();
+      if (threadIdx.x < 64) {
+        const unsigned cnt = lane < (1 << kPairLocalBits) ? s_bucket[lane] : 0;
+        unsigned incl = cnt;
+        for (int d = 1; d < (1 << kPairLocalBits); d <<= 1) {
+          const unsigned up = (unsigned)__shfl_up((int)incl, d);
+          if (lane >= d) incl += up;
+        }
+        if (lane < (1 << kPairLocalBits)) s_bucket[lane] = incl - cnt;
+      }
+      __syncthreads();
+#pragma unroll
+      for (int it = 0; it < kFusePer; it++) {
+        const int i = it * kBlock + threadIdx.x;
+        if (i < ntile) s_place[atomicAdd(&s_bucket[bucket[it]], 1u)] = (uint16_t)i;
+      }
+      __syncthreads();
+    }
+  }
   SliceRec *slice = f.slices + b0;
   unsigned nseed = 0, maxlen = 0;
   for (int it = 0; it < kFusePer; it++) {
-    const int64_t x = b0 + (int64_t)it * kBlock + threadIdx.x;
+    const int i = it * kBlock + threadIdx.x;
     bool keep = false;
     WalkHit w{};
     int query = 0;
-    if (x <= b1) {
-      const uint64_t v = f.vals[x];
-      const int db_sp = (int)(uint32_t)v, jrel = (int)(v >> (32 + kPairCandBits));
-      const CandDev c = f.cands[pair_cand(v)];
+    if (i < ntile) {
+      int64_t x = b0 + i;
+      int db_sp, jrel, ci;
+      if constexpr (kNarrow) {
+        if (placed) x = b0 + s_place[i];
+        const uint32_t v = static_cast<const uint32_t *>(f.vals)[x];
+        db_sp = (int)(f.keys[x] & ((1u << f.pbits) - 1));
+        jrel = (int)(v >> kPairCandBits);
+        ci = pair_cand(v);
+      } else {
+        const uint64_t v = static_cast<const uint64_t *>(f.vals)[x];
+        db_sp = (int)(uint32_t)v;
+        jrel = (int)(v >> (32 + kPairCandBits));
+        ci = pair_cand(v);
+      }
+      const CandDev c = f.cands[ci];
       int id = pg.blk_seq[db_sp >> kSeqBlkShift];
       while (id + 1 < pg.nseq && pg.start_pos[id + 1] <= db_sp) id++;
       const int sp0 = pg.start_pos[id];
@@ -496,31 +558,44 @@
   return hipGetLastError();
 }
 hipError_t launch_pair_keys(const CandDev *cands, const int64_t *pair0, int32_t ncand, int64_t npairs, const PageDev &pg, int qmin,
-                            int shift, int dbits, bool wide, void *key, uint64_t *val, hipStream_t s) {
-  if (wide)
-    return launch_1d(k_pair_key<uint64_t>, npairs, kBlock, 0, s, cands, pair0, ncand, npairs, pg, qmin, shift, dbits, (uint64_t *)key, val);
-  return launch_1d(k_pair_key<uint32_t>, npairs, kBlock, 0, s, cands, pair0, ncand, npairs, pg, qmin, shift, dbits, (uint32_t *)key, val);
-}
-hipError_t launch_allow_test(const CandDev *cands, const int64_t *pair0, const uint64_t *val, int64_t npairs, const PageDev &pg,
-                             const AllowDev &allow, uint64_t *ballot, int32_t *count, hipStream_t s) {
-  return launch_1d(k_allow_test, npairs, kBlock, 0, s, cands, pair0, val, npairs, pg, allow, ballot, count);
-}
-hipError_t launch_allow_scatter(const void *key_in, const uint64_t *val_in, int64_t npairs, bool wide, const uint64_t *ballot,
-                                const int64_t *off, void *key_out, uint64_t *val_out, hipStream_t s) {
-  if (wide)
-    return launch_1d(k_allow_scatter<uint64_t>, npairs, kBlock, 0, s, (const uint64_t *)key_in, val_in, npairs, ballot, off, (uint64_t *)key_out,
-                     val_out);
-  return launch_1d(k_allow_scatter<uint32_t>, npairs, kBlock, 0, s, (const uint32_t *)key_in, val_in, npairs, ballot, off, (uint32_t *)key_out,
-                   val_out);
-}
-hipError_t launch_seed_extend(const CandDev *cands, const uint64_t *vals, int64_t npairs, const QBatchDev &qb, const PageDev &pg,
-                              const SearchConst &sc, ExtOpts o, const double *qacc, double thr, int max_query_len, void *slices,
-                              int32_t *slice_count, uint64_t *nseed, hipStream_t s) {
+                            const PairLayout &lay, void *key, void *val, hipStream_t s) {
+  if (lay.narrow)
+    return launch_1d(k_pair_key<uint32_t, uint32_t>, npairs, kBlock, 0, s, cands, pair0, ncand, npairs, pg, qmin, 0, lay.pbits, (uint32_t *)key,
+                     (uint32_t *)val);
+  if (lay.wide_key())
+    return launch_1d(k_pair_key<uint64_t, uint64_t>, npairs, kBlock, 0, s, cands, pair0, ncand, npairs, pg, qmin, lay.shift, lay.pbits,
+                     (uint64_t *)key, (uint64_t *)val);
+  return launch_1d(k_pair_key<uint32_t, uint64_t>, npairs, kBlock, 0, s, cands, pair0, ncand, npairs, pg, qmin, lay.shift, lay.pbits,
+                   (uint32_t *)key, (uint64_t *)val);
+}
+hipError_t launch_allow_test(const CandDev *cands, const int64_t *pair0, const void *val, const PairLayout &lay, int64_t npairs,
+                             const PageDev &pg, const AllowDev &allow, uint64_t *ballot, int32_t *count, hipStream_t s) {
+  if (lay.narrow) return launch_1d(k_allow_test<uint32_t>, npairs, kBlock, 0, s, cands, pair0, (const uint32_t *)val, npairs, pg, allow, ballot, count);
+  return launch_1d(k_allow_test<uint64_t>, npairs, kBlock, 0, s, cands, pair0, (const uint64_t *)val, npairs, pg, allow, ballot, count);
+}
+hipError_t launch_allow_scatter(const void *key_in, const void *val_in, int64_t npairs, const PairLayout &lay, const uint64_t *ballot,
+                                const int64_t *off, void *key_out, void *val_out, hipStream_t s) {
+  if (lay.narrow)
+    return launch_1d(k_allow_scatter<uint32_t, uint32_t>, npairs, kBlock, 0, s, (const uint32_t *)key_in, (const uint32_t *)val_in, npairs, ballot,
+                     off, (uint32_t *)key_out, (uint32_t *)val_out);
+  if (lay.wide_key())
+    return launch_1d(k_allow_scatter<uint64_t, uint64_t>, npairs, kBlock, 0, s, (const uint64_t *)key_in, (const uint64_t *)val_in, npairs, ballot,
+                     off, (uint64_t *)key_out, (uint64_t *)val_out);
+  return launch_1d(k_allow_scatter<uint32_t, uint64_t>, npairs, kBlock, 0, s, (const uint32_t *)key_in, (const uint64_t *)val_in, npairs, ballot, off,
+                   (uint32_t *)key_out, (uint64_t *)val_out);
+}
+hipError_t launch_seed_extend(const CandDev *cands, const void *keys, const void *vals, const PairLayout &lay, int64_t npairs,
+                              const QBatchDev &qb, const PageDev &pg, const SearchConst &sc, ExtOpts o, const double *qacc, double thr,
+                              int max_query_len, void *slices, int32_t *slice_count, uint64_t *nseed, hipStream_t s) {
   if (npairs <= 0) return hipSuccess;
   const int qcap = query_lds_slots(max_query_len);
-  FuseArgs f{cands, vals, npairs, qacc, thr, static_cast<SliceRec *>(slices), slice_count, reinterpret_cast<unsigned long long *>(nseed),
-             qcap};
-  hipLaunchKernelGGL(k_seed_extend<8>, dim3((unsigned)fused_slices(npairs)), dim3(kBlock), (size_t)qcap * 9, s, f, qb, pg, sc, o);
+  const int lbits = lay.narrow ? std::min(lay.local_bits, kPairLocalBits) : 0;
+  FuseArgs f{cands, lay.narrow ? static_cast<const uint32_t *>(keys) : nullptr, vals, lay.pbits, lay.begin - lbits, lbits, npairs, qacc, thr,
+             static_cast<SliceRec *>(slices), slice_count, reinterpret_cast<unsigned long long *>(nseed), qcap};
+  if (lay.narrow)
+    hipLaunchKernelGGL((k_seed_extend<8, true>), dim3((unsigned)fused_slices(npairs)), dim3(kBlock), (size_t)qcap * 9, s, f, qb, pg, sc, o);
+  else
+    hipLaunchKernelGGL((k_seed_extend<8, false>), dim3((unsigned)fused_slices(npairs)), dim3(kBlock), (size_t)qcap * 9, s, f, qb, pg, sc, o);
   return hipGetLastError();
 }
 hipError_t launch_collect_slices(const void *slices, const int32_t *slice_count, const int64_t *slice_off, int64_t nslices, HitRec *out,
```

After: 7.771, median of 6. 1.01x the previous value.
